# linnanwang/FastGen

Measured on AMD Instinct MI355X. Metric: images/sec at 4-step distilled (DMD2) sampling, higher is better.
Workload: dtype fp32 (tensors, accumulate) with split-bf16 x3 MFMA conv products; 1 GPU; EDM CIFAR-10 32x32 SongUNet (55.7M params) DMD2 4-step 'sde' sampling, batch=512 per GPU; global_batch=512, sample_steps=4, parallelism=replicas x1 (no data-path collective), graph=True

## Files before the change

### fastgen_amd/_lib.py

```python
import ctypes
import os
from ctypes import POINTER, c_char_p, c_double, c_float, c_int, c_int64, c_size_t, c_uint64, c_void_p

_HERE = os.path.dirname(os.path.abspath(__file__))
LIB_PATH = os.path.join(_HERE, "libfastgen_amd.so")

FG_MAX_LEVELS = 8
FG_DTYPE_F32, FG_DTYPE_BF16, FG_DTYPE_BF16X3 = 0, 1, 2
DTYPE_NAMES = {"fp32": FG_DTYPE_F32, "bf16": FG_DTYPE_BF16, "bf16x3": FG_DTYPE_BF16X3}
FG_SAMPLE_SDE, FG_SAMPLE_ODE = 0, 1
SAMPLE_TYPES = {"sde": FG_SAMPLE_SDE, "ode": FG_SAMPLE_ODE}
FG_LOOP_X0, FG_LOOP_MEANFLOW, FG_LOOP_EULER = 0, 1, 2
LOOP_KINDS = {"x0": FG_LOOP_X0, "meanflow": FG_LOOP_MEANFLOW, "euler": FG_LOOP_EULER}
FG_SCHEDULE_EDM, FG_SCHEDULE_RF = 0, 1
FG_DROP_PRECOND_INPUT, FG_DROP_PRECOND_OUTPUT = 1, 2
FG_BWD_DECODER, FG_BWD_ENCODER, FG_BWD_EMBED = 1, 2, 4
FG_MODEL_SONGUNET, FG_MODEL_DHARIWAL = 0, 1


class fg_edm_config(ctypes.Structure):
    _fields_ = [
        ("img_resolution", c_int), ("img_channels", c_int), ("label_dim", c_int), ("augment_dim", c_int),
        ("model_channels", c_int), ("num_levels", c_int), ("channel_mult", c_int * FG_MAX_LEVELS),
        ("channel_mult_emb", c_int), ("num_blocks", c_int), ("num_attn_resolutions", c_int),
        ("attn_resolutions", c_int * FG_MAX_LEVELS), ("channel_mult_noise", c_int), ("sigma_data", c_double),
        ("sigma_shift", c_double), ("compute_dtype", c_int), ("r_timestep", c_int), ("drop_precond", c_int),
        ("schedule", c_int), ("model_type", c_int),
    ]


class fg_edm2_config(ctypes.Structure):
    _fields_ = [
        ("img_resolution", c_int), ("img_channels", c_int), ("label_dim", c_int), ("model_channels", c_int), ("num_levels", c_int),
        ("channel_mult", c_int * FG_MAX_LEVELS), ("channel_mult_noise", c_int), ("channel_mult_emb", c_int), ("num_blocks", c_int),
        ("num_attn_resolutions", c_int), ("attn_resolutions", c_int * FG_MAX_LEVELS), ("label_balance", c_double),
        ("concat_balance", c_double), ("res_balance", c_double), ("attn_balance", c_double), ("clip_act", c_double),
        ("sigma_data", c_double), ("sigma_shift", c_double), ("compute_dtype", c_int), ("drop_precond", c_int),
    ]


class fg_dit_config(ctypes.Structure):
    _fields_ = [("input_size", c_int), ("patch_size", c_int), ("in_channels", c_int), ("hidden_size", c_int), ("depth", c_int),
                ("num_heads", c_int), ("mlp_hidden", c_int), ("embedding_rows", c_int), ("r_timestep", c_int), ("compute_dtype", c_int)]


class fg_wan_config(ctypes.Structure):
    _fields_ = [("num_heads", c_int), ("head_dim", c_int), ("in_channels", c_int), ("out_channels", c_int), ("text_dim", c_int),
                ("freq_dim", c_int), ("ffn_dim", c_int), ("num_layers", c_int), ("rope_max_seq_len", c_int), ("chunk_size", c_int),
                ("total_num_frames", c_int), ("eps", c_float)]


class fg_wan_block_taps(ctypes.Structure):
    _fields_ = [("attn1", c_void_p), ("x_attn1", c_void_p), ("attn2", c_void_p), ("x_attn2", c_void_p), ("x_ffn", c_void_p)]


class fg_dit_sampler_config(ctypes.Structure):
    _fields_ = [("t_scale", c_double), ("guidance_scale", c_double), ("use_sit_convention", c_int), ("time_cond_diff", c_int),
                ("net_pred_flow", c_int), ("schedule", c_int)]


class fg_wan_sampler_config(ctypes.Structure):
    _fields_ = [("t_scale", c_double), ("context_noise", c_double), ("net_pred_flow", c_int), ("schedule", c_int), ("prefill_frames", c_int)]


class fg_wan_guided_sampler_config(ctypes.Structure):
    _fields_ = [("t_scale", c_double), ("context_noise", c_double), ("guidance", c_int)]


SIGNATURES = {
    "fg_last_error": (c_char_p, []),
    "fg_version": (c_char_p, []),
    "fg_edm_create": (c_int, [POINTER(fg_edm_config), POINTER(c_void_p)]),
    "fg_edm_destroy": (None, [c_void_p]),
    "fg_edm_num_params": (c_int, [c_void_p]),
    "fg_edm_param_info": (c_int, [c_void_p, c_int, POINTER(c_char_p), POINTER(c_int), POINTER(c_int64)]),
    "fg_edm_bind_param": (c_int, [c_void_p, c_char_p, c_void_p, c_int64]),
    "fg_edm_pack_weights": (c_int, [c_void_p, c_void_p]),
    "fg_edm_workspace_bytes": (c_size_t, [c_void_p, c_int]),
    "fg_edm_forward": (c_int, [c_void_p, c_void_p, c_void_p, c_void_p, c_void_p, c_void_p, c_void_p, c_int, c_void_p,
                               c_size_t, c_void_p]),
    "fg_edm_num_feature_taps": (c_int, [c_void_p]),
    "fg_edm_feature_info": (c_int, [c_void_p, c_int, POINTER(c_char_p), POINTER(c_int), POINTER(c_int)]),
    "fg_edm_forward_features": (c_int, [c_void_p, c_void_p, c_void_p, c_void_p, c_void_p, c_void_p, POINTER(c_void_p), c_int,
                                        c_void_p, c_size_t, c_void_p]),
    "fg_sampler_run": (c_int, [c_void_p, c_void_p, c_void_p, POINTER(c_double), c_int, c_int, c_int, c_void_p, c_uint64,
                               c_void_p, c_int, c_void_p, c_size_t, c_int, c_void_p]),
    "fg_edm_t_list": (c_int, [c_int, POINTER(c_double)]),
    "fg_rf_t_list": (c_int, [c_int, POINTER(c_double)]),
    "fg_edm_profile_begin": (c_int, [c_void_p]),
    "fg_edm_profile_end": (c_int, [c_void_p, POINTER(c_int64), POINTER(c_double), POINTER(c_double)]),
    "fg_edm_num_blocks": (c_int, [c_void_p]),
    "fg_edm_block_info": (c_int, [c_void_p, c_int, POINTER(c_char_p), POINTER(c_int), POINTER(c_int), POINTER(c_int),
                                  POINTER(c_int), POINTER(c_int)]),
    "fg_edm_run_block": (c_int, [c_void_p, c_int, c_void_p, c_int, c_void_p, c_int, c_void_p, c_void_p, c_int, c_void_p,
                                 c_size_t, c_void_p]),
    "fg_op_gn_coeffs": (c_int, [c_void_p, c_int, c_void_p, c_int, c_void_p, c_void_p, c_float, c_void_p, c_int, c_int, c_void_p]),
    "fg_op_adm_conv_pack_bytes": (c_size_t, [c_int, c_int, c_int, c_int]),
    "fg_op_adm_conv_pack": (c_int, [c_int, c_void_p, c_void_p, c_int, c_int, c_int, c_void_p]),
    "fg_op_adm_conv": (c_int, [c_int, c_int, c_void_p, c_int, c_void_p, c_int, c_int, c_int, c_int, c_int, c_void_p, c_int, c_void_p,
                               c_void_p, c_void_p, c_int, c_void_p, c_int, c_void_p]),
    "fg_op_adm_gn_workspace_bytes": (c_size_t, [c_int, c_int, c_int]),
    "fg_op_adm_gn_coeffs": (c_int, [c_void_p, c_int, c_void_p, c_int, c_void_p, c_void_p, c_float, c_void_p, c_int, c_void_p, c_int,
                                    c_int, c_void_p, c_size_t, c_void_p]),
    "fg_op_adm_attention": (c_int, [c_void_p, c_void_p, c_int, c_int, c_int, c_void_p]),
    "fg_op_adm_map_in": (c_int, [c_void_p, c_void_p, c_void_p, c_void_p, c_int, c_void_p, c_int, c_int, c_void_p]),
    "fg_op_latents": (c_int, [c_void_p, c_double, c_void_p, c_int64, c_void_p]),
    "fg_op_forward_process": (c_int, [c_void_p, c_void_p, c_double, c_int, c_void_p, c_int64, c_void_p]),
    "fg_op_x0_to_eps": (c_int, [c_void_p, c_void_p, c_double, c_int, c_void_p, c_int64, c_void_p]),
    "fg_op_conv_wgrad_workspace_bytes": (ctypes.c_size_t, [c_int, c_int, c_int, c_int, c_int]),
    "fg_op_conv_wgrad": (c_int, [c_void_p, c_void_p, c_void_p, c_int, c_int, c_int, c_int, c_int, c_int, c_void_p, ctypes.c_size_t, c_void_p]),
    "fg_op_conv_wgrad_f32": (c_int, [c_void_p, c_void_p, c_void_p, c_int, c_int, c_int, c_int, c_int, c_int, c_void_p, ctypes.c_size_t, c_void_p]),
    "fg_edm_bind_grad": (c_int, [c_void_p, c_char_p, c_void_p, c_int64]),
    "fg_edm_block_backward_workspace_bytes": (c_size_t, [c_void_p, c_int, c_int]),
    "fg_edm_run_block_backward": (c_int, [c_void_p, c_int, c_void_p, c_int, c_void_p, c_int, c_void_p, c_void_p, c_void_p,
                                          c_void_p, c_void_p, c_int, c_void_p, c_size_t, c_void_p]),
    "fg_edm_backward_workspace_bytes": (c_size_t, [c_void_p, c_int]),
    "fg_edm_backward": (c_int, [c_void_p, c_void_p, c_void_p, c_void_p, c_void_p, c_void_p, c_void_p, c_int, c_int, c_void_p,
                                c_size_t, c_void_p]),
    "fg_edm_forward_train": (c_int, [c_void_p, c_void_p, c_void_p, c_void_p, c_void_p, c_void_p, c_void_p, c_int, c_void_p,
                                     c_size_t, c_void_p]),
    "fg_edm_backward_ex": (c_int, [c_void_p, c_void_p, c_void_p, c_void_p, c_void_p, c_void_p, c_void_p, c_void_p, c_void_p, c_int,
                                   c_int, c_void_p, c_size_t, c_void_p]),
    "fg_edm_backward_part": (c_int, [c_void_p, c_void_p, c_void_p, c_void_p, c_void_p, c_void_p, c_void_p, c_void_p, c_void_p, c_int,
                                     c_int, c_int, c_void_p, c_size_t, c_void_p]),
    "fg_edm2_create": (c_int, [POINTER(fg_edm2_config), POINTER(c_void_p)]),
    "fg_edm2_destroy": (None, [c_void_p]),
    "fg_edm2_num_params": (c_int, [c_void_p]),
    "fg_edm2_param_info": (c_int, [c_void_p, c_int, POINTER(c_char_p), POINTER(c_int), POINTER(c_int64)]),
    "fg_edm2_bind_param": (c_int, [c_void_p, c_char_p, c_void_p, c_int64]),
    "fg_edm2_pack_weights": (c_int, [c_void_p, c_void_p]),
    "fg_edm2_workspace_bytes": (c_size_t, [c_void_p, c_int]),
    "fg_edm2_forward": (c_int, [c_void_p, c_void_p, c_void_p, c_void_p, c_void_p, c_void_p, c_int, c_void_p, c_size_t, c_void_p]),
    "fg_edm2_set_training": (c_int, [c_void_p, c_int]),
    "fg_edm2_sampler_run": (c_int, [c_void_p, c_void_p, c_void_p, POINTER(c_double), c_int, c_int, c_int, c_void_p, c_uint64,
                                    c_void_p, c_int, c_void_p, c_size_t, c_int, c_void_p]),
    "fg_edm2_num_blocks": (c_int, [c_void_p]),
    "fg_edm2_block_info": (c_int, [c_void_p, c_int, POINTER(c_char_p), POINTER(c_int), POINTER(c_int), POINTER(c_int),
                                   POINTER(c_int), POINTER(c_int)]),
    "fg_edm2_run_block": (c_int, [c_void_p, c_int, c_void_p, c_int, c_void_p, c_int, c_void_p, c_void_p, c_int, c_void_p,
                                  c_size_t, c_void_p]),
    "fg_dit_create": (c_int, [POINTER(fg_dit_config), POINTER(c_void_p)]),
    "fg_dit_destroy": (None, [c_void_p]),
    "fg_dit_num_params": (c_int, [c_void_p]),
    "fg_dit_param_info": (c_int, [c_void_p, c_int, POINTER(c_char_p), POINTER(c_int), POINTER(c_int64)]),
    "fg_dit_bind_param": (c_int, [c_void_p, c_char_p, c_void_p, c_int64]),
    "fg_dit_pack_weights": (c_int, [c_void_p, c_void_p]),
    "fg_dit_pack_group": (c_int, [c_void_p, c_char_p, c_char_p, c_void_p]),
    "fg_dit_workspace_bytes": (c_size_t, [c_void_p, c_int]),
    "fg_dit_forward": (c_int, [c_void_p, c_void_p, c_void_p, c_void_p, c_void_p, c_void_p, c_void_p, c_int, c_void_p, c_size_t, c_void_p]),
    "fg_dit_forward_features": (c_int, [c_void_p, c_void_p, c_void_p, c_void_p, c_void_p, c_void_p, c_void_p, POINTER(c_int), POINTER(c_void_p),
                                        c_int, c_int, c_void_p, c_size_t, c_void_p]),
    "fg_dit_sampler_workspace_bytes": (c_size_t, [c_void_p, c_int, c_int]),
    "fg_dit_sampler_run": (c_int, [c_void_p, POINTER(fg_dit_sampler_config), c_void_p, c_void_p, c_void_p, POINTER(c_double), c_int, c_int, c_int,
                                   c_void_p, c_uint64, c_void_p, c_int, c_void_p, c_size_t, c_int, c_void_p]),
    "fg_wan_sampler_workspace_bytes": (c_size_t, [c_void_p, c_int, c_int, c_int, c_int]),
    "fg_wan_sampler_run": (c_int, [c_void_p, POINTER(fg_wan_sampler_config), c_void_p, POINTER(c_double), c_int, c_int, POINTER(c_int), c_void_p,
                                   c_uint64, c_int, c_int, c_int, c_int, c_void_p, c_size_t, c_int, c_void_p]),
    "fg_wan_guided_sampler_workspace_bytes": (c_size_t, [c_void_p, c_int, c_int, c_int, c_int, c_int, c_int]),
    "fg_wan_guided_sampler_run": (c_int, [c_void_p, POINTER(fg_wan_guided_sampler_config), c_void_p, POINTER(c_double), POINTER(c_double), c_int,
                                          c_void_p, c_uint64, c_int, c_int, c_int, c_int, c_void_p, c_size_t, c_int, c_void_p]),
    "fg_op_guided_multistep": (c_int, [c_void_p, c_void_p, c_void_p, c_void_p, c_void_p, c_void_p, c_int, c_int, c_int64, c_void_p]),
    "fg_wan_select_cache_tag": (c_int, [c_void_p, c_int]),
    "fg_wan_create": (c_int, [POINTER(fg_wan_config), POINTER(c_void_p)]),
    "fg_wan_destroy": (None, [c_void_p]),
    "fg_wan_num_params": (c_int, [c_void_p]),
    "fg_wan_param_info": (c_int, [c_void_p, c_int, POINTER(c_char_p), POINTER(c_int), POINTER(c_int64)]),
    "fg_wan_bind_param": (c_int, [c_void_p, c_char_p, c_void_p, c_int64]),
    "fg_wan_pack_weights": (c_int, [c_void_p, c_void_p]),
    "fg_wan_pack_group": (c_int, [c_void_p, c_char_p, c_char_p, c_void_p]),
    "fg_wan_workspace_bytes": (c_size_t, [c_void_p, c_int, c_int, c_int, c_int]),
    "fg_wan_clear_caches": (c_int, [c_void_p, c_void_p]),
    "fg_wan_set_text": (c_int, [c_void_p, c_void_p, c_int, c_int, c_void_p, c_size_t, c_void_p]),
    "fg_wan_forward": (c_int, [c_void_p, c_void_p, c_void_p, c_void_p, c_int, c_int, c_int, c_int, c_int, c_int, c_void_p, c_size_t,
                               c_void_p]),
    "fg_wan_forward_block_causal": (c_int, [c_void_p, c_void_p, c_void_p, c_void_p, c_int, c_int, c_int, c_int, c_void_p, c_size_t, c_void_p]),
    "fg_wan_forward_features": (c_int, [c_void_p, c_void_p, c_void_p, c_void_p, c_int, c_int, c_int, c_int, c_int, c_int, c_int, POINTER(c_int),
                                        POINTER(fg_wan_block_taps), c_int, c_void_p, c_void_p, c_void_p, c_size_t, c_void_p]),
    "fg_disc_edm_num_params": (c_int, [c_int]),
    "fg_disc_edm_workspace_bytes": (c_size_t, [c_int, c_int]),
    "fg_disc_edm_run": (c_int, [c_void_p, c_int, c_void_p, c_void_p, c_void_p, c_void_p, c_void_p, c_int, c_void_p, c_size_t, c_void_p]),
    "fg_edm_jvp": (c_int, [c_void_p, c_void_p, c_void_p, c_void_p, c_void_p, c_void_p, c_void_p, c_void_p, c_void_p, c_void_p, c_int,
                           c_void_p, c_size_t, c_void_p]),
    "fg_edm_set_dropout": (c_int, [c_void_p, c_float, c_uint64]),
    "fg_op_dropout_mask": (c_int, [c_void_p, c_int64, c_float, ctypes.c_uint32, c_uint64, c_void_p]),
    "fg_edm_set_augment": (c_int, [c_void_p, c_void_p]),
    "fg_edm_set_training": (c_int, [c_void_p, c_int]),
    "fg_op_images_to_u8": (c_int, [c_void_p, c_void_p, c_int64, c_int, c_int, c_int, c_void_p]),
    "fg_op_randn": (c_int, [c_void_p, c_int64, c_uint64, c_uint64, c_void_p]),
    "fg_op_attention": (c_int, [c_void_p, c_void_p, c_void_p, c_void_p, c_int, c_int, c_int, c_int, c_int, c_void_p]),
    "fg_op_attention_split": (c_int, [c_void_p, c_void_p, c_void_p, c_void_p, c_int, c_int, c_int, c_int, c_int, c_int, c_void_p]),
    "fg_op_gemm_bf16": (c_int, [c_void_p, c_void_p, c_void_p, c_void_p, c_int, c_int, c_int, c_int, c_void_p, c_int, c_int, c_void_p,
                                c_int, c_void_p]),
    "fg_op_gemm_x3": (c_int, [c_void_p, c_void_p, c_void_p, c_void_p, c_int, c_int, c_int, c_int, c_void_p, c_int, c_int, c_void_p,
                              c_int, c_void_p]),
}

_lib = None


def lib():
    global _lib
    if _lib is None:
        if not os.path.exists(LIB_PATH):
            raise RuntimeError(
                f"{LIB_PATH} not found: build it with `python -c 'import __graft_entry__ as g; g.build()'` "
                "(or `make -C fastgen_amd/csrc`).  fastgen_amd has no non-HIP fallback.")
        L = ctypes.CDLL(LIB_PATH)
        for name, (res, args) in SIGNATURES.items():
            fn = getattr(L, name)
            fn.restype = res
            fn.argtypes = args
        _lib = L
    return _lib


class FastGenAMDError(RuntimeError):
    pass


def check(rc: int):
    if rc != 0:
        msg = lib().fg_last_error().decode("utf-8", "replace")
        raise FastGenAMDError(f"fastgen_amd error {rc}: {msg}")
```

### fastgen_amd/csrc/aux.hip

```cpp
#include "common.h"
#include "misc.h"

namespace {

constexpr int APITCH = 144;
constexpr int HWID = 34, HROWS = 6;

template <typename T>
__global__ __launch_bounds__(256) void aux_head_kernel(const typename DT<T>::ST* __restrict__ x, const float2* __restrict__ ab,
                                                       const typename DT<T>::WT* __restrict__ wpack, const float* __restrict__ bias,
                                                       const float* __restrict__ x_t, const float* __restrict__ coef,
                                                       float* __restrict__ out, float* __restrict__ raw, int B, int C, int cout) {
    typedef typename DT<T>::ST ST;
    typedef typename DT<T>::WT WT;
    constexpr int KC = DT<T>::KC, KK = KC / 16, OPP = KC / 8;
    constexpr int FB = DT<T>::FRAG_BYTES, WP = DT<T>::WPARTS;
    constexpr bool FAST = DT<T>::FAST;
    constexpr int LOG_OPP = (OPP == 8) ? 3 : 2;
    constexpr int PSTRIDE = 256 / OPP;
    constexpr int HALO_PIX = HROWS * HWID;
    constexpr int NITEMS = (HALO_PIX * OPP + 255) / 256;
    __shared__ __attribute__((aligned(16))) char smem[HALO_PIX * APITCH];

    const int tid = threadIdx.x, lane = tid & 63, wave = tid >> 6;
    const int r = lane & 31, h = lane >> 5;
    const int n = blockIdx.x >> 3, row0 = (blockIdx.x & 7) * 4;
    const int oct = tid & (OPP - 1), hq0 = tid >> LOG_OPP;
    const int nchunk = C / KC;

    f32x16 acc;
#pragma unroll
    for (int i = 0; i < 16; ++i) acc[i] = 0.f;

    for (int chunk = 0; chunk < nchunk; ++chunk) {
        float2 abr[8];
        {
            const float2* p = ab + (size_t)n * C + chunk * KC + oct * 8;
#pragma unroll
            for (int j = 0; j < 8; j += 2) {
                const f32x4 q = *reinterpret_cast<const f32x4*>(p + j);
                abr[j] = make_float2(q[0], q[1]);
                abr[j + 1] = make_float2(q[2], q[3]);
            }
        }
#pragma unroll
        for (int i = 0; i < NITEMS; ++i) {
            const int hq = hq0 + i * PSTRIDE;
            if (hq < HALO_PIX) {
                const int hx = hq % HWID, hy = hq / HWID;
                const int y = row0 + hy - 1, xx = hx - 1;
                float o[8];
#pragma unroll
                for (int j = 0; j < 8; ++j) o[j] = 0.f;
                if (y >= 0 && y < 32 && xx >= 0 && xx < 32) {
                    const ST* p = x + (((size_t)n * 32 + y) * 32 + xx) * C + chunk * KC + oct * 8;
                    const f32x4 lo = load4(p), hi = load4(p + 4);
#pragma unroll
                    for (int j = 0; j < 4; ++j) {
                        o[j] = silu_f<FAST>(fmaf(lo[j], abr[j].x, abr[j].y));
                        o[j + 4] = silu_f<FAST>(fmaf(hi[j], abr[j + 4].x, abr[j + 4].y));
                    }
                }
                lds_store_a<T>(smem + hq * APITCH + oct * FB, o);
            }
        }
        __syncthreads();
        const WT* wp = wpack + (size_t)chunk * 9 * KK * 512 * WP + lane * 8;
#pragma unroll
        for (int tap = 0; tap < 9; ++tap) {
            const char* abase = smem + ((wave + tap / 3) * HWID + r + tap % 3) * APITCH + h * FB;
#pragma unroll
            for (int kk = 0; kk < KK; ++kk) {
                const Frag8<T> af = lds_read_a<T>(abase, kk);
                const Frag8<T> bf = load_wfrag<T>(wp + (tap * KK + kk) * 512 * WP);
                mma16(acc, af, bf);
            }
        }
        __syncthreads();
    }
    if (r < cout) {
        const float c_skip = coef[2 * B + n], c_out = coef[3 * B + n];
        const float bv = bias[r];
        const int y = row0 + wave;
#pragma unroll
        for (int i = 0; i < 16; ++i) {
            const size_t o = (((size_t)n * cout + r) * 32 + y) * 32 + acc_row(i, h);
            out[o] = c_skip * x_t[o] + c_out * (acc[i] + bv);
            if (raw) raw[o] = acc[i] + bv;
        }
    }
}

template <typename T>
__global__ void pack_aux_weights_kernel(const float* __restrict__ w, typename DT<T>::WT* __restrict__ out, int C, int cout) {
    constexpr int KC = DT<T>::KC, KK = KC / 16;
    const int total = C * 9 * 32;
    for (int idx = blockIdx.x * blockDim.x + threadIdx.x; idx < total; idx += gridDim.x * blockDim.x) {
        int t = idx;
        const int j = t % 8; t /= 8;
        const int lane = t % 64; t /= 64;
        const int kk = t % KK; t /= KK;
        const int tap = t % 9; t /= 9;
        const int chunk = t;
        const int co = lane & 31;
        const int ci = chunk * KC + kk * 16 + 8 * (lane >> 5) + j;
        const float v = (co < cout) ? w[((size_t)co * C + ci) * 9 + tap] : 0.f;
        if constexpr (DT<T>::WPARTS == 1) {
            out[idx] = (typename DT<T>::WT)v;
        } else {
            const size_t o = ((size_t)idx / 512) * 1024 + (idx % 512);
            const __bf16 hi = (__bf16)v;
            out[o] = hi;
            out[o + 512] = (__bf16)(v - (float)hi);
        }
    }
}

template <typename T>
__global__ __launch_bounds__(256) void stem_kernel(const float* __restrict__ x, const float* __restrict__ c_in,
                                                   const T* __restrict__ wpack, const float* __restrict__ bias,
                                                   T* __restrict__ out, float2* __restrict__ stats, int B, int res, int cin) {
    const int lane = threadIdx.x & 63, wave = threadIdx.x >> 6;
    const int r = lane & 31, h = lane >> 5;
    const int hw = res * res;
    const long long p0 = ((long long)blockIdx.x * 4 + wave) * 32;
    const int n = (int)(p0 / hw);
    if (n >= B) return;
    const int pix = (int)(p0 % hw) + r;
    const int y = pix / res, xx = pix % res;
    const float ci_scale = c_in[n];
    f32x16 acc[4];
#pragma unroll
    for (int nt = 0; nt < 4; ++nt)
#pragma unroll
        for (int i = 0; i < 16; ++i) acc[nt][i] = 0.f;
#pragma unroll
    for (int s = 0; s < 2; ++s) {
        float v[8];
#pragma unroll
        for (int j = 0; j < 8; ++j) {
            const int k = s * 16 + 8 * h + j;
            const int ci = k / 9, kh = (k % 9) / 3, kw = k % 3;
            const int yy = y + kh - 1, xs = xx + kw - 1;
            v[j] = 0.f;
            if (k < cin * 9 && yy >= 0 && yy < res && xs >= 0 && xs < res)
                v[j] = ci_scale * x[(((size_t)n * cin + ci) * res + yy) * res + xs];
        }
        Frag8<T> af;
        store_frag(reinterpret_cast<T*>(&af), v);
#pragma unroll
        for (int nt = 0; nt < 4; ++nt) {
            const Frag8<T> bf = load_frag(wpack + ((s * 4 + nt) * 64 + lane) * 8);
            mma16(acc[nt], af, bf);
        }
    }
    T* obase = out + ((size_t)n * hw + (p0 % hw)) * 128;
#pragma unroll
    for (int nt = 0; nt < 4; ++nt) {
        const float bv = bias[nt * 32 + r];
        float sv = 0.f, qv = 0.f;
#pragma unroll
        for (int i = 0; i < 16; ++i) {
            const float v = acc[nt][i] + bv;
            obase[(size_t)acc_row(i, h) * 128 + nt * 32 + r] = (T)v;
            sv += v;
            qv = fmaf(v, v, qv);
        }
        if (stats) {
            sv += __shfl_xor(sv, 32), qv += __shfl_xor(qv, 32);
            sv += __shfl_xor(sv, 1), qv += __shfl_xor(qv, 1);
            sv += __shfl_xor(sv, 2), qv += __shfl_xor(qv, 2);
            if (h == 0 && (r & 3) == 0)
                stats[((size_t)n * (hw / 32) + (int)(p0 % hw) / 32) * 32 + nt * 8 + (r >> 2)] = make_float2(sv, qv);
        }
    }
}

template <typename T>
__global__ void pack_stem_weights_kernel(const float* __restrict__ w, T* __restrict__ out, int cin) {
    const int idx = blockIdx.x * blockDim.x + threadIdx.x;
    if (idx >= 2 * 4 * 64 * 8) return;
    const int j = idx & 7, lane = (idx >> 3) & 63, nt = (idx >> 9) & 3, s = idx >> 11;
    const int co = nt * 32 + (lane & 31), k = s * 16 + 8 * (lane >> 5) + j;
    out[idx] = (k < cin * 9) ? (T)w[(size_t)co * cin * 9 + k] : (T)0.f;
}

}

size_t aux_pack_elems(int C) { return (size_t)C * 9 * 32; }

int launch_pack_aux_weights(int dtype, const float* w, void* out, int C, int cout, hipStream_t s) {
    const int grid = (int)((aux_pack_elems(C) + 255) / 256);
    if (dtype == 2)
        hipLaunchKernelGGL(pack_aux_weights_kernel<bf16x3>, dim3(grid), dim3(256), 0, s, w, (__bf16*)out, C, cout);
    else if (dtype)
        hipLaunchKernelGGL(pack_aux_weights_kernel<__bf16>, dim3(grid), dim3(256), 0, s, w, (__bf16*)out, C, cout);
    else
        hipLaunchKernelGGL(pack_aux_weights_kernel<float>, dim3(grid), dim3(256), 0, s, w, (float*)out, C, cout);
    return (int)hipGetLastError();
}

int aux_head_supported(int dtype, int res, int C, int cout) { return res == 32 && C % (dtype == 1 ? 64 : 32) == 0 && cout <= 32; }

int launch_aux_head(int dtype, const void* x, const float2* ab, const void* wpack, const float* bias, const float* x_t,
                    const float* coef, float* out, int B, int C, int cout, hipStream_t s, float* raw) {
    if (dtype == 2)
        hipLaunchKernelGGL(aux_head_kernel<bf16x3>, dim3(B * 8), dim3(256), 0, s, (const float*)x, ab, (const __bf16*)wpack, bias, x_t, coef, out, raw, B, C, cout);
    else if (dtype)
        hipLaunchKernelGGL(aux_head_kernel<__bf16>, dim3(B * 8), dim3(256), 0, s, (const __bf16*)x, ab, (const __bf16*)wpack, bias, x_t, coef, out, raw, B, C, cout);
    else
        hipLaunchKernelGGL(aux_head_kernel<float>, dim3(B * 8), dim3(256), 0, s, (const float*)x, ab, (const float*)wpack, bias, x_t, coef, out, raw, B, C, cout);
    return (int)hipGetLastError();
}

int stem_supported(int res, int cin, int cout) { return cout == 128 && cin * 9 <= 32 && (res * res) % 32 == 0; }
size_t stem_pack_elems() { return 2 * 4 * 64 * 8; }
int launch_pack_stem_weights(int dtype, const float* w, void* out, int cin, hipStream_t s) {
    if (dtype)
        hipLaunchKernelGGL(pack_stem_weights_kernel<__bf16>, dim3(16), dim3(256), 0, s, w, (__bf16*)out, cin);
    else
        hipLaunchKernelGGL(pack_stem_weights_kernel<float>, dim3(16), dim3(256), 0, s, w, (float*)out, cin);
    return (int)hipGetLastError();
}
int launch_stem(int dtype, const float* x, const float* c_in, const void* wpack, const float* bias, void* out, float2* stats,
                int B, int res, int cin, hipStream_t s) {
    const long long waves = (long long)B * res * res / 32;
    dim3 grid((unsigned)((waves + 3) / 4));
    if (dtype)
        hipLaunchKernelGGL(stem_kernel<__bf16>, grid, dim3(256), 0, s, x, c_in, (const __bf16*)wpack, bias, (__bf16*)out, stats, B, res, cin);
    else
        hipLaunchKernelGGL(stem_kernel<float>, grid, dim3(256), 0, s, x, c_in, (const float*)wpack, bias, (float*)out, stats, B, res, cin);
    return (int)hipGetLastError();
}
```

### fastgen_amd/csrc/engine.hip

```cpp
#include <hip/hip_runtime.h>

#include <cmath>
#include <cstdarg>
#include <cstdio>
#include <cstdlib>
#include <cstring>
#include <string>
#include <map>
#include <vector>

#include "../../include/fastgen_amd.h"
#include "common.h"
#include "adm.h"
#include "edm2.h"
#include "conv.h"
#include "misc.h"

namespace {

thread_local std::string g_err;

int fail(int code, const char* fmt, ...) {
    char buf[512];
    va_list ap;
    va_start(ap, fmt);
    vsnprintf(buf, sizeof buf, fmt, ap);
    va_end(ap);
    g_err = buf;
    return code;
}

#define HIP_TRY(expr)                                                                                          \
    do {                                                                                                       \
        hipError_t e_ = (hipError_t)(expr);                                                                    \
        if (e_ != hipSuccess) return fail(FG_EHIP, "%s failed: %s (%s:%d)", #expr, hipGetErrorString(e_), __FILE__, __LINE__); \
    } while (0)

struct Param {
    std::string name;
    int ndim = 0;
    int64_t shape[4] = {1, 1, 1, 1};
    int64_t numel = 0;
    const float* ptr = nullptr;
    float* grad = nullptr;
};

enum Kind { K_STEM, K_BLOCK, K_AUX_NORM, K_AUX_CONV };

struct Block {
    std::string key;
    Kind kind = K_BLOCK;
    int cin = 0, cout = 0, res_in = 0, res_out = 0;
    bool up = false, down = false, attn = false, has_skip = false, is_dec = false;
    int skip_c = 0;
    int temb_off = 0;
    int norm0_w = -1, norm0_b = -1, conv0_w = -1, conv0_b = -1, aff_w = -1, aff_b = -1, norm1_w = -1, norm1_b = -1,
        conv1_w = -1, conv1_b = -1, skip_w = -1, skip_b = -1, norm2_w = -1, norm2_b = -1, qkv_w = -1, qkv_b = -1,
        proj_w = -1, proj_b = -1, w = -1, b = -1;
    void *p_conv0 = nullptr, *p_conv1 = nullptr, *p_skip = nullptr, *p_qkv = nullptr, *p_proj = nullptr;
    void *p_conv0_ws = nullptr, *p_conv1_ws = nullptr;
    void* p_conv0_sub = nullptr;
    int tap = -1;
    float* qkv_bias = nullptr;
    void* p_qv = nullptr;
    float* qv_bias = nullptr;
    void* p_aux = nullptr;
    void* p_stem = nullptr;
};

struct Arena {
    char* base = nullptr;
    size_t off = 0, cap = 0;
    bool dry = false;
    void* take(size_t bytes) {
        off = (off + 255) & ~(size_t)255;
        void* p = dry ? nullptr : base + off;
        off += bytes;
        return p;
    }
    template <typename T>
    T* get(size_t n) {
        return reinterpret_cast<T*>(take(n * sizeof(T)));
    }
};

struct Act {
    void* p = nullptr;
    float2* st = nullptr;
    int slots = 0;
};

struct AdmWs {
    float *e2 = nullptr, *lab = nullptr;
    float2* part = nullptr;
    std::vector<float*> skip;
    float *xa = nullptr, *xb = nullptr, *h = nullptr, *s = nullptr, *t1 = nullptr, *qkv = nullptr, *a = nullptr;
};
struct AdmNet;

struct Workspace {
    AdmWs adm;
    float *coef, *emb0, *emb1, *emb, *temb;
    float2 *ab0, *ab1, *ab2;
    float2 *mr0 = nullptr, *mr1 = nullptr, *mr2 = nullptr;
    void* a1d = nullptr;
    bool infer = false;
    DropArgs drop;
    std::vector<Act> skip;
    Act xa, xb, h, xattn;
    void *sbuf, *aout, *pool;
    void *cvt1, *cvt2;
    void *q, *k, *vt;
    float *x, *x_pred, *eps;
    double* tl;
    uint64_t* seed;
};

struct BlockStash {
    void* h = nullptr;
    float2 *ab0 = nullptr, *ab1 = nullptr, *ab2 = nullptr, *mr0 = nullptr, *mr1 = nullptr, *mr2 = nullptr;
    void *xattn = nullptr, *q = nullptr, *k = nullptr, *vt = nullptr, *aout = nullptr;
    void* a1d = nullptr;
    uint32_t index = 0;
};
struct TrainStash {
    std::vector<Act> dec_store;
    std::vector<BlockStash> blocks;
    float2* aux_ab = nullptr;
    float2* aux_mr = nullptr;
    float* raw_out = nullptr;
};

struct HandleBase {
    std::vector<Param> params;
    std::string name_prefix;
    std::vector<void*> owned;
    bool packed = false, device_ready = false;

    HandleBase() = default;
    HandleBase(const HandleBase&) = delete;
    HandleBase& operator=(const HandleBase&) = delete;
    ~HandleBase() {
        for (void* p : owned) (void)hipFree(p);
    }
    int find(const std::string& n) const {
        for (size_t i = 0; i < params.size(); ++i)
            if (params[i].name == n) return (int)i;
        return -1;
    }
    int add(const std::string& n, std::initializer_list<int64_t> shp) {
        Param p;
        p.name = name_prefix + n;
        p.ndim = (int)shp.size();
        p.numel = 1;
        int i = 0;
        for (int64_t s : shp) {
            p.shape[i++] = s;
            p.numel *= s;
        }
        params.push_back(p);
        return (int)params.size() - 1;
    }
    template <typename F>
    int check_bound(F&& optional) const {
        for (size_t i = 0; i < params.size(); ++i)
            if (!params[i].ptr && !optional((int)i)) return fail(FG_ENOTREADY, "parameter '%s' is not bound", params[i].name.c_str());
        return FG_OK;
    }
    int alloc(void** p, size_t bytes) {
        HIP_TRY(hipMalloc(p, bytes));
        owned.push_back(*p);
        return FG_OK;
    }
    void free(void* p) {
        if (!p) return;
        for (size_t i = 0; i < owned.size(); ++i)
            if (owned[i] == p) {
                owned.erase(owned.begin() + i);
                break;
            }
        (void)hipFree(p);
    }
};

int param_info(const HandleBase* h, int index, const char** name, int* ndim, int64_t shape[4]) {
    if (!h || index < 0 || index >= (int)h->params.size()) return fail(FG_EINVAL, "param index out of range");
    const Param& p = h->params[index];
    if (name) *name = p.name.c_str();
    if (ndim) *ndim = p.ndim;
    if (shape)
        for (int i = 0; i < 4; ++i) shape[i] = p.shape[i];
    return FG_OK;
}
int bind_param(HandleBase* h, const char* name, const float* device_ptr, int64_t numel, int* index = nullptr) {
    if (!h || !name || !device_ptr) return fail(FG_EINVAL, "null argument");
    const int i = h->find(name);
    if (i < 0) return fail(FG_EINVAL, "unknown parameter '%s'", name);
    if (h->params[i].numel != numel)
        return fail(FG_EINVAL, "parameter '%s': expected %lld elements, got %lld", name, (long long)h->params[i].numel, (long long)numel);
    h->params[i].ptr = device_ptr;
    h->packed = false;
    if (index) *index = i;
    return FG_OK;
}

struct ScalarRing {
    static constexpr int kSlots = 8, kDoubles = 72;
    struct Slot {
        double tl[kDoubles];
        uint64_t seed[8];
    };
    Slot* slots = nullptr;
    hipEvent_t ev[kSlots] = {};
    bool used[kSlots] = {};
    int next = 0;
    int ensure() {
        if (slots) return FG_OK;
        HIP_TRY(hipHostMalloc((void**)&slots, sizeof(Slot) * kSlots));
        for (int i = 0; i < kSlots; ++i) HIP_TRY(hipEventCreateWithFlags(&ev[i], hipEventDisableTiming));
        return FG_OK;
    }
    int upload(const double* tl, int n, uint64_t seed, double* tl_dev, uint64_t* seed_dev, hipStream_t s) {
        int rc = ensure();
        if (rc) return rc;
        const int si = next;
        next = (si + 1) % kSlots;
        if (used[si]) HIP_TRY(hipEventSynchronize(ev[si]));
        Slot& sl = slots[si];
        for (int i = 0; i < n; ++i) sl.tl[i] = tl[i];
        sl.seed[0] = seed;
        sl.seed[1] = 0;
        HIP_TRY(hipMemcpyAsync(tl_dev, sl.tl, sizeof(double) * n, hipMemcpyHostToDevice, s));
        HIP_TRY(hipMemcpyAsync(seed_dev, sl.seed, sizeof(uint64_t) * 2, hipMemcpyHostToDevice, s));
        HIP_TRY(hipEventRecord(ev[si], s));
        used[si] = true;
        return FG_OK;
    }
    void destroy() {
        if (slots) (void)hipHostFree(slots);
        for (int i = 0; i < kSlots; ++i)
            if (ev[i]) (void)hipEventDestroy(ev[i]);
        slots = nullptr;
    }
};

struct GraphEntry {
    std::vector<int64_t> key;
    hipGraph_t graph = nullptr;
    hipGraphExec_t exec = nullptr;
    void drop() {
        if (exec) (void)hipGraphExecDestroy(exec);
        if (graph) (void)hipGraphDestroy(graph);
        exec = nullptr, graph = nullptr;
        key.clear();
    }
};

template <typename F>
int graph_run(GraphEntry& e, const std::vector<int64_t>& key, hipStream_t& cap, hipStream_t s, F&& enqueue) {
    if (!e.exec || e.key != key) {
        e.drop();
        if (!cap) HIP_TRY(hipStreamCreateWithFlags(&cap, hipStreamNonBlocking));
        HIP_TRY(hipStreamBeginCapture(cap, hipStreamCaptureModeThreadLocal));
// ... 253 lines not shown
            b.skip_w = h->add(key + ".skip.weight", {cout, cin, 1, 1});
            b.skip_b = h->add(key + ".skip.bias", {cout});
        }
        if (attn) {
            b.norm2_w = h->add(key + ".norm2.weight", {cout});
            b.norm2_b = h->add(key + ".norm2.bias", {cout});
            b.qkv_w = h->add(key + ".qkv.weight", {3 * cout, cout, 1, 1});
            b.qkv_b = h->add(key + ".qkv.bias", {3 * cout});
            b.proj_w = h->add(key + ".proj.weight", {cout, cout, 1, 1});
            b.proj_b = h->add(key + ".proj.bias", {cout});
        }
        b.temb_off = h->temb_total;
        h->temb_total += cout;
        return b;
    };
    auto res_name = [](int r) { return std::to_string(r) + "x" + std::to_string(r); };

    std::vector<int> skips;
    int cout = c.img_channels;
    for (int level = 0; level < c.num_levels; ++level) {
        const int res = c.img_resolution >> level;
        if (level == 0) {
            Block b;
            b.key = "model.enc." + res_name(res) + "_conv";
            b.kind = K_STEM;
            b.cin = cout;
            b.cout = cout = c.model_channels;
            b.res_in = b.res_out = res;
            b.w = h->add(b.key + ".weight", {b.cout, b.cin, 3, 3});
            b.b = h->add(b.key + ".bias", {b.cout});
            h->enc.push_back(b);
        } else {
            h->enc.push_back(make_block("model.enc." + res_name(res) + "_down", cout, cout, res, false, true, false, 0, false));
        }
        skips.push_back(cout);
        for (int idx = 0; idx < c.num_blocks; ++idx) {
            const int cin = cout;
            cout = c.model_channels * c.channel_mult[level];
            h->enc.push_back(make_block("model.enc." + res_name(res) + "_block" + std::to_string(idx), cin, cout, res,
                                        false, false, is_attn_res(res), 0, false));
            if (std::to_string(idx).rfind("3", 0) == 0) h->enc.back().tap = h->num_taps++;
            skips.push_back(cout);
        }
    }
    for (int level = c.num_levels - 1; level >= 0; --level) {
        const int res = c.img_resolution >> level;
        if (level == c.num_levels - 1) {
            h->dec.push_back(make_block("model.dec." + res_name(res) + "_in0", cout, cout, res, false, false, true, 0, true));
            h->dec.push_back(make_block("model.dec." + res_name(res) + "_in1", cout, cout, res, false, false, false, 0, true));
        } else {
            h->dec.push_back(make_block("model.dec." + res_name(res) + "_up", cout, cout, res, true, false, false, 0, true));
        }
        for (int idx = 0; idx <= c.num_blocks; ++idx) {
            const int sk = skips.back();
            skips.pop_back();
            const int cin = cout + sk;
            cout = c.model_channels * c.channel_mult[level];
            const bool attn = (idx == c.num_blocks) && is_attn_res(res);
            h->dec.push_back(make_block("model.dec." + res_name(res) + "_block" + std::to_string(idx), cin, cout, res,
                                        false, false, attn, sk, true));
        }
        if (level == 0) {
            Block n;
            n.key = "model.dec." + res_name(res) + "_aux_norm";
            n.kind = K_AUX_NORM;
            n.cin = n.cout = cout;
            n.res_in = n.res_out = res;
            n.w = h->add(n.key + ".weight", {cout});
            n.b = h->add(n.key + ".bias", {cout});
            h->dec.push_back(n);
            Block a;
            a.key = "model.dec." + res_name(res) + "_aux_conv";
            a.kind = K_AUX_CONV;
            a.cin = cout;
            a.cout = c.img_channels;
            a.res_in = a.res_out = res;
            a.w = h->add(a.key + ".weight", {a.cout, a.cin, 3, 3});
            a.b = h->add(a.key + ".bias", {a.cout});
            h->dec.push_back(a);
        }
    }
    h->add("model.logvar_linear.weight", {1, h->noise_ch});
    h->add("model.logvar_linear.bias", {1});
    for (auto& b : h->enc)
        if (b.kind == K_BLOCK) h->blocks.push_back(&b);
    for (auto& b : h->dec)
        if (b.kind == K_BLOCK) h->blocks.push_back(&b);
}

int check_supported(const fg_edm* h) {
    const fg_edm_config& c = h->cfg;
    const int kc = h->dtype ? 64 : 32;
    if (c.img_resolution != 32 && c.img_resolution != 16 && c.img_resolution != 8)
        return fail(FG_EINVAL, "img_resolution %d unsupported (8, 16, 32)", c.img_resolution);
    if ((c.img_resolution >> (c.num_levels - 1)) < 8)
        return fail(FG_EINVAL, "lowest resolution %d < 8 unsupported", c.img_resolution >> (c.num_levels - 1));
    if (c.img_channels > 4) return fail(FG_EINVAL, "img_channels %d > 4 unsupported", c.img_channels);
    for (const Block* b : h->blocks) {
        if (b->cout != 256) return fail(FG_EINVAL, "%s: out_channels %d unsupported (kernels are tiled for 256)", b->key.c_str(), b->cout);
        if (b->cin % kc || (b->cin - b->skip_c) % kc)
            return fail(FG_EINVAL, "%s: in_channels %d not a multiple of %d", b->key.c_str(), b->cin, kc);
        if (b->attn && b->res_out > 16) return fail(FG_EINVAL, "%s: attention at %dx%d unsupported", b->key.c_str(), b->res_out, b->res_out);
    }
    return FG_OK;
}

void adm_build_layout(fg_edm* h);
int adm_check_supported(const fg_edm* h);
size_t adm_plan_workspace(const fg_edm* h, int B, Arena& A, Workspace& w);
int adm_pack_weights(fg_edm* h, hipStream_t s);
int adm_forward(fg_edm* h, const float* x_t, const double* t, int t_stride, const float* labels, float* out, int B, Workspace& w,
                hipStream_t s);
int adm_refuse(const fg_edm* h, const char* what) {
    return fail(FG_EINVAL, "%s is not implemented for DhariwalUNet (forward and sampling only)", what);
}

size_t plan_workspace(const fg_edm* h, int B, Arena& A, Workspace& w) {
    if (h->adm) return adm_plan_workspace(h, B, A, w);
    const fg_edm_config& c = h->cfg;
    const size_t tsz = h->dtype ? 2 : 4;
    const int R = c.img_resolution;
    size_t max_act = 0;
    int max_c = 0, max_attn_hw = 0;
    for (const Block& b : h->enc) max_act = std::max(max_act, (size_t)b.res_out * b.res_out * b.cout);
    for (const Block* b : h->blocks) {
        max_act = std::max(max_act, (size_t)b->res_out * b->res_out * b->cout);
        max_c = std::max(max_c, std::max(b->cin, b->cout));
        if (b->attn) max_attn_hw = std::max(max_attn_hw, b->res_out * b->res_out);
    }
    w.coef = A.get<float>(5 * (size_t)B);
    w.emb0 = A.get<float>((size_t)B * h->cond_ch);
    w.emb1 = A.get<float>((size_t)B * h->emb_ch);
    w.emb = A.get<float>((size_t)B * h->emb_ch);
    w.temb = A.get<float>((size_t)B * h->temb_total);
    w.ab0 = A.get<float2>((size_t)B * max_c);
    w.ab1 = A.get<float2>((size_t)B * max_c);
    w.ab2 = A.get<float2>((size_t)B * max_c);
    const size_t st_elems = (size_t)B * 32 * 64;
    auto act = [&](size_t elems, size_t st_n) {
        Act a;
        a.p = A.take(elems * tsz);
        a.st = A.get<float2>(st_n);
        return a;
    };
    w.skip.clear();
    for (const Block& b : h->enc)
        w.skip.push_back(act((size_t)B * b.res_out * b.res_out * b.cout,
                             (b.kind == K_STEM && b.p_stem) ? (size_t)B * b.res_out * b.res_out : st_elems));
    w.xa = act((size_t)B * max_act, st_elems);
    w.xb = act((size_t)B * max_act, st_elems);
    w.h = act((size_t)B * max_act, st_elems);
    w.sbuf = A.take((size_t)B * max_act * tsz);
    w.pool = A.take((size_t)B * max_act * tsz);
    w.cvt1 = A.take((size_t)B * max_act * 4 * tsz);
    w.cvt2 = A.take((size_t)B * max_act * 4 * tsz);
    w.xattn = act((size_t)B * max_attn_hw * 256, st_elems);
    w.aout = A.take((size_t)B * max_attn_hw * 256 * tsz);
    w.q = A.take((size_t)B * max_attn_hw * 256 * tsz);
    w.k = A.take((size_t)B * max_attn_hw * 256 * tsz);
    w.vt = A.take((size_t)B * max_attn_hw * 256 * tsz);
    const size_t img = (size_t)B * c.img_channels * R * R;
    w.x = A.get<float>(img);
    w.x_pred = A.get<float>(img);
    w.eps = A.get<float>(img);
    w.tl = A.get<double>(ScalarRing::kDoubles);
    w.seed = A.get<uint64_t>(8);
    return (A.off + 255) & ~(size_t)255;
}

int conv_launch(fg_edm* h, int ks, int pro, int res, int outmode, const ConvArgs& a, hipStream_t s) {
    const bool timed = h->prof_on && ks == 3 && res == RES_NONE && a.W == 32 && outmode == OUT_NHWC;
    hipEvent_t e0 = nullptr, e1 = nullptr;
    if (timed) {
        if (hipEventCreate(&e0) != hipSuccess || hipEventCreate(&e1) != hipSuccess) return (int)hipErrorUnknown;
        (void)hipEventRecord(e0, s);
    }
    const int rc = launch_conv_fused(h->cmode, ks, pro, res, outmode, a, s);
    if (timed) {
        (void)hipEventRecord(e1, s);
        h->prof_ev.push_back(e0);
        h->prof_ev.push_back(e1);
        h->prof_flops += 2.0 * a.B * a.H * a.W * (double)a.Cout * 9.0 * (a.C1 + a.C2);
    }
    return rc;
}

const float kSkipScale = (float)std::sqrt(0.5);
const float kBlockEps = 1e-6f;

int norm_coeffs(int dtype, const Act& x1, int c1, const Act& x2, int c2, const float* gamma, const float* beta, float2* ab,
                int B, int hw, hipStream_t s, float2* mr = nullptr) {
    if (x1.st && (!c2 || x2.st))
        HIP_TRY(launch_gn_finalize(x1.st, c1, x1.slots, c2 ? x2.st : nullptr, c2, c2 ? x2.slots : 0, gamma, beta, kBlockEps, ab, B, hw, s, mr));
    else
        HIP_TRY(launch_gn_coeffs(dtype, x1.p, c1, c2 ? x2.p : nullptr, c2, gamma, beta, kBlockEps, ab, B, hw, s, mr));
    return FG_OK;
}

void use_stash(Workspace& w, const BlockStash& st) {
    w.h.p = st.h;
    w.ab0 = st.ab0, w.ab1 = st.ab1, w.mr0 = st.mr0, w.mr1 = st.mr1;
    w.a1d = st.a1d;
    w.drop.block = st.index;
    if (st.xattn) {
        w.xattn.p = st.xattn;
        w.ab2 = st.ab2, w.mr2 = st.mr2;
        w.q = st.q, w.k = st.k, w.vt = st.vt, w.aout = st.aout;
    }
}
int block_index(const fg_edm* h, const Block* b) {
    for (size_t i = 0; i < h->blocks.size(); ++i)
        if (h->blocks[i] == b) return (int)i;
    return -1;
}

bool attn_merge_enabled() {
    static const bool on = [] {
        const char* e = getenv("FASTGEN_AMD_ATTN_MERGE");
        return !(e && e[0] == '0');
    }();
    return on;
}

int run_block(fg_edm* h, const Block& b, const Act& x1, int c1, const Act& x2, int c2, const float* temb, Act& out, int B,
              Workspace& w, hipStream_t s) {
    if (c1 + c2 != b.cin) return fail(FG_EINVAL, "%s: got %d+%d input channels, expected %d", b.key.c_str(), c1, c2, b.cin);
    const int hw_in = b.res_in * b.res_in, hw = b.res_out * b.res_out;
    const int res_mode = b.down ? RES_DOWN : (b.up ? RES_UP : RES_NONE);
    const int slots = conv_stat_slots(b.res_out);
    int rc;
    if ((rc = norm_coeffs(h->dtype, x1, c1, x2, c2, h->P(b.norm0_w), h->P(b.norm0_b), w.ab0, B, hw_in, s, w.mr0))) return rc;
    ConvArgs a{};
    a.src1 = x1.p; a.src2 = c2 ? x2.p : nullptr; a.C1 = c1; a.C2 = c2;
    a.Hs = a.Ws = b.res_in; a.H = a.W = b.res_out; a.B = B;
    a.ab = w.ab0; a.wpack = b.p_conv0; a.wpack_ws = b.p_conv0_ws; a.bias = h->P(b.conv0_b);
    a.temb = temb + b.temb_off; a.temb_stride = h->temb_total;
    a.resid = nullptr; a.scale = 1.0f; a.out = w.h.p; a.Cout = b.cout; a.stats = w.h.st;
    const bool x3_up = b.up && w.infer && !w.a1d && h->cmode == FG_DTYPE_BF16X3 && conv_ws_enabled();
    bool sub0 = false;
    if (x3_up && conv_subpix_mode() == 2 && b.p_conv0_sub) {
        ConvArgs p = a;
        p.wpack_ws = b.p_conv0_sub;
        sub0 = conv_x3ws_supported(3, PRO_GN_SILU, RES_SUBPIX, OUT_NHWC, p);
    }
    if (sub0) {
        a.wpack_ws = b.p_conv0_sub;
        w.h.slots = conv_launch_stat_slots(h->cmode, 3, PRO_GN_SILU, RES_SUBPIX, OUT_NHWC, a);
        HIP_TRY(conv_launch(h, 3, PRO_GN_SILU, RES_SUBPIX, OUT_NHWC, a, s));
    } else if (b.down && !c2) {
        HIP_TRY(launch_gn_silu_pool(h->dtype, x1.p, w.ab0, w.pool, B, b.res_out, b.res_out, c1, s));
        a.src1 = w.pool; a.Hs = a.Ws = b.res_out; a.ab = nullptr;
        w.h.slots = conv_launch_stat_slots(h->cmode, 3, PRO_NONE, RES_NONE, OUT_NHWC, a);
        HIP_TRY(conv_launch(h, 3, PRO_NONE, RES_NONE, OUT_NHWC, a, s));
    } else {
        w.h.slots = conv_launch_stat_slots(h->cmode, 3, PRO_GN_SILU, res_mode, OUT_NHWC, a);
        HIP_TRY(conv_launch(h, 3, PRO_GN_SILU, res_mode, OUT_NHWC, a, s));
    }
    ConvArgs d{};
    d.src1 = w.h.p; d.C1 = b.cout; d.Hs = d.Ws = d.H = d.W = b.res_out; d.B = B;
    d.ab = w.ab1; d.wpack = b.p_conv1; d.wpack_ws = b.p_conv1_ws; d.bias = h->P(b.conv1_b);
    d.scale = kSkipScale; d.Cout = b.cout;
    const void* resid = x1.p;
    if (b.has_skip) {
        bool low = false;
        if (x3_up && conv_subpix_mode() >= 1) {
            ConvArgs p = d;
            p.resid = w.sbuf; p.rshift = 1;
            low = conv_x3ws_supported(3, PRO_GN_SILU, RES_NONE, OUT_NHWC, p);
        }
        ConvArgs k{};
        k.src1 = x1.p; k.src2 = c2 ? x2.p : nullptr; k.C1 = c1; k.C2 = c2;
        k.Hs = k.Ws = b.res_in; k.H = k.W = low ? b.res_in : b.res_out; k.B = B;
        k.wpack = b.p_skip; k.bias = h->P(b.skip_b); k.scale = 1.0f; k.out = w.sbuf; k.Cout = b.cout;
        HIP_TRY(conv_launch(h, 1, PRO_NONE, low ? RES_NONE : res_mode, OUT_NHWC, k, s));
        resid = w.sbuf;
        d.rshift = low ? 1 : 0;
    }
    HIP_TRY(launch_gn_finalize(w.h.st, b.cout, w.h.slots, nullptr, 0, 0, h->P(b.norm1_w), h->P(b.norm1_b), kBlockEps, w.ab1, B, hw, s, w.mr1));
    Act& x_mid = b.attn ? w.xattn : out;
    d.resid = resid; d.out = x_mid.p; d.stats = x_mid.st;
    if (w.a1d) {
        HIP_TRY(launch_gn_act(h->dtype, 0, w.h.p, b.cout, nullptr, 0, w.ab1, w.a1d, B, b.res_out, 0, s, w.drop));
        d.src1 = w.a1d; d.ab = nullptr;
        x_mid.slots = conv_launch_stat_slots(h->cmode, 3, PRO_NONE, RES_NONE, OUT_NHWC, d);
        HIP_TRY(conv_launch(h, 3, PRO_NONE, RES_NONE, OUT_NHWC, d, s));
    } else {
        x_mid.slots = conv_launch_stat_slots(h->cmode, 3, PRO_GN_SILU, RES_NONE, OUT_NHWC, d);
        HIP_TRY(conv_launch(h, 3, PRO_GN_SILU, RES_NONE, OUT_NHWC, d, s));
    }
    if (b.attn) {
        HIP_TRY(launch_gn_finalize(x_mid.st, b.cout, x_mid.slots, nullptr, 0, 0, h->P(b.norm2_w), h->P(b.norm2_b), kBlockEps, w.ab2, B, hw, s, w.mr2));
        ConvArgs q{};
        q.src1 = x_mid.p; q.C1 = b.cout; q.Hs = q.Ws = q.H = q.W = b.res_out; q.B = B;
        if (w.infer && !w.a1d && h->cmode == FG_DTYPE_BF16X3 && hw == 256 && b.cout == 256 && b.p_qv && attn_merge_enabled()) {
            q.ab = w.ab2; q.wpack = b.p_qv; q.bias = b.qv_bias; q.scale = 1.0f; q.Cout = 2 * b.cout;
            q.q_out = w.q; q.vt_out = w.vt;
            HIP_TRY(conv_launch(h, 1, PRO_GN, RES_NONE, OUT_QV, q, s));
            HIP_TRY(launch_attention_merged((const float*)w.q, (const float*)x_mid.p, w.ab2, (const float*)w.vt, h->P(b.proj_b), kSkipScale,
                                            (float*)out.p, out.st, B, s));
            out.slots = 8;
            return FG_OK;
        }
        q.ab = w.ab2; q.wpack = b.p_qkv; q.bias = b.qkv_bias; q.scale = 1.0f; q.Cout = 3 * b.cout;
        q.q_out = w.q; q.k_out = w.k; q.vt_out = w.vt;
        HIP_TRY(conv_launch(h, 1, PRO_GN, RES_NONE, OUT_QKV, q, s));
        HIP_TRY(launch_attention(h->cmode, w.q, w.k, w.vt, w.aout, B, hw, s));
        ConvArgs p{};
        p.src1 = w.aout; p.C1 = b.cout; p.Hs = p.Ws = p.H = p.W = b.res_out; p.B = B;
        p.wpack = b.p_proj; p.bias = h->P(b.proj_b); p.resid = x_mid.p; p.scale = kSkipScale; p.out = out.p; p.Cout = b.cout;
        p.stats = out.st;
        HIP_TRY(conv_launch(h, 1, PRO_NONE, RES_NONE, OUT_NHWC, p, s));
        out.slots = slots;
    }
    return FG_OK;
}

int run_mapping(fg_edm* h, const float* labels, int B, Workspace& w, hipStream_t s) {
    const fg_edm_config& c = h->cfg;
    HIP_TRY(launch_mapping_in(w.coef + B, w.coef + 4 * (size_t)B, h->freqs, labels, c.label_dim,
                              h->P(h->find("model.map_label.weight")), h->P(h->find("model.map_label.bias")), w.emb0, B,
                              h->cond_ch, h->noise_ch, s, h->augment, h->augment ? h->P(h->find("model.map_augment.weight")) : nullptr, c.augment_dim));
    HIP_TRY(launch_linear(w.emb0, h->P(h->find("model.map_layer0.weight")), h->P(h->find("model.map_layer0.bias")), w.emb1,
                          B, h->cond_ch, h->emb_ch, 1, s));
    HIP_TRY(launch_linear(w.emb1, h->P(h->find("model.map_layer1.weight")), h->P(h->find("model.map_layer1.bias")), w.emb, B,
                          h->emb_ch, h->emb_ch, 1, s));
    HIP_TRY(launch_linear(w.emb, h->aff_w, h->aff_b, w.temb, B, h->emb_ch, h->temb_total, 0, s));
    return FG_OK;
}

int run_forward(fg_edm* h, const float* x_t, const double* t, int t_stride, const double* r, int r_stride,
                const float* labels, float* out, int B, Workspace& w, hipStream_t s, float* const* feats = nullptr,
                bool early = false, TrainStash* ts = nullptr) {
    if (h->adm) return adm_forward(h, x_t, t, t_stride, labels, out, B, w, s);
    const fg_edm_config& c = h->cfg;
    HIP_TRY(launch_precond_coef(t, t_stride, c.r_timestep ? r : nullptr, r_stride, c.sigma_data, h->shift(), 1e-6,
                                c.drop_precond, w.coef, B, s));
    int rc = run_mapping(h, labels, B, w, s);
    if (rc) return rc;
    w.drop = DropArgs{};
    w.infer = ts == nullptr;
    if (ts && h->dropout_p > 0.f) w.drop.p = h->dropout_p, w.drop.seed = h->dropout_seed;
    const Act none;
    const Act* x = nullptr;
    for (size_t i = 0; i < h->enc.size(); ++i) {
        const Block& b = h->enc[i];
        if (b.kind == K_STEM) {
            if (b.p_stem) {
                HIP_TRY(launch_stem(h->dtype, x_t, w.coef, b.p_stem, h->P(b.b), w.skip[i].p, w.skip[i].st, B, b.res_out, b.cin, s));
                w.skip[i].slots = b.res_out * b.res_out / 32;
            } else {
                HIP_TRY(launch_conv_in(h->dtype, x_t, w.coef, h->P(b.w), h->P(b.b), w.skip[i].p, B, b.res_out, b.cin, b.cout, s));
                w.skip[i].st = nullptr;
            }
        } else {
            if (ts) use_stash(w, ts->blocks[block_index(h, &b)]);
            rc = run_block(h, b, *x, b.cin, none, 0, w.temb, w.skip[i], B, w, s);
            if (rc) return rc;
            if (feats && b.tap >= 0 && feats[b.tap])
                HIP_TRY(launch_act_to_nchw(h->dtype, w.skip[i].p, feats[b.tap], B, b.cout, b.res_out * b.res_out, s));
        }
        x = &w.skip[i];
    }
    if (early) return FG_OK;
    int sp = (int)h->enc.size();
    Act* pong[2] = {&w.xa, &w.xb};
    int cur = 0;
    size_t di = 0;
    const float2* aux_ab = nullptr;
    for (const Block& b : h->dec) {
        if (b.kind == K_BLOCK) {
            const Act& x2 = b.skip_c ? w.skip[--sp] : none;
            Act& dst = ts ? ts->dec_store[di++] : *pong[cur];
            if (ts) use_stash(w, ts->blocks[block_index(h, &b)]);
            rc = run_block(h, b, *x, b.cin - b.skip_c, x2, b.skip_c, w.temb, dst, B, w, s);
            if (rc) return rc;
            x = &dst;
            cur ^= 1;
        } else if (b.kind == K_AUX_NORM) {
            if (ts) w.ab0 = ts->aux_ab, w.mr0 = ts->aux_mr;
            if ((rc = norm_coeffs(h->dtype, *x, b.cin, none, 0, h->P(b.w), h->P(b.b), w.ab0, B, b.res_in * b.res_in, s, ts ? w.mr0 : nullptr))) return rc;
            aux_ab = w.ab0;
        } else if (b.kind == K_AUX_CONV) {
            if (b.p_aux)
                HIP_TRY(launch_aux_head(h->cmode, x->p, aux_ab, b.p_aux, h->P(b.b), x_t, w.coef, out, B, b.cin, b.cout, s, ts ? ts->raw_out : nullptr));
            else
                HIP_TRY(launch_aux_out(h->dtype, x->p, aux_ab, h->P(b.w), h->P(b.b), x_t, w.coef, out, B, b.res_out, b.cin, b.cout, s, ts ? ts->raw_out : nullptr));
        }
    }
    return FG_OK;
}

int enqueue_sampler(fg_edm* h, const float* noise, const float* labels, const double* t_list, int steps, int type,
                    int loop, const float* eps, float* out, int B, Workspace& w, hipStream_t s) {
    const fg_edm_config& c = h->cfg;
    const int64_t total = (int64_t)B * c.img_channels * c.img_resolution * c.img_resolution;
    const StudentLoop L{noise, t_list, steps, type, c.schedule, total, w.x, w.eps, eps, w.tl, w.seed, out, s};
    if (loop == FG_LOOP_MEANFLOW)
        return meanflow_loop(L, w.x_pred, [&](int i, float* u) {
            return run_forward(h, w.x, w.tl + i, 0, w.tl + (type == FG_SAMPLE_SDE ? steps : i + 1), 0, labels, u, B, w, s);
        });
    return x0_loop(L, w.x_pred, [&](int i, float* pred) { return run_forward(h, w.x, w.tl + i, 0, w.tl + steps, 0, labels, pred, B, w, s); });
}

int ensure_device_state(fg_edm* h) {
    if (h->device_ready) return FG_OK;
    int rc;
    const size_t tsz = h->dtype ? 2 : 4;
    for (Block* b : h->blocks) {
        if ((rc = h->alloc(&b->p_conv0, conv_pack_elems(b->cout, b->cin, 3) * tsz))) return rc;
        if ((rc = h->alloc(&b->p_conv1, conv_pack_elems(b->cout, b->cout, 3) * tsz))) return rc;
        const bool x3 = h->cmode == FG_DTYPE_BF16X3;
        if ((x3 ? conv_x3ws_shape_ok(b->cout, b->cin, b->res_out) : conv_ws_shape_ok(h->cmode, b->cout, b->cin, b->res_out)) && !b->down &&
            (rc = h->alloc(&b->p_conv0_ws, conv_pack_elems(b->cout, b->cin, 3) * tsz)))
            return rc;
        if ((x3 ? conv_x3ws_shape_ok(b->cout, b->cout, b->res_out) : conv_ws_shape_ok(h->cmode, b->cout, b->cout, b->res_out)) &&
            (rc = h->alloc(&b->p_conv1_ws, conv_pack_elems(b->cout, b->cout, 3) * tsz)))
            return rc;
        if (x3 && b->up && conv_x3ws_shape_ok(b->cout, b->cin, b->res_in) && (rc = h->alloc(&b->p_conv0_sub, conv_pack_elems(b->cout, b->cin, 4) * 4)))
            return rc;
        if (b->has_skip && (rc = h->alloc(&b->p_skip, conv_pack_elems(b->cout, b->cin, 1) * tsz))) return rc;
        if (b->attn) {
            if ((rc = h->alloc(&b->p_qkv, conv_pack_elems(3 * b->cout, b->cout, 1) * tsz))) return rc;
            if ((rc = h->alloc(&b->p_proj, conv_pack_elems(b->cout, b->cout, 1) * tsz))) return rc;
            if ((rc = h->alloc((void**)&b->qkv_bias, sizeof(float) * 3 * b->cout))) return rc;
            if (x3 && b->cout == 256 && b->res_out == 16) {
                if ((rc = h->alloc(&b->p_qv, conv_pack_elems(2 * b->cout, b->cout, 1) * tsz))) return rc;
                if ((rc = h->alloc((void**)&b->qv_bias, sizeof(float) * 2 * b->cout))) return rc;
                if (!h->qv_w && (rc = h->alloc((void**)&h->qv_w, sizeof(float) * 2 * b->cout * b->cout))) return rc;
            }
        }
    }
    for (Block& b : h->enc)
        if (b.kind == K_STEM && stem_supported(b.res_out, b.cin, b.cout))
            if ((rc = h->alloc(&b.p_stem, stem_pack_elems() * tsz))) return rc;
    for (Block& b : h->dec)
        if (b.kind == K_AUX_CONV && aux_head_supported(h->cmode, b.res_out, b.cin, b.cout))
            if ((rc = h->alloc(&b.p_aux, aux_pack_elems(b.cin) * tsz))) return rc;
    if ((rc = h->alloc((void**)&h->aff_w, sizeof(float) * (size_t)h->temb_total * h->emb_ch))) return rc;
    if ((rc = h->alloc((void**)&h->aff_b, sizeof(float) * (size_t)h->temb_total))) return rc;
    const int half = h->noise_ch / 2;
    std::vector<float> fr(half);
    for (int j = 0; j < half; ++j) fr[j] = powf(1.0f / 10000.0f, (float)j / (float)(half - 1));
    if ((rc = h->alloc((void**)&h->freqs, sizeof(float) * half))) return rc;
    HIP_TRY(hipMemcpy(h->freqs, fr.data(), sizeof(float) * half, hipMemcpyHostToDevice));
    if (conv_prepare_all(h->cmode) != 0) return fail(FG_EHIP, "hipFuncSetAttribute(dynamic LDS) failed");
    if (launch_attention(h->cmode, nullptr, nullptr, nullptr, nullptr, 1, 256, nullptr) != 0) return fail(FG_EHIP, "attention prepare failed");
    if (h->cmode == FG_DTYPE_BF16X3 && launch_attention_merged(nullptr, nullptr, nullptr, nullptr, nullptr, 0.f, nullptr, nullptr, 1, nullptr) != 0)
        return fail(FG_EHIP, "attention prepare failed");
    h->device_ready = true;
    return FG_OK;
}

#include "engine_adm.inc"

}

extern "C" {

const char* fg_last_error(void) { return g_err.c_str(); }
const char* fg_version(void) { return "fastgen_amd 0.1 gfx950"; }

int fg_edm_create(const fg_edm_config* cfg, fg_edm** out) {
    if (!cfg || !out) return fail(FG_EINVAL, "null argument");
    if (cfg->num_levels < 1 || cfg->num_levels > FG_MAX_LEVELS || cfg->num_attn_resolutions < 0 ||
        cfg->num_attn_resolutions > FG_MAX_LEVELS)
        return fail(FG_EINVAL, "bad num_levels / num_attn_resolutions");
    if (cfg->compute_dtype != FG_DTYPE_F32 && cfg->compute_dtype != FG_DTYPE_BF16 && cfg->compute_dtype != FG_DTYPE_BF16X3)
        return fail(FG_EINVAL, "bad compute_dtype");
    if ((cfg->drop_precond & ~3) || (cfg->schedule != FG_SCHEDULE_EDM && cfg->schedule != FG_SCHEDULE_RF) ||
        (cfg->r_timestep & ~1))
        return fail(FG_EINVAL, "bad r_timestep / drop_precond / schedule");
    if (cfg->model_channels <= 0 || cfg->model_channels % 16 || cfg->channel_mult_noise < 1 || cfg->channel_mult_emb < 1)
        return fail(FG_EINVAL, "bad channel configuration");
    if (cfg->model_type != FG_MODEL_SONGUNET && cfg->model_type != FG_MODEL_DHARIWAL) return fail(FG_EINVAL, "bad model_type");
    fg_edm* h = new fg_edm();
    h->cfg = *cfg;
    h->cmode = cfg->compute_dtype;
    h->dtype = cfg->compute_dtype == FG_DTYPE_BF16 ? 1 : 0;
    h->emb_ch = cfg->model_channels * cfg->channel_mult_emb;
    int rc;
    if (cfg->model_type == FG_MODEL_DHARIWAL) {
        h->adm = new AdmNet();
        h->dtype = 0;
        h->noise_ch = h->cond_ch = cfg->model_channels;
        adm_build_layout(h);
        rc = adm_check_supported(h);
        if (rc) {
            delete h->adm;
            delete h;
            return rc;
        }
        *out = h;
        return FG_OK;
    }
    h->noise_ch = cfg->model_channels * cfg->channel_mult_noise;
    h->cond_ch = h->noise_ch * (cfg->r_timestep ? 2 : 1);
    build_layout(h);
    rc = check_supported(h);
    if (rc) {
        delete h;
        return rc;
    }
    *out = h;
    return FG_OK;
}

void fg_edm_destroy(fg_edm* h) {
    if (!h) return;
    h->sampler.release();
    for (hipEvent_t e : h->prof_ev) (void)hipEventDestroy(e);
    delete h->adm;
    delete h;
}

int fg_edm_num_params(const fg_edm* h) { return h ? (int)h->params.size() : 0; }

int fg_edm_param_info(const fg_edm* h, int index, const char** name, int* ndim, int64_t shape[4]) {
    return param_info(h, index, name, ndim, shape);
}

int fg_edm_bind_param(fg_edm* h, const char* name, const float* device_ptr, int64_t numel) {
    return bind_param(h, name, device_ptr, numel);
}

int fg_edm_pack_weights(fg_edm* h, void* stream) {
    if (!h) return fail(FG_EINVAL, "null handle");
    hipStream_t s = (hipStream_t)stream;
    auto unused = [&](int i) {
        const std::string& n = h->params[i].name;
        return (n == "model.map_augment.weight" && (h->adm || !h->augment)) || n.rfind("model.logvar_linear", 0) == 0;
    };
    int rc;
    if (h->adm) {
        if ((rc = h->check_bound(unused))) return rc;
        ++h->pack_epoch;
        if ((rc = adm_pack_weights(h, s))) return rc;
        h->sampler.graph.drop();
        h->packed = true;
        return FG_OK;
    }
    if ((rc = ensure_device_state(h)) || (rc = h->check_bound(unused))) return rc;
    ++h->pack_epoch;
    for (Block* b : h->blocks) {
        HIP_TRY(launch_pack_conv_weights(h->cmode, h->P(b->conv0_w), b->p_conv0, b->cout, b->cin, 3, 0, s));
        HIP_TRY(launch_pack_conv_weights(h->cmode, h->P(b->conv1_w), b->p_conv1, b->cout, b->cout, 3, 0, s));
        if (h->cmode == FG_DTYPE_BF16X3) {
            if (b->p_conv0_ws) HIP_TRY(launch_pack_conv_weights_x3ws(h->P(b->conv0_w), b->p_conv0_ws, b->cout, b->cin, s));
            if (b->p_conv0_sub) HIP_TRY(launch_pack_conv_weights_x3sub(h->P(b->conv0_w), b->p_conv0_sub, b->cout, b->cin, s));
            if (b->p_conv1_ws) HIP_TRY(launch_pack_conv_weights_x3ws(h->P(b->conv1_w), b->p_conv1_ws, b->cout, b->cout, s));
        } else {
            if (b->p_conv0_ws) HIP_TRY(launch_pack_conv_weights_ws(h->P(b->conv0_w), b->p_conv0_ws, b->cout, b->cin, s));
            if (b->p_conv1_ws) HIP_TRY(launch_pack_conv_weights_ws(h->P(b->conv1_w), b->p_conv1_ws, b->cout, b->cout, s));
        }
        if (b->has_skip) HIP_TRY(launch_pack_conv_weights(h->cmode, h->P(b->skip_w), b->p_skip, b->cout, b->cin, 1, 0, s));
        if (b->attn) {
            HIP_TRY(launch_pack_conv_weights(h->cmode, h->P(b->qkv_w), b->p_qkv, 3 * b->cout, b->cout, 1, 1, s));
            HIP_TRY(launch_pack_conv_weights(h->cmode, h->P(b->proj_w), b->p_proj, b->cout, b->cout, 1, 0, s));
            for (int plane = 0; plane < 3; ++plane)
                HIP_TRY(hipMemcpy2DAsync(b->qkv_bias + plane * b->cout, sizeof(float), h->P(b->qkv_b) + plane,
                                         3 * sizeof(float), sizeof(float), b->cout, hipMemcpyDeviceToDevice, s));
            if (b->p_qv) {
                HIP_TRY(launch_attn_merge_weights(h->P(b->qkv_w), h->P(b->qkv_b), h->P(b->proj_w), h->qv_w, b->qv_bias, b->cout, s));
                HIP_TRY(launch_pack_conv_weights(h->cmode, h->qv_w, b->p_qv, 2 * b->cout, b->cout, 1, 0, s));
            }
        }
// ... 71 lines not shown
    if (sample_steps < 1 || sample_steps > 64 || !out_host) return fail(FG_EINVAL, "bad sample_steps");
    const int num_steps = 1000;
    const double min_t = 0.002, max_t = 80.0, rho = 7.0;
    const double a = std::pow(min_t, 1.0 / rho), b = std::pow(max_t, 1.0 / rho);
    const int lo = (int)(0.002 * num_steps), hi = (int)(0.998 * num_steps);
    for (int i = 0; i <= sample_steps; ++i) {
        const int n = sample_steps + 1;
        const float step = ((float)lo - (float)hi) / (float)(n - 1);
        const float v = (i < n / 2) ? (float)hi + step * (float)i : (float)lo - step * (float)(n - 1 - i);
        const int idx = (int)v;
        const int j = num_steps - 1 - idx;
        const double dstep = 1.0 / (double)(num_steps - 1);
        const double ramp = (j < num_steps / 2) ? dstep * j : 1.0 - dstep * (double)(num_steps - 1 - j);
        double sig = std::pow(b + ramp * (a - b), rho);
        if (i == sample_steps) sig = 0.0;
        out_host[i] = sig > max_t ? max_t : sig;
    }
    return FG_OK;
}

int fg_rf_t_list(int sample_steps, double* out_host) {
    if (sample_steps < 1 || sample_steps > 64 || !out_host) return fail(FG_EINVAL, "bad sample_steps");
    const double max_t = 0.999;
    const int n = sample_steps + 1;
    const double step = (0.0 - max_t) / (double)(n - 1);
    for (int i = 0; i < n; ++i) {
        const double v = (i < n / 2) ? max_t + step * (double)i : 0.0 - step * (double)(n - 1 - i);
        out_host[i] = v > max_t ? max_t : v;
    }
    return FG_OK;
}

int fg_sampler_run(fg_edm* h, const float* noise, const float* class_labels, const double* t_list, int steps,
                   int sample_type, int loop_kind, const float* eps, uint64_t seed, float* out, int batch, void* workspace,
                   size_t workspace_bytes, int use_graph, void* stream) {
    if (!h || !noise || !t_list || !out) return fail(FG_EINVAL, "null argument");
    int rc = check_sampler_args(t_list, steps, sample_type, loop_kind, h->cfg.schedule);
    if (rc) return rc;
    if (loop_kind != FG_LOOP_X0 && loop_kind != FG_LOOP_MEANFLOW) return fail(FG_EINVAL, "bad loop_kind");
    if ((loop_kind == FG_LOOP_MEANFLOW) != (h->cfg.r_timestep != 0))
        return fail(FG_EINVAL, "FG_LOOP_MEANFLOW needs an r_timestep network and FG_LOOP_X0 a network without one");
    Workspace w;
    if ((rc = setup_ws(plan_workspace, h, batch, workspace, workspace_bytes, w))) return rc;
    if (!h->packed) return fail(FG_ENOTREADY, "weights are not packed (call fg_edm_pack_weights)");
    return sampler_launch(h->sampler, batch, t_list, steps, sample_type, loop_kind, seed, w.tl, w.seed, use_graph && !h->prof_on,
                          {(int64_t)(uintptr_t)noise, (int64_t)(uintptr_t)class_labels, (int64_t)(uintptr_t)eps, (int64_t)(uintptr_t)out,
                           (int64_t)(uintptr_t)workspace, sample_type == FG_SAMPLE_SDE && !eps},
                          (hipStream_t)stream, [&](hipStream_t q) {
                              return enqueue_sampler(h, noise, class_labels, t_list, steps, sample_type, loop_kind, eps, out, batch, w, q);
                          });
}

int fg_edm_profile_begin(fg_edm* h) {
    if (!h) return fail(FG_EINVAL, "null handle");
    for (hipEvent_t e : h->prof_ev) (void)hipEventDestroy(e);
    h->prof_ev.clear();
    h->prof_flops = 0.0;
    h->prof_on = true;
    return FG_OK;
}

int fg_edm_profile_end(fg_edm* h, int64_t* launches, double* total_ms, double* total_flops) {
    if (!h) return fail(FG_EINVAL, "null handle");
    h->prof_on = false;
    double ms = 0.0;
    for (size_t i = 0; i + 1 < h->prof_ev.size(); i += 2) {
        HIP_TRY(hipEventSynchronize(h->prof_ev[i + 1]));
        float t = 0.f;
        HIP_TRY(hipEventElapsedTime(&t, h->prof_ev[i], h->prof_ev[i + 1]));
        ms += t;
    }
    if (launches) *launches = (int64_t)h->prof_ev.size() / 2;
    if (total_ms) *total_ms = ms;
    if (total_flops) *total_flops = h->prof_flops;
    for (hipEvent_t e : h->prof_ev) (void)hipEventDestroy(e);
    h->prof_ev.clear();
    return FG_OK;
}

FG_API int fg_debug_conv_bench(int dtype, int batch, int cin, int res, int ks, int with_resid, int dbg, int iters, float* ms_out) {
    const size_t npix = (size_t)batch * res * res;
    float *x = nullptr, *out = nullptr, *resid = nullptr, *bias = nullptr;
    float2* ab = nullptr;
    void* wp = nullptr;
    if (dtype < 0 || dtype > 2) return fail(FG_EINVAL, "bad dtype");
    HIP_TRY(hipMalloc((void**)&x, npix * cin * 4));
    HIP_TRY(hipMalloc((void**)&out, npix * 256 * 4));
    HIP_TRY(hipMalloc((void**)&resid, npix * 256 * 4));
    HIP_TRY(hipMalloc((void**)&bias, 256 * 4));
    HIP_TRY(hipMalloc((void**)&ab, (size_t)batch * cin * 8));
    HIP_TRY(hipMalloc(&wp, (size_t)256 * cin * ks * ks * 4));
    {
        const size_t blk = 4u << 20;
        std::vector<uint16_t> hb(blk / 2);
        uint32_t st = 0x12345u;
        for (auto& v : hb) {
            st = st * 1664525u + 1013904223u;
            v = (uint16_t)(((st >> 16) & 0x8000u) | ((0x78u + ((st >> 12) & 7u)) << 7) | ((st >> 20) & 0x7fu));
        }
        auto fill = [&](void* dst, size_t bytes) -> int {
            for (size_t o = 0; o < bytes; o += blk)
                HIP_TRY(hipMemcpy((char*)dst + o, hb.data(), std::min(blk, bytes - o), hipMemcpyHostToDevice));
            return FG_OK;
        };
        int rc;
        if ((rc = fill(x, npix * cin * 4)) || (rc = fill(resid, npix * 256 * 4)) || (rc = fill(ab, (size_t)batch * cin * 8)) ||
            (rc = fill(wp, (size_t)256 * cin * ks * ks * (dtype == 1 ? 2 : 4))))
            return rc;
    }
    HIP_TRY(hipMemset(bias, 0, 256 * 4));
    if (conv_prepare_all(dtype) != 0) return fail(FG_EHIP, "prepare failed");
    ConvArgs a{};
    a.src1 = x; a.C1 = cin; a.Hs = a.Ws = a.H = a.W = res; a.B = batch;
    a.ab = ab; a.wpack = wp; a.wpack_ws = wp; a.bias = bias; a.resid = with_resid ? resid : nullptr; a.scale = 1.f; a.out = out; a.Cout = 256;
    a.dbg = dbg;
    hipEvent_t e0, e1;
    HIP_TRY(hipEventCreate(&e0));
    HIP_TRY(hipEventCreate(&e1));
    auto run = [&]() { return dbg >= 64 ? launch_conv_ws_debug(a, dbg - 64, nullptr) : dbg < 0 ? launch_conv_fused(dtype, ks, ks == 3 ? PRO_GN_SILU : PRO_NONE, RES_NONE, OUT_NHWC, a, nullptr) : launch_conv_debug(dtype, a, nullptr); };
    for (int i = 0; i < 3; ++i) HIP_TRY(run());
    HIP_TRY(hipEventRecord(e0, nullptr));
    for (int i = 0; i < iters; ++i) HIP_TRY(run());
    HIP_TRY(hipEventRecord(e1, nullptr));
    HIP_TRY(hipEventSynchronize(e1));
    float ms = 0.f;
    HIP_TRY(hipEventElapsedTime(&ms, e0, e1));
    if (ms_out) *ms_out = ms / iters;
    (void)hipEventDestroy(e0); (void)hipEventDestroy(e1);
    (void)hipFree(x); (void)hipFree(out); (void)hipFree(resid); (void)hipFree(bias); (void)hipFree(ab); (void)hipFree(wp);
    return FG_OK;
}

int fg_edm_num_blocks(const fg_edm* h) {
    if (h && h->adm) return adm_num_blocks(h);
    return h ? (int)h->blocks.size() : 0;
}

int fg_edm_block_info(const fg_edm* h, int index, const char** key, int* cin, int* cout, int* res_in, int* res_out,
                      int* has_attention) {
    if (h && h->adm) return adm_block_info(h, index, key, cin, cout, res_in, res_out, has_attention);
    if (!h || index < 0 || index >= (int)h->blocks.size()) return fail(FG_EINVAL, "block index out of range");
    const Block* b = h->blocks[index];
    if (key) *key = b->key.c_str();
    if (cin) *cin = b->cin;
    if (cout) *cout = b->cout;
    if (res_in) *res_in = b->res_in;
    if (res_out) *res_out = b->res_out;
    if (has_attention) *has_attention = b->attn ? 1 : 0;
    return FG_OK;
}

int fg_edm_run_block(fg_edm* h, int index, const float* x1, int c1, const float* x2, int c2, const float* emb, float* out,
                     int batch, void* workspace, size_t workspace_bytes, void* stream) {
    if (!h || !x1 || !emb || !out) return fail(FG_EINVAL, "null argument");
    if (h->adm) return adm_run_block(h, index, x1, c1, x2, c2, emb, out, batch, workspace, workspace_bytes, (hipStream_t)stream);
    if (!h->packed) return fail(FG_ENOTREADY, "weights are not packed (call fg_edm_pack_weights)");
    if (index < 0 || index >= (int)h->blocks.size()) return fail(FG_EINVAL, "block index out of range");
    Workspace w;
    int rc0 = setup_ws(plan_workspace, h, batch, workspace, workspace_bytes, w);
    if (rc0) return rc0;
    hipStream_t s = (hipStream_t)stream;
    HIP_TRY(launch_linear(emb, h->aff_w, h->aff_b, w.temb, batch, h->emb_ch, h->temb_total, 0, s));
    const Block& b = *h->blocks[index];
    const size_t npix_in = (size_t)batch * b.res_in * b.res_in, npix_out = (size_t)batch * b.res_out * b.res_out;
    Act a1, a2;
    HIP_TRY(launch_to_act(h->dtype, x1, w.cvt1, (int64_t)npix_in * c1, s));
    a1.p = w.cvt1;
    if (c2) {
        HIP_TRY(launch_to_act(h->dtype, x2, w.cvt2, (int64_t)npix_in * c2, s));
        a2.p = w.cvt2;
    }
    w.infer = true;
    int rc = run_block(h, b, a1, c1, a2, c2, w.temb, w.xa, batch, w, s);
    if (rc) return rc;
    HIP_TRY(launch_from_act(h->dtype, w.xa.p, out, (int64_t)npix_out * b.cout, s));
    return FG_OK;
}

#include "engine_train.inc"
#include "engine_dit.inc"
#include "engine_wan.inc"
#include "engine_sampler.inc"
#include "engine_edm2.inc"

int fg_op_gn_coeffs(const float* x1, int c1, const float* x2, int c2, const float* gamma, const float* beta, float eps,
                    float* ab_out, int batch, int hw, void* stream) {
    if (!x1 || !gamma || !beta || !ab_out) return fail(FG_EINVAL, "null argument");
    HIP_TRY(launch_gn_coeffs(0, x1, c1, c2 ? x2 : nullptr, c2, gamma, beta, eps, (float2*)ab_out, batch, hw, (hipStream_t)stream));
    return FG_OK;
}

size_t fg_op_adm_conv_pack_bytes(int mode, int cout, int cin, int ks) {
    if ((mode != FG_DTYPE_BF16 && mode != FG_DTYPE_BF16X3) || (ks != 1 && ks != 3) || cout <= 0 || cin <= 0 || cin % 32) return 0;
    return adm_conv_pack_elems(mode, cout, cin, ks) * sizeof(__bf16);
}
int fg_op_adm_conv_pack(int mode, const float* w_oihw, void* packed, int cout, int cin, int ks, void* stream) {
    if (!fg_op_adm_conv_pack_bytes(mode, cout, cin, ks))
        return fail(FG_EINVAL, "fg_op_adm_conv_pack: mode %d (1 bf16, 2 bf16x3), ks %d (1, 3), cout %d > 0, cin %d (multiple of 32)", mode,
                    ks, cout, cin);
    if (!w_oihw || !packed) return fail(FG_EINVAL, "fg_op_adm_conv_pack: null pointer");
    HIP_TRY(adm_pack_conv_weights(mode, w_oihw, packed, cout, cin, ks, (hipStream_t)stream));
    return FG_OK;
}
int fg_op_adm_conv(int mode, int ks, const float* src1, int c1, const float* src2, int c2, int batch, int hs, int h, int res_mode,
                   const float* ab, int silu, const void* packed, const float* bias, const float* resid, int resid_mode, float* out,
                   int cout, void* stream) {
    if ((mode != FG_DTYPE_BF16 && mode != FG_DTYPE_BF16X3) || (ks != 1 && ks != 3))
        return fail(FG_EINVAL, "fg_op_adm_conv: mode %d (1 bf16, 2 bf16x3), ks %d (1, 3)", mode, ks);
    if (c1 <= 0 || c1 % 32 || c2 < 0 || c2 % 32 || cout <= 0 || batch <= 0 || batch > 65535)
        return fail(FG_EINVAL, "fg_op_adm_conv: c1 %d > 0 and c2 %d >= 0 multiples of 32, cout %d > 0, batch %d in 1 .. 65535", c1, c2,
                    cout, batch);
    const bool res_ok = (res_mode == 0 && hs == h) || (res_mode == 1 && hs == 2 * h) || (res_mode == 2 && h == 2 * hs);
    if (h <= 0 || h > 4096 || !res_ok) return fail(FG_EINVAL, "fg_op_adm_conv: res_mode %d with hs %d, h %d", res_mode, hs, h);
    if (resid && (resid_mode < 0 || resid_mode > 2 || (resid_mode == 2 && h % 2)))
        return fail(FG_EINVAL, "fg_op_adm_conv: resid_mode %d (0, 1, 2 with h even) at h %d", resid_mode, h);
    if (!src1 || (c2 && !src2) || !packed || !out) return fail(FG_EINVAL, "fg_op_adm_conv: null pointer");
    if (((uintptr_t)src1 | (uintptr_t)(c2 ? src2 : nullptr) | (uintptr_t)packed) & 15 || (uintptr_t)ab & 7)
        return fail(FG_EINVAL, "fg_op_adm_conv: src1 / src2 / packed must be 16-byte aligned, ab 8-byte aligned");
    AdmConvArgs a;
    a.src1 = src1, a.src2 = c2 ? src2 : nullptr, a.C1 = c1, a.C2 = c2, a.Hs = hs, a.H = h, a.B = batch, a.res_mode = res_mode;
    a.ab = (const float2*)ab, a.silu = silu ? 1 : 0, a.w = packed, a.bias = bias, a.resid = resid, a.resid_mode = resid ? resid_mode : 0;
    a.out = out, a.Cout = cout;
    HIP_TRY(adm_launch_conv(mode, ks, a, (hipStream_t)stream));
    return FG_OK;
}
size_t fg_op_adm_gn_workspace_bytes(int batch, int hw, int c) {
    if (batch <= 0 || hw <= 0 || c <= 0) return 0;
    return adm_gn_part_elems(batch, hw, c) * sizeof(float2);
}
int fg_op_adm_gn_coeffs(const float* x1, int c1, const float* x2, int c2, const float* gamma, const float* beta, float eps,
                        const float* temb, int temb_stride, float* ab_out, int batch, int hw, void* workspace, size_t workspace_bytes,
                        void* stream) {
    const int C = c1 + c2;
    if (c1 <= 0 || c1 % 2 || c2 < 0 || c2 % 2 || C < 8)
        return fail(FG_EINVAL, "fg_op_adm_gn_coeffs: c1 %d > 0 and c2 %d >= 0 must be even, c1 + c2 >= 8", c1, c2);
    const int G = std::min(32, C / 4);
    if (C % G || (C / G) % 2)
        return fail(FG_EINVAL, "fg_op_adm_gn_coeffs: %d channels in %d groups: the group size must be a whole, even number", C, G);
    if (batch <= 0 || batch > 65535 || hw <= 0 || hw > (1 << 22))
        return fail(FG_EINVAL, "fg_op_adm_gn_coeffs: batch %d (1 .. 65535), hw %d (1 .. 2^22)", batch, hw);
    if (temb && temb_stride < 2 * C) return fail(FG_EINVAL, "fg_op_adm_gn_coeffs: temb_stride %d < 2 C = %d", temb_stride, 2 * C);
    if (!x1 || (c2 && !x2) || !gamma || !beta || !ab_out || !workspace) return fail(FG_EINVAL, "fg_op_adm_gn_coeffs: null pointer");
    if (((uintptr_t)x1 | (uintptr_t)(c2 ? x2 : nullptr) | (uintptr_t)ab_out | (uintptr_t)workspace) & 7)
        return fail(FG_EINVAL, "fg_op_adm_gn_coeffs: x1 / x2 / ab_out / workspace must be 8-byte aligned");
    const size_t need = fg_op_adm_gn_workspace_bytes(batch, hw, C);
    if (workspace_bytes < need)
        return fail(FG_EINVAL, "fg_op_adm_gn_coeffs: workspace too small (%zu < %zu bytes)", workspace_bytes, need);
    HIP_TRY(adm_launch_gn(x1, c1, c2 ? x2 : nullptr, c2, gamma, beta, eps, temb, temb_stride, (float2*)workspace, (float2*)ab_out, batch,
                          hw, (hipStream_t)stream));
    return FG_OK;
}
int fg_op_adm_attention(const float* qkv, float* out, int batch, int t, int heads, void* stream) {
    if (t <= 0 || t % 64 || heads <= 0 || heads > 65535 || batch <= 0 || batch > 65535)
        return fail(FG_EINVAL, "fg_op_adm_attention: t %d (a positive multiple of 64), heads %d, batch %d (1 .. 65535)", t, heads, batch);
    if (!qkv || !out) return fail(FG_EINVAL, "fg_op_adm_attention: null pointer");
    HIP_TRY(adm_launch_attention(qkv, out, batch, t, heads, (hipStream_t)stream));
    return FG_OK;
}
int fg_op_adm_map_in(const float* c_noise, const float* freqs, const float* aug, const float* wa, int aug_dim, float* out, int batch,
                     int n, void* stream) {
    if (batch <= 0 || n <= 0 || n % 2 || (int64_t)batch * n > (1 << 30) || (aug && aug_dim <= 0))
        return fail(FG_EINVAL, "fg_op_adm_map_in: batch %d > 0, n %d > 0 even, aug_dim %d > 0 with aug", batch, n, aug_dim);
    if (!c_noise || !freqs || !out || (aug && !wa)) return fail(FG_EINVAL, "fg_op_adm_map_in: null pointer");
    HIP_TRY(adm_launch_map_in(c_noise, freqs, aug, aug ? wa : nullptr, aug ? aug_dim : 0, out, batch, n, (hipStream_t)stream));
    return FG_OK;
}
int fg_op_latents(const float* noise, double t_init, float* out, int64_t total, void* stream) {
    HIP_TRY(launch_latents(noise, t_init, nullptr, 0, out, total, (hipStream_t)stream));
    return FG_OK;
}
int fg_op_forward_process(const float* x0, const float* eps, double t, int schedule, float* out, int64_t total,
                          void* stream) {
    HIP_TRY(launch_forward_process(x0, eps, t, nullptr, 0, schedule, out, total, (hipStream_t)stream));
    return FG_OK;
}
int fg_op_x0_to_eps(const float* xt, const float* x0, double t, int schedule, float* out, int64_t total, void* stream) {
    HIP_TRY(launch_x0_to_eps(xt, x0, t, nullptr, 0, schedule, 1e-6, out, total, (hipStream_t)stream));
    return FG_OK;
}
int fg_edm_set_dropout(fg_edm* h, float p, uint64_t seed) {
    if (!h) return fail(FG_EINVAL, "null handle");
    if (!(p >= 0.f && p < 1.f)) return fail(FG_EINVAL, "dropout probability must be in [0, 1), got %g", (double)p);
    h->dropout_p = p;
    h->dropout_seed = seed;
    return FG_OK;
}
int fg_op_guided_multistep(const float* v, float* x, float* x2, float* x_last, float* m_prev, const double* tab, int guided, int first,
                           int64_t total, void* stream) {
    if (!v || !x || !x_last || !m_prev || !tab || total <= 0) return fail(FG_EINVAL, "fg_op_guided_multistep: bad argument");
    HIP_TRY(launch_guided_multistep(v, x, x2, x_last, m_prev, tab, guided != 0, first != 0, total, (hipStream_t)stream));
    return FG_OK;
}

int fg_op_dropout_mask(float* out, int64_t total, float p, uint32_t block_index, uint64_t seed, void* stream) {
    if (!out || total <= 0 || (total % 8)) return fail(FG_EINVAL, "fg_op_dropout_mask: bad argument");
    DropArgs d;
    d.p = p, d.block = block_index, d.seed = seed;
    HIP_TRY(launch_dropout_mask(out, total, d, (hipStream_t)stream));
    return FG_OK;
}
int fg_edm_set_training(fg_edm* h, int training) {
    if (!h) return fail(FG_EINVAL, "null handle");
    if ((training != 0) != h->training && h->cfg.sigma_shift != 0.0) h->sampler.graph.drop();
    h->training = training != 0;
    return FG_OK;
}
int fg_edm_set_augment(fg_edm* h, const float* augment_labels) {
    if (!h) return fail(FG_EINVAL, "null handle");
    if (augment_labels && h->cfg.augment_dim <= 0) return fail(FG_EINVAL, "this network was built without augment_dim");
    h->augment = augment_labels;
    return FG_OK;
}
int fg_disc_edm_num_params(int res) { return disc_num_params(res); }
size_t fg_disc_edm_workspace_bytes(int res, int batch) { return disc_workspace_bytes(res, batch); }
int fg_disc_edm_run(const float* feat, int res, const float* const* params, float* logits, const float* dlogits, float* dfeat,
                    float* const* grads, int batch, void* workspace, size_t workspace_bytes, void* stream) {
    const int np = disc_num_params(res);
    if (!np) return fail(FG_EINVAL, "fg_disc_edm_run: resolution %d unsupported (8, 16, 32)", res);
    if (!feat || !params || !logits || batch <= 0 || !workspace || (((uintptr_t)workspace) & 255))
        return fail(FG_EINVAL, "fg_disc_edm_run: bad argument");
    for (int i = 0; i < np; ++i)
        if (!params[i]) return fail(FG_EINVAL, "fg_disc_edm_run: parameter %d is null", i);
    if (workspace_bytes < disc_workspace_bytes(res, batch))
        return fail(FG_ENOMEM, "fg_disc_edm_run: workspace too small (%zu < %zu bytes)", workspace_bytes, disc_workspace_bytes(res, batch));
    HIP_TRY(disc_run(feat, res, params, logits, dlogits, dfeat, grads, batch, workspace, (hipStream_t)stream));
    return FG_OK;
}
size_t fg_op_conv_wgrad_workspace_bytes(int batch, int res, int cin, int cout, int ks) {
    return conv_wgrad_supported(res, cin, cout, ks) && batch > 0 ? conv_wgrad_workspace_bytes(batch, res, cin, cout, ks) : 0;
}
int fg_op_conv_wgrad(const void* act, const void* dy, float* dw, int batch, int res, int cin, int cout, int ks,
                     int accumulate, void* workspace, size_t workspace_bytes, void* stream) {
    if (!conv_wgrad_supported(res, cin, cout, ks))
        return fail(FG_EINVAL, "fg_op_conv_wgrad: unsupported shape res=%d cin=%d cout=%d ks=%d (res 8/16/32, cin %% 32 [k3] / 128 [k1], cout %% 128, ks 1/3)",
                    res, cin, cout, ks);
    if (batch <= 0 || !act || !dy || !dw || !workspace) return fail(FG_EINVAL, "fg_op_conv_wgrad: bad argument");
    if (workspace_bytes < conv_wgrad_workspace_bytes(batch, res, cin, cout, ks))
        return fail(FG_EINVAL, "fg_op_conv_wgrad: workspace too small (%zu < %zu bytes)", workspace_bytes,
                    conv_wgrad_workspace_bytes(batch, res, cin, cout, ks));
    HIP_TRY(launch_conv_wgrad(FG_DTYPE_BF16, act, dy, dw, batch, res, cin, cout, ks, accumulate, workspace, (hipStream_t)stream));
    return FG_OK;
// ... 134 lines not shown
```

### fastgen_amd/csrc/engine_train.inc

```

namespace {
struct BwdScratch {
    void *g1, *aop, *da, *dh0, *dskip, *dxin, *wpk, *wg;
    void *gmid = nullptr, *dq = nullptr, *dk = nullptr, *dvt = nullptr, *dqkv = nullptr, *att = nullptr;
    float2 *P, *S, *mr0, *mr1, *mr2;
    float *dtemb, *wt;
    size_t wg_bytes;
};
int pad256(int c) { return (c + 255) / 256 * 256; }
size_t block_wgrad_bytes(int B, int res, int cin, int cout, bool attn) {
    size_t m = 0;
    const int shapes[5][3] = {{cout, cout, 3}, {cin, cout, 3}, {cin, cout, 1}, {cout, 3 * cout, 1}, {cout, cout, 1}};
    for (int i = 0; i < (attn ? 5 : 3); ++i)
        if (conv_wgrad_supported(res, shapes[i][0], shapes[i][1], shapes[i][2]))
            m = std::max(m, conv_wgrad_workspace_bytes(B, res, shapes[i][0], shapes[i][1], shapes[i][2]));
    return m;
}
size_t plan_block_bwd(const fg_edm* h, int B, int res_in, int res, int cin, int cout, Arena& A, BwdScratch& q, int attn_hw = 0, size_t wg_bytes = 0) {
    const size_t tsz = h->dtype ? 2 : 4, wsz = h->cmode == FG_DTYPE_BF16 ? 2 : 4;
    const size_t npix = (size_t)B * res * res, npix_in = (size_t)B * res_in * res_in;
    const int cp = pad256(cin), cm = cin > cout ? cin : cout;
    q.g1 = A.take(npix * cout * tsz);
    q.aop = A.take(npix * cm * tsz);
    q.da = A.take(npix * (cp > cout ? cp : cout) * tsz);
// ... 293 lines not shown
        HIP_TRY(hipMemsetAsync(nb.vec, 0, sizeof(float) * 8, s));
        HIP_TRY(launch_batchsum_add(q.dtemb, nb.vec, B, 8, s));
        HIP_TRY(launch_add_sub_tensor(nb.vec, 8, h->G(aux_conv->b), 1, aux_conv->cout, 1, s));
    }
    if (h->G(aux_conv->w)) {
        HIP_TRY(launch_gn_act(h->dtype, 0, y.p, 256, nullptr, 0, w.ab0, q.aop, B, res, 0, s));
        if ((rc = wgrad_checked(h, q.aop, nb.dfp, nb.wtmp, B, res, 256, 128, 3, 0, nb.wgx, nb.wgx_bytes, s))) return rc;
        HIP_TRY(launch_add_sub_tensor(nb.wtmp, 256, h->G(aux_conv->w), aux_conv->cout, 256, 9, s));
    }
    HIP_TRY(launch_pad_rows(h->P(aux_conv->w), nb.wpad, aux_conv->cout, 128, 256 * 9, s));
    if ((rc = conv_dgrad(h, nb.wpad, 128, 256, 3, nb.dfp, q.da, B, res, q, s, false))) return rc;
    void* g_cur = nb.ga;
    void* g_alt = nb.gb;
    HIP_TRY(launch_gn_bwd(h->dtype, 0, y.p, 256, nullptr, 0, q.da, 256, w.ab0, q.mr0, h->P(aux_norm->w), q.P, q.S, h->G(aux_norm->w),
                          h->G(aux_norm->b), nullptr, 0, 0.f, g_cur, B, res, 0, s));
    struct Rec {
        const Block* b;
        const Act* x;
        const Act* x2;
        int sk;
    };
    std::vector<Rec> recs;
    {
        int sp = (int)h->enc.size();
        const Act* x = &w.skip.back();
        size_t di = 0;
        for (const Block& b : h->dec) {
            if (b.kind != K_BLOCK) continue;
            Rec rcd{&b, x, nullptr, -1};
            if (b.skip_c) {
                rcd.sk = --sp;
                rcd.x2 = &w.skip[rcd.sk];
            }
            recs.push_back(rcd);
            x = &nb.ts.dec_store[di++];
        }
    }
    for (int i = (int)recs.size() - 1; i >= 0; --i) {
        const Block& b = *recs[i].b;
        const int c2 = b.skip_c, c1 = b.cin - c2;
        const size_t npin = (size_t)B * b.res_in * b.res_in;
        if ((rc = block_backward(h, b, *recs[i].x, c1, c2 ? *recs[i].x2 : none, c2, w.emb, w.temb, g_cur, g_alt, nb.demb, B, w, q, s, nb.dtemb_all,
                                 &nb.ts.blocks[block_index(h, &b)], c2 ? nb.genc[recs[i].sk] : nullptr, 0)))
            return rc;
        if ((rc = block_affine_grads(h, b, nb, w, B, s))) return rc;
        (void)npin;
        std::swap(g_cur, g_alt);
    }
    {
        const Block& last = h->enc.back();
        HIP_TRY(launch_add_act(h->dtype, nb.genc.back(), g_cur, (int64_t)B * last.res_out * last.res_out * last.cout, s));
    }
    }
    if (parts & FG_BWD_ENCODER) {
    if (dfeats)
        for (size_t i = 0; i < h->enc.size(); ++i) {
            const Block& b = h->enc[i];
            if (b.tap >= 0 && dfeats[b.tap]) HIP_TRY(launch_add_nchw_to_nhwc(h->dtype, dfeats[b.tap], nb.genc[i], B, b.cout, b.res_out * b.res_out, s));
        }
    for (int i = (int)h->enc.size() - 1; i >= 1; --i) {
        const Block& b = h->enc[i];
        if ((rc = block_backward(h, b, w.skip[i - 1], b.cin, none, 0, w.emb, w.temb, nb.genc[i], nb.genc[i - 1], nb.demb, B, w, q, s, nb.dtemb_all,
                                 &nb.ts.blocks[block_index(h, &b)], nullptr, 1)))
            return rc;
        if ((rc = block_affine_grads(h, b, nb, w, B, s))) return rc;
    }
    {
        const Block& b = h->enc[0];
        if (h->G(b.b)) {
            HIP_TRY(launch_colsum(h->dtype, nb.genc[0], b.cout, b.cout, q.dtemb, B, hw, 1.0f, s));
            HIP_TRY(launch_batchsum_add(q.dtemb, h->G(b.b), B, b.cout, s));
        }
        if (h->G(b.w)) {
            HIP_TRY(launch_stem_operand(h->dtype, x_t, w.coef, nb.op32, B, b.cin, 32, hw, s));
            if ((rc = wgrad_checked(h, nb.op32, nb.genc[0], nb.wtmp, B, res, 32, b.cout, 3, 0, nb.wgx, nb.wgx_bytes, s))) return rc;
            HIP_TRY(launch_add_sub_tensor(nb.wtmp, 32, h->G(b.w), b.cout, b.cin, 9, s));
        }
        if (dx_t) {
            if ((rc = conv_dgrad(h, h->P(b.w), b.cout, b.cin, 3, nb.genc[0], q.da, B, res, q, s))) return rc;
            HIP_TRY(launch_input_grad(h->dtype, q.da, 256, w.coef, w.coef + 2 * (size_t)B, dout, dx_t, B, b.cin, hw, s));
        }
    }
    }
    if (!(parts & FG_BWD_EMBED)) return FG_OK;
    {
        const int E = h->emb_ch, TT = h->temb_total;
        if (!h->aff_wT) {
            int rc2 = h->alloc((void**)&h->aff_wT, sizeof(float) * (size_t)E * TT);
            if (rc2) return rc2;
        }
        if (h->aff_wT_epoch != h->pack_epoch) {
            HIP_TRY(launch_transpose_f32(h->aff_w, h->aff_wT, TT, E, s));
            h->aff_wT_epoch = h->pack_epoch;
        }
        HIP_TRY(launch_linear(nb.dtemb_all, h->aff_wT, nullptr, nb.demb, B, TT, E, 0, s));
    }
    {
        const int E = h->emb_ch, N = h->cond_ch;
        const int w1 = h->find("model.map_layer1.weight"), b1 = h->find("model.map_layer1.bias");
        const int w0 = h->find("model.map_layer0.weight"), b0 = h->find("model.map_layer0.bias");
        HIP_TRY(launch_linear(w.emb1, h->P(w1), h->P(b1), nb.pre, B, E, E, 0, s));
        HIP_TRY(launch_silu_bwd(nb.demb, nb.pre, nb.d1, B * E, s));
        HIP_TRY(hipMemsetAsync(nb.d0, 0, sizeof(float) * (size_t)B * E, s));
        HIP_TRY(launch_linear_bwd(nb.d1, w.emb1, h->P(w1), h->G(w1), h->G(b1), nb.d0, B, E, E, 1.0f, s));
        HIP_TRY(launch_linear(w.emb0, h->P(w0), h->P(b0), nb.pre, B, N, E, 0, s));
        HIP_TRY(launch_silu_bwd(nb.d0, nb.pre, nb.d1, B * E, s));
        HIP_TRY(hipMemsetAsync(nb.d0, 0, sizeof(float) * (size_t)B * N, s));
        HIP_TRY(launch_linear_bwd(nb.d1, w.emb0, h->P(w0), h->G(w0), h->G(b0), nb.d0, B, E, N, 1.0f, s));
        if (h->augment && c.augment_dim > 0) {
            const int wa = h->find("model.map_augment.weight");
            if (h->G(wa)) HIP_TRY(launch_linear_bwd(nb.d0, h->augment, nullptr, h->G(wa), nullptr, nullptr, B, N, c.augment_dim, 1.0f, s));
        }
        if (c.label_dim > 0) {
            const int wl = h->find("model.map_label.weight"), bl = h->find("model.map_label.bias");
            HIP_TRY(launch_linear_bwd(nb.d0, labels, nullptr, labels ? h->G(wl) : nullptr, h->G(bl), nullptr, B, N, c.label_dim,
                                      std::sqrt((float)c.label_dim), s));
        }
    }
    return FG_OK;
}

int tangent_conv(fg_edm* h, int ks, int res_mode, const void* src, int cin, int res_in, int res_out, const void* wpack, int cout,
                 const float* temb, const void* resid, float scale, void* out, int B, hipStream_t s, const void* wpack_ws = nullptr) {
    ConvArgs a{};
    a.src1 = src; a.C1 = cin; a.C2 = 0;
    a.Hs = a.Ws = res_in; a.H = a.W = res_out; a.B = B;
    a.wpack = wpack; a.wpack_ws = wpack_ws; a.bias = nullptr;
    a.temb = temb; a.temb_stride = h->temb_total;
    a.resid = resid; a.scale = scale; a.out = out; a.Cout = cout;
    HIP_TRY(launch_conv_fused(h->cmode, ks, PRO_NONE, res_mode, OUT_NHWC, a, s));
    return FG_OK;
}

int block_jvp(fg_edm* h, const Block& b, const Act& a1, int c1, const void* xd1, const Act& a2, int c2, const void* xd2,
              const float* dtemb, void* yd, int B, Workspace& w, BwdScratch& q, const BlockStash& st, const float2* ident_ab,
              hipStream_t s) {
    const int res = b.res_out, res_in = b.res_in, hw = res * res, cin = b.cin, cout = b.cout;
    const int rm = b.down ? 1 : (b.up ? 2 : 0);
    const int res_mode = b.down ? RES_DOWN : (b.up ? RES_UP : RES_NONE);
    int rc;
    use_stash(w, st);
    const void* xd = xd1;
    if (c2) {
        HIP_TRY(launch_gn_act(h->dtype, 2, xd1, c1, xd2, c2, nullptr, q.aop, B, res_in, 0, s));
        xd = q.aop;
    }
    HIP_TRY(launch_gn_jvp(h->dtype, 0, a1.p, c1, c2 ? a2.p : nullptr, c2, xd, st.ab0, st.mr0, q.P, q.S, q.da, B, res_in, s));
    const void* ad0 = q.da;
    if (rm) {
        HIP_TRY(launch_gn_act(h->dtype, 2, q.da, cin, nullptr, 0, nullptr, q.dskip, B, res, rm, s));
        ad0 = q.dskip;
    }
    if ((rc = tangent_conv(h, 3, RES_NONE, ad0, cin, res, res, b.p_conv0, cout, dtemb + b.temb_off, nullptr, 1.0f, q.dh0, B, s,
                           b.p_conv0_ws))) return rc;
    DropArgs drop;
    if (st.a1d && h->dropout_p > 0.f) drop.p = h->dropout_p, drop.seed = h->dropout_seed, drop.block = st.index;
    HIP_TRY(launch_gn_jvp(h->dtype, 0, st.h, cout, nullptr, 0, q.dh0, st.ab1, st.mr1, q.P, q.S, q.g1, B, res, s, drop));
    const void* sd = xd;
    if (b.has_skip) {
        if ((rc = tangent_conv(h, 1, res_mode, xd, cin, res_in, res, b.p_skip, cout, nullptr, nullptr, 1.0f, q.dxin, B, s))) return rc;
        sd = q.dxin;
    }
    void* mid = b.attn ? q.gmid : yd;
    if ((rc = tangent_conv(h, 3, RES_NONE, q.g1, cout, res, res, b.p_conv1, cout, nullptr, sd, kSkipScale, mid, B, s, b.p_conv1_ws))) return rc;
    if (b.attn) {
        HIP_TRY(launch_gn_jvp(h->dtype, 1, st.xattn, cout, nullptr, 0, q.gmid, st.ab2, st.mr2, q.P, q.S, q.da, B, res, s));
        ConvArgs qa{};
        qa.src1 = q.da; qa.C1 = cout; qa.Hs = qa.Ws = qa.H = qa.W = res; qa.B = B;
        qa.ab = ident_ab; qa.wpack = b.p_qkv; qa.bias = nullptr; qa.scale = 1.0f; qa.Cout = 3 * cout;
        qa.q_out = q.dq; qa.k_out = q.dk; qa.vt_out = q.dvt;
        HIP_TRY(launch_conv_fused(h->cmode, 1, PRO_GN, RES_NONE, OUT_QKV, qa, s));
        HIP_TRY(launch_attention_jvp(h->dtype, st.q, st.k, st.vt, q.dq, q.dk, q.dvt, q.da, q.att, B, hw, cout, s));
        if ((rc = tangent_conv(h, 1, RES_NONE, q.da, cout, res, res, b.p_proj, cout, nullptr, q.gmid, kSkipScale, yd, B, s))) return rc;
    }
    return FG_OK;
}

int run_jvp(fg_edm* h, const float* x_t, const double* t, const double* r, const float* labels, const float* vx, const float* vt,
            const float* vr, float* out, float* jvp, int B, Workspace& w, NetBwd& nb, hipStream_t s) {
    const fg_edm_config& c = h->cfg;
    const int res = c.img_resolution, hw = res * res, C = c.img_channels;
    BwdScratch& q = nb.q;
    if (h->dropout_p <= 0.f)
        for (BlockStash& st : nb.ts.blocks) st.a1d = nullptr;
    int rc = run_forward(h, x_t, t, 1, r, 1, labels, out, B, w, s, nullptr, false, &nb.ts);
    if (rc) return rc;
    const Block *aux_norm = nullptr, *aux_conv = nullptr;
    for (const Block& b : h->dec) {
        if (b.kind == K_AUX_NORM) aux_norm = &b;
        if (b.kind == K_AUX_CONV) aux_conv = &b;
    }
    if (!aux_norm || !aux_conv || aux_conv->cin != 256 || !h->enc[0].p_stem || !q.att)
        return fail(FG_EINVAL, "jvp: head / stem shape not covered");
    const int E = h->emb_ch, N = h->cond_ch, TT = h->temb_total;
    float* ct = nb.vec_all;
    if (8 * B > TT) return fail(FG_EINVAL, "jvp: batch too large for the coefficient scratch");
    float* e0 = nb.d0;
    float* dtemb = nb.dtemb_all;
    float2* ident = (float2*)nb.pre;
    float* ones = nb.vec;
    float* zeros = nb.vec + 512;
    if (B > 512) return fail(FG_EINVAL, "jvp: batch too large for the constant scratch");
    HIP_TRY(launch_fill_f32(ones, 1.0f, 512, s));
    HIP_TRY(launch_fill_f32(zeros, 0.0f, 512, s));
    HIP_TRY(launch_jvp_coef(t, c.r_timestep ? r : nullptr, vt, vr, c.sigma_data, h->shift(), c.drop_precond, ct, B, s));
    {
        const int w1 = h->find("model.map_layer1.weight"), b1 = h->find("model.map_layer1.bias");
        const int w0 = h->find("model.map_layer0.weight"), b0 = h->find("model.map_layer0.bias");
        HIP_TRY(launch_jvp_embed(w.coef + B, w.coef + 4 * (size_t)B, ct + 2 * (size_t)B, ct + 3 * (size_t)B, h->freqs, e0, B, N, h->noise_ch, s));
        HIP_TRY(launch_linear(w.emb0, h->P(w0), h->P(b0), nb.d1, B, N, E, 0, s));
        HIP_TRY(launch_linear(e0, h->P(w0), nullptr, nb.demb, B, N, E, 0, s));
        HIP_TRY(launch_silu_bwd(nb.demb, nb.d1, e0, B * E, s));
        HIP_TRY(launch_linear(w.emb1, h->P(w1), h->P(b1), nb.d1, B, E, E, 0, s));
        HIP_TRY(launch_linear(e0, h->P(w1), nullptr, nb.demb, B, E, E, 0, s));
        HIP_TRY(launch_silu_bwd(nb.demb, nb.d1, e0, B * E, s));
        HIP_TRY(launch_linear(e0, h->aff_w, nullptr, dtemb, B, E, TT, 0, s));
    }
    HIP_TRY(launch_fill_f2(ident, 1.0f, 0.0f, B * 256, s));
    float* xin = (float*)q.wg;
    HIP_TRY(launch_jvp_input(vx, x_t, ct, ct + B, xin, B, C * hw, s));
    HIP_TRY(launch_stem(h->dtype, xin, ones, h->enc[0].p_stem, zeros, nb.genc[0], nullptr, B, res, h->enc[0].cin, s));
    const Act none;
    for (size_t i = 1; i < h->enc.size(); ++i) {
        const Block& b = h->enc[i];
        if ((rc = block_jvp(h, b, w.skip[i - 1], b.cin, nb.genc[i - 1], none, 0, nullptr, dtemb, nb.genc[i], B, w, q,
                            nb.ts.blocks[block_index(h, &b)], ident, s)))
            return rc;
    }
    const Act* x = &w.skip.back();
    const void* xd = nb.genc.back();
    void* pong[2] = {nb.ga, nb.gb};
    int cur = 0, sp = (int)h->enc.size();
    size_t di = 0;
    for (const Block& b : h->dec) {
        if (b.kind != K_BLOCK) continue;
        const int c2 = b.skip_c, c1 = b.cin - c2;
        const Act* x2 = &none;
        const void* xd2 = nullptr;
        if (c2) {
            --sp;
            x2 = &w.skip[sp];
            xd2 = nb.genc[sp];
        }
        if ((rc = block_jvp(h, b, *x, c1, xd, *x2, c2, xd2, dtemb, pong[cur], B, w, q, nb.ts.blocks[block_index(h, &b)], ident, s)))
            return rc;
        x = &nb.ts.dec_store[di++];
        xd = pong[cur];
        cur ^= 1;
    }
    HIP_TRY(launch_gn_jvp(h->dtype, 0, x->p, 256, nullptr, 0, xd, nb.ts.aux_ab, nb.ts.aux_mr, q.P, q.S, q.da, B, res, s));
    HIP_TRY(launch_pad_rows(h->P(aux_conv->w), nb.wpad, aux_conv->cout, 256, 256 * 9, s));
    HIP_TRY(launch_pack_conv_weights(h->cmode, nb.wpad, q.wpk, 256, 256, 3, 0, s));
    if ((rc = tangent_conv(h, 3, RES_NONE, q.da, 256, res, res, q.wpk, 256, nullptr, nullptr, 1.0f, q.dh0, B, s))) return rc;
    HIP_TRY(launch_jvp_output(h->dtype, q.dh0, 256, nb.ts.raw_out, x_t, vx, ct, jvp, B, C, hw, s));
    return FG_OK;
}
}

int fg_edm_jvp(fg_edm* h, const float* x_t, const double* t, const double* r, const float* labels, const float* vx, const float* vt,
               const float* vr, float* out, float* jvp, int batch, void* workspace, size_t workspace_bytes, void* stream) {
    if (!h || !x_t || !t || !vx || !out || !jvp) return fail(FG_EINVAL, "null argument");
    if (h->adm) return adm_refuse(h, "fg_edm_jvp");
    if (!h->packed) return fail(FG_ENOTREADY, "weights are not packed (call fg_edm_pack_weights)");
    if (h->cmode == FG_DTYPE_F32) return fail(FG_EINVAL, "the forward-mode pass runs in the bf16 and bf16x3 compute modes (not in exact fp32)");
    if (h->cfg.r_timestep && !r) return fail(FG_EINVAL, "r is required by an r_timestep network");
    if (batch <= 0 || !workspace || (((uintptr_t)workspace) & 255)) return fail(FG_EINVAL, "bad batch / workspace");
    Arena A;
    A.base = (char*)workspace;
    Workspace w;
    plan_workspace(h, batch, A, w);
    NetBwd nb;
    const size_t need = plan_net_bwd(h, batch, A, nb);
    if (need > workspace_bytes) return fail(FG_ENOMEM, "workspace too small: need %zu bytes for batch %d, got %zu", need, batch, workspace_bytes);
    return run_jvp(h, x_t, t, r, labels, vx, vt, vr, out, jvp, batch, w, nb, (hipStream_t)stream);
}

size_t fg_edm_backward_workspace_bytes(const fg_edm* h, int batch) {
    if (!h || batch <= 0 || h->adm) return 0;
    Arena A;
    A.dry = true;
    Workspace w;
    plan_workspace(h, batch, A, w);
    NetBwd nb;
    return plan_net_bwd(h, batch, A, nb);
}

int fg_edm_forward_train(fg_edm* h, const float* x_t, const double* t, const double* r, const float* labels, float* out,
                         float* const* features, int batch, void* workspace, size_t workspace_bytes, void* stream) {
    if (!h || !x_t || !t || (!out && !features)) return fail(FG_EINVAL, "null argument");
    if (h->adm) return adm_refuse(h, "fg_edm_forward_train");
    if (!h->packed) return fail(FG_ENOTREADY, "weights are not packed (call fg_edm_pack_weights)");
    if (h->cmode == FG_DTYPE_F32) return fail(FG_EINVAL, "the backward pass runs in the bf16 and bf16x3 compute modes (not in exact fp32)");
    if (features)
        for (const Block& b : h->enc)
            if (b.tap >= 0 && features[b.tap] && ((b.cout % 32) || ((b.res_out * b.res_out) % 32)))
                return fail(FG_EINVAL, "feature tap %d: channels and pixels must be multiples of 32", b.tap);
    if (h->cfg.r_timestep && !r) return fail(FG_EINVAL, "r is required by an r_timestep network");
    if (batch <= 0 || !workspace || (((uintptr_t)workspace) & 255)) return fail(FG_EINVAL, "bad batch / workspace");
    Arena A;
    A.base = (char*)workspace;
    Workspace w;
    plan_workspace(h, batch, A, w);
    NetBwd nb;
    const size_t need = plan_net_bwd(h, batch, A, nb);
    if (need > workspace_bytes) return fail(FG_ENOMEM, "workspace too small: need %zu bytes for batch %d, got %zu", need, batch, workspace_bytes);
    return run_forward(h, x_t, t, 1, r, 1, labels, out, batch, w, (hipStream_t)stream, features, out == nullptr, &nb.ts);
}
// ... 95 lines not shown
```

### fastgen_amd/csrc/misc.h

```cpp
#pragma once
#include <hip/hip_runtime.h>
#include <stdint.h>

int launch_gn_coeffs(int dtype, const void* x1, int c1, const void* x2, int c2, const float* gamma, const float* beta,
                     float eps, float2* ab, int batch, int hw, hipStream_t s, float2* mr = nullptr);
int launch_gn_finalize(const float2* st1, int c1, int s1, const float2* st2, int c2, int s2, const float* gamma,
                       const float* beta, float eps, float2* ab, int batch, int hw, hipStream_t s, float2* mr = nullptr);
int launch_precond_coef(const double* t, int t_stride, const double* r, int r_stride, double sigma_data,
                        double sigma_shift, double clamp_min, int drop, float* coef, int B, hipStream_t s);
int launch_mapping_in(const float* c_noise, const float* r_noise, const float* freqs, const float* labels, int label_dim,
                      const float* wl, const float* bl, float* out, int B, int N, int noise_ch, hipStream_t s, const float* aug = nullptr, const float* wa = nullptr, int aug_dim = 0);
int launch_linear(const float* x, const float* w, const float* bias, float* y, int B, int I, int O, int act_silu,
                  hipStream_t s);
int launch_conv_in(int dtype, const float* x, const float* c_in, const float* w, const float* bias, void* out, int B,
                   int res, int cin, int cout, hipStream_t s);
int launch_aux_out(int dtype, const void* x, const float2* ab, const float* w, const float* bias, const float* x_t,
                   const float* coef, float* out, int B, int res, int C, int cout, hipStream_t s, float* raw = nullptr);
int launch_latents(const float* noise, double tv, const double* tp, int ti, float* out, int64_t total, hipStream_t s);
int launch_forward_process(const float* x0, const float* eps, double tv, const double* tp, int ti, int sched, float* out,
                           int64_t total, hipStream_t s);
int launch_x0_to_eps(const float* xt, const float* x0, double tv, const double* tp, int ti, int sched, double clamp_min,
                     float* out, int64_t total, hipStream_t s);
int launch_meanflow_update(const float* x, const float* u, const double* tp, int ia, int ib, float* out, int64_t total,
                           hipStream_t s);
int launch_randn(float* out, int64_t total, uint64_t seed, uint64_t offset, const uint64_t* seed_dev, hipStream_t s);
int launch_embed_times(const double* tp, int ti, double tv, int ri, double rv, double scale, int sit, int diff, int f32in, float* te, float* re,
                       int n, hipStream_t s);
int launch_flow_to_x0(const float* xt, const float* v, const double* tp, int ti, float sign, float* out, int64_t total, hipStream_t s);
int launch_euler_step(const float* x, const float* v, const double* tp, int ti, float g, int cfg, float sign, float* out, float* out2,
                      int64_t total, hipStream_t s);
int launch_guided_multistep(const float* v, float* x, float* x2, float* x_last, float* m_prev, const double* tab, int guided, int first,
                            int64_t total, hipStream_t s);
int launch_copy_rows(const float* src, int64_t src_pitch, float* dst, int64_t dst_pitch, int64_t run, int64_t rows, hipStream_t s);
int launch_gn_silu_pool(int dtype, const void* x, const float2* ab, void* out, int B, int H, int W, int C, hipStream_t s);
int launch_to_act(int dtype, const float* in, void* out, int64_t total, hipStream_t s);
int launch_from_act(int dtype, const void* in, float* out, int64_t total, hipStream_t s);
struct DropArgs {
    float p = 0.f;
    uint32_t block = 0;
    uint64_t seed = 0;
};
int launch_dropout_mask(float* out, int64_t total, DropArgs drop, hipStream_t s);
int launch_gn_act(int dtype, int mode, const void* x1, int c1, const void* x2, int c2, const float2* ab, void* out, int B, int res, int rm,
                  hipStream_t s, DropArgs drop = DropArgs{});
int launch_gn_bwd(int dtype, int mode, const void* x1, int c1, const void* x2, int c2, const void* dact, int cd, const float2* ab,
                  const float2* mr, const float* gamma, float2* P, float2* S, float* dgamma, float* dbeta, const void* add, int ca,
                  float add_scale, void* dx, int B, int res, int rm, hipStream_t s, void* dx2 = nullptr, int accumulate = 0,
                  DropArgs drop = DropArgs{});
int launch_colsum(int dtype, const void* t, int ct, int C, float* out, int B, int hw, float scale, hipStream_t s, int out_stride = 0);
int launch_transpose_f32(const float* in, float* out, int R, int Cc, hipStream_t s);
int launch_batchsum_add(const float* in, float* out, int B, int C, hipStream_t s, float* out2 = nullptr, int in_stride = 0);
int launch_scale_to_act(int dtype, const float* in, void* out, float scale, int64_t total, hipStream_t s);
int launch_slice_to_f32(int dtype, const void* in, int cs, int c_off, float* out, int C, int64_t npix, hipStream_t s);
int launch_affine_bwd(const float* dtemb, const float* emb, const float* w, float* dw, float* demb, int B, int C, int K, hipStream_t s);
int launch_dgrad_weights(const float* w, float* wt, int cout, int cin, int cin_pad, int taps, hipStream_t s);
int launch_head_grad(int dtype, const float* dout, const float* c_out, void* out, int B, int C, int Cp, int hw, hipStream_t s);
int launch_stem_operand(int dtype, const float* x, const float* c_in, void* out, int B, int C, int Cp, int hw, hipStream_t s);
int launch_add_sub_tensor(const float* src, int Is, float* dst, int O, int I, int T, hipStream_t s);
int launch_pad_rows(const float* src, float* dst, int O, int Op, int IT, hipStream_t s);
int launch_add_act(int dtype, void* dst, const void* src, int64_t total, hipStream_t s);
int launch_silu_bwd(const float* dy, const float* pre, float* dpre, int total, hipStream_t s);
int launch_linear_bwd(const float* dy, const float* x, const float* w, float* dw, float* db, float* dx, int B, int C, int K,
                      float scale, hipStream_t s, int dy_stride = 0);
int launch_add_nchw_to_nhwc(int dtype, const float* src, void* dst, int B, int C, int hw, hipStream_t s);
int launch_input_grad(int dtype, const void* da, int cd, const float* c_in, const float* c_skip, const float* dout, float* dx, int B, int C, int hw,
                      hipStream_t s);
int launch_gn_jvp(int dtype, int mode, const void* x1, int c1, const void* x2, int c2, const void* xd, const float2* ab, const float2* mr,
                  float2* P, float2* S, void* out, int B, int res, hipStream_t s, DropArgs drop = DropArgs{});
int launch_jvp_coef(const double* t, const double* r, const float* vt, const float* vr, double sigma_data, double sigma_shift, int drop,
                    float* ct, int B, hipStream_t s);
int launch_jvp_embed(const float* c_noise, const float* r_noise, const float* dc, const float* dr, const float* freqs, float* out, int B,
                     int N, int noise_ch, hipStream_t s);
int launch_jvp_input(const float* vx, const float* x, const float* c_in, const float* dc_in, float* out, int B, int chw, hipStream_t s);
int launch_jvp_output(int dtype, const void* fd, int cf, const float* out, const float* x, const float* vx, const float* ct, float* jvp, int B, int C,
                      int hw, hipStream_t s);
int launch_fill_f32(float* p, float v, int n, hipStream_t s);
int launch_fill_f2(float2* p, float a, float b, int n, hipStream_t s);
int launch_attention_jvp(int dtype, const void* q, const void* k, const void* vt, const void* qd, const void* kd, const void* vtd, void* od,
                         void* scratch, int B, int T, int C, hipStream_t s);
size_t attention_backward_scratch_bytes(int dtype, int B, int T, int C);
int launch_attention_backward(int dtype, const void* q, const void* k, const void* vt, const void* dO, void* dq, void* dk, void* dvt,
                              void* scratch, int B, int T, int C, hipStream_t s);
int launch_qkv_interleave(int dtype, const void* dq, const void* dk, const void* dvt, void* out, int B, int T, int C, hipStream_t s);
int launch_nt_gemm(const void* A, const void* Bm, void* C, int M, int N, int K, float scale, int out_bf16, hipStream_t s);
int launch_transpose_bf16(const void* in, void* out, int R, int Cc, hipStream_t s);
int disc_num_params(int res);
size_t disc_workspace_bytes(int res, int B);
int disc_run(const float* feat, int res, const float* const* params, float* logits, const float* dlogits, float* dfeat,
             float* const* grads, int B, void* ws, hipStream_t s);
int conv_wgrad_supported(int res, int cin, int cout, int ks);
size_t conv_wgrad_workspace_bytes(int B, int res, int cin, int cout, int ks);
int launch_conv_wgrad(int mode, const void* act, const void* dy, float* dw, int B, int res, int cin, int cout, int ks, int accumulate,
                      void* workspace, hipStream_t s, float scale = 1.0f);
int launch_images_to_u8(const float* x, uint8_t* out, int64_t B, int C, int HW, hipStream_t s);
int launch_act_to_nchw(int dtype, const void* in, float* out, int B, int C, int HW, hipStream_t s);
int launch_nchw_to_nhwc(const float* in, float* out, int B, int C, int HW, hipStream_t s);

int launch_attention(int dtype, const void* q, const void* k, const void* vt, void* out, int B, int T, hipStream_t s);
int launch_attn_merge_weights(const float* qkv_w, const float* qkv_b, const float* proj_w, float* w_out, float* b_out, int C, hipStream_t s);
int launch_attention_merged(const float* qm, const float* x_mid, const float2* ab, const float* vmt, const float* bp, float scale, float* out,
                            float2* stats, int B, hipStream_t s);

size_t aux_pack_elems(int C);
int launch_pack_aux_weights(int dtype, const float* w, void* out, int C, int cout, hipStream_t s);
int aux_head_supported(int dtype, int res, int C, int cout);
int launch_aux_head(int dtype, const void* x, const float2* ab, const void* wpack, const float* bias, const float* x_t,
                    const float* coef, float* out, int B, int C, int cout, hipStream_t s, float* raw = nullptr);

int stem_supported(int res, int cin, int cout);
size_t stem_pack_elems();
int launch_pack_stem_weights(int dtype, const float* w, void* out, int cin, hipStream_t s);
int launch_stem(int dtype, const float* x, const float* c_in, const void* wpack, const float* bias, void* out, float2* stats,
                int B, int res, int cin, hipStream_t s);

int launch_dit_ln_modulate(int dtype, int D, const void* x, const float* mod, int mod_stride, int shift_off, int scale_off, void* y,
                           int ntok, int tokens_per_image, hipStream_t s);
int launch_dit_ln_modulate_split(int D, const float* x, const float* mod, int mod_stride, int shift_off, int scale_off, void* y, int ntok,
                                 int tokens_per_image, hipStream_t s);
int launch_dit_final(int dtype, int D, const void* x, const float* mod, const float* w, const float* bias, float* out, int ntok, int grid,
                     int p, int C, hipStream_t s);
int launch_dit_patch_embed(int dtype, const float* x, const float* w, const float* bias, const float* pos, void* out, int B, int C, int grid,
                           int p, int D, hipStream_t s);
int launch_dit_fourier(const float* t, float* f, int B, int dim, hipStream_t s);
int launch_dit_cond(const float* t_emb, const float* r_emb, const float* table, const int64_t* cls, float* c, float* sc, int B, int D,
                    int rows, int* err, hipStream_t s);
int launch_dit_attention(int mode, const void* q, const void* k, const void* vt, void* out, int B, int heads, int head_dim, size_t lo_off,
                         hipStream_t s);

struct GemmArgs {
    const void* A = nullptr;
    const void* W = nullptr;
    const float* bias = nullptr;
    void* out = nullptr;
    int M = 0, N = 0, K = 0;
    int act = 0;
    const float* gate = nullptr;
    int gate_stride = 0, gate_rows = 1;
    const void* resid = nullptr;
    void *q = nullptr, *k = nullptr, *vt = nullptr;
    int heads = 0, head_dim = 0, T = 0;
    int row0 = 0;
    int lda = 0, ldw = 0;
    int a_wrap = 0;
    size_t lo_off = 0;
    float* scratch = nullptr;
    size_t scratch_bytes = 0;
    int ksplit = 1;
    int out_f32 = 0;
    int variant = -1;
    int xn = 1;
};
bool gemm_bf16_supported(const GemmArgs& a);
int launch_gemm_bf16(const GemmArgs& a, hipStream_t s, bool prepare_only = false);
int launch_cvt_bf16(const float* in, void* out, size_t n, hipStream_t s);
int launch_gemm_x3(const GemmArgs& a, int out_mode, hipStream_t s);
int launch_split3_weights(const float* w, void* out, int N, int K, hipStream_t s);
int launch_split_planes(const float* x, void* out, int64_t M, int K, hipStream_t s);

int launch_wan_patch_embed(const float* x, const float* w, const float* bias, void* out, int B, int C, int Fr, int H, int W, int D, hipStream_t s);
int launch_wan_mod(const float* table, const float* tproj, float* mod, int rows, int J, int D, hipStream_t s);
int launch_wan_outmod(const float* table, const float* temb, float* mod, int rows, int D, hipStream_t s);
int launch_silu(const float* x, float* y, int64_t n, hipStream_t s);
int launch_cvt_rows_bf16(const float* x, void* y, int64_t n, hipStream_t s);
int launch_wan_rope_table(const float2* tab_t, const float2* tab_h, const float2* tab_w, float2* cs, int L, int fs, int gw, int start, int S,
                          int nt, int nh, int nw, hipStream_t s);
int launch_rms_rope(int D, const void* src, int ld_src, const float* w, float eps, const float2* cs, void* dst, int64_t dst_bs, int dst_row0,
                    int ld_dst, int rows, int L, hipStream_t s);
size_t fa128_scratch_bytes(int B, int heads, int Lq);
int launch_fa(int hd, const void* q, int ldq, int64_t q_bs, const void* k, const void* v, int ldk, int64_t kv_bs, void* out, int ldo, int64_t o_bs,
              int B, int heads, int Lq, int Lkv, hipStream_t s, void* scratch = nullptr, int force_split = 0);
int launch_fa128(const void* q, int ldq, int64_t q_bs, const void* k, const void* v, int ldk, int64_t kv_bs, void* out, int ldo, int64_t o_bs,
                 int B, int heads, int Lq, int Lkv, hipStream_t s, void* scratch = nullptr);
int launch_wan_final(int D, const void* x, const float* mod, const float* w, const float* bias, float* out, int ntok, int Fr, int gh, int gw, int C,
                     float eps, hipStream_t s);
```

### fastgen_amd/csrc/misc.hip

```cpp
#include "common.h"
#include "misc.h"

namespace {

template <typename AT>
__global__ __launch_bounds__(512) void gn_coeffs_kernel(const AT* __restrict__ x1, int C1, const AT* __restrict__ x2,
                                                        int C2, const float* __restrict__ gamma,
                                                        const float* __restrict__ beta, float eps, float2* __restrict__ ab,
                                                        int hw, float2* __restrict__ mr) {
    const int C = C1 + C2;
    const int Q = C >> 2;
    const int lanes = blockDim.x / Q;
    const int groups = min(32, C / 4);
    const int cpg = C / groups;
    const int n = blockIdx.x;
    const int t = threadIdx.x;
    __shared__ double s_sum[512], s_sq[512];
    __shared__ float s_mean[32], s_rstd[32];
    float s = 0.f, ss = 0.f;
    if (t < Q * lanes) {
        const int q = t % Q, pl = t / Q;
        const int c = q * 4;
        const AT* base = (c < C1) ? x1 + (size_t)n * hw * C1 + c : x2 + (size_t)n * hw * C2 + (c - C1);
        const int stride = (c < C1) ? C1 : C2;
// ... 249 lines not shown
                    const float v = ci_scale * x[(((size_t)n * cin + ci) * res + yy) * res + xx];
                    const float* wr = sw + (size_t)(ci * 9 + kh * 3 + kw) * cout + cg * 16;
#pragma unroll
                    for (int j = 0; j < 16; ++j) acc[j] = fmaf(v, wr[j], acc[j]);
                }
            }
        AT* o = out + (((size_t)n * res + y) * res + px) * cout + cg * 16;
#pragma unroll
        for (int j = 0; j < 16; j += 4)
            store4(o + j, f32x4{acc[j] + bias[cg * 16 + j], acc[j + 1] + bias[cg * 16 + j + 1],
                                acc[j + 2] + bias[cg * 16 + j + 2], acc[j + 3] + bias[cg * 16 + j + 3]});
    }
}

template <bool FAST, typename AT>
__global__ __launch_bounds__(256) void aux_out_kernel(const AT* __restrict__ x, const float2* __restrict__ ab,
                                                      const float* __restrict__ w, const float* __restrict__ bias,
                                                      const float* __restrict__ x_t, const float* __restrict__ coef,
                                                      float* __restrict__ out, float* __restrict__ raw, int B, int res, int C, int cout) {
    extern __shared__ float smem_f[];
    float* sw = smem_f;
    float2* sab = reinterpret_cast<float2*>(smem_f + 9 * cout * C);
    const int n = blockIdx.x / res, y = blockIdx.x % res;
    for (int e = threadIdx.x; e < 9 * cout * C; e += blockDim.x) {
        const int c = e % C, co = (e / C) % cout, tap = e / (C * cout);
        sw[e] = w[((size_t)co * C + c) * 9 + tap];
    }
    for (int c = threadIdx.x; c < C; c += blockDim.x) sab[c] = ab[(size_t)n * C + c];
    __syncthreads();
    const int slice = C / 8;
    for (int px0 = 0; px0 < res; px0 += 32) {
        const int px = px0 + (threadIdx.x >> 3), cs = threadIdx.x & 7;
        float acc[4] = {0.f, 0.f, 0.f, 0.f};
        if (px < res) {
            for (int tap = 0; tap < 9; ++tap) {
                const int yy = y + tap / 3 - 1, xx = px + tap % 3 - 1;
                if (yy < 0 || yy >= res || xx < 0 || xx >= res) continue;
                const AT* xp = x + (((size_t)n * res + yy) * res + xx) * C + cs * slice;
                for (int c = 0; c < slice; c += 4) {
                    const f32x4 v = load4(xp + c);
#pragma unroll
                    for (int d = 0; d < 4; ++d) {
                        const float2 k = sab[cs * slice + c + d];
                        const float s = silu_f<FAST>(fmaf(v[d], k.x, k.y));
                        for (int co = 0; co < cout; ++co)
                            acc[co] = fmaf(s, sw[(tap * cout + co) * C + cs * slice + c + d], acc[co]);
                    }
                }
            }
        }
#pragma unroll
        for (int co = 0; co < 4; ++co) {
            acc[co] += __shfl_xor(acc[co], 1);
            acc[co] += __shfl_xor(acc[co], 2);
            acc[co] += __shfl_xor(acc[co], 4);
        }
        if (cs == 0 && px < res) {
            const float c_skip = coef[2 * B + n], c_out = coef[3 * B + n];
            for (int co = 0; co < cout; ++co) {
                const size_t o = (((size_t)n * cout + co) * res + y) * res + px;
                out[o] = c_skip * x_t[o] + c_out * (acc[co] + bias[co]);
                if (raw) raw[o] = acc[co] + bias[co];
            }
        }
    }
}

__device__ __forceinline__ double pick_t(double tv, const double* tp, int ti) { return tp ? tp[ti] : tv; }

__global__ void latents_kernel(const float* __restrict__ noise, double tv, const double* tp, int ti,
                               float* __restrict__ out, int64_t total) {
    const double t = pick_t(tv, tp, ti);
    for (int64_t i = (int64_t)blockIdx.x * blockDim.x + threadIdx.x; i < total; i += (int64_t)gridDim.x * blockDim.x)
        out[i] = (float)((double)noise[i] * t);
}
__device__ __forceinline__ double alpha_of(double t, int sched) { return sched ? 1.0 - t : 1.0; }

__global__ void forward_process_kernel(const float* x0, const float* __restrict__ eps, double tv, const double* tp,
                                       int ti, int sched, float* out, int64_t total) {
#pragma clang fp contract(off)
    const double t = pick_t(tv, tp, ti);
    const double al = alpha_of(t, sched);
    for (int64_t i = (int64_t)blockIdx.x * blockDim.x + threadIdx.x; i < total; i += (int64_t)gridDim.x * blockDim.x)
        out[i] = (float)((double)x0[i] * al + (double)eps[i] * t);
}
__global__ void x0_to_eps_kernel(const float* __restrict__ xt, const float* __restrict__ x0, double tv, const double* tp,
                                 int ti, int sched, double clamp_min, float* __restrict__ out, int64_t total) {
#pragma clang fp contract(off)
    const double t0 = pick_t(tv, tp, ti);
    const double al = alpha_of(t0, sched);
    const double t = (t0 >= 0.0) ? fmax(t0, clamp_min) : fmin(t0, -clamp_min);
    for (int64_t i = (int64_t)blockIdx.x * blockDim.x + threadIdx.x; i < total; i += (int64_t)gridDim.x * blockDim.x)
        out[i] = (float)(((double)xt[i] - (double)x0[i] * al) / t);
}
__global__ void meanflow_update_kernel(const float* x, const float* __restrict__ u, const double* tp, int ia, int ib,
                                       float* out, int64_t total) {
#pragma clang fp contract(off)
    const float dt = (float)(ib >= 0 ? tp[ia] - tp[ib] : tp[ia]);
    for (int64_t i = (int64_t)blockIdx.x * blockDim.x + threadIdx.x; i < total; i += (int64_t)gridDim.x * blockDim.x)
        out[i] = x[i] - dt * u[i];
}

__device__ __forceinline__ void philox_round(uint32_t (&c)[4], uint32_t k0, uint32_t k1) {
    const uint64_t p0 = (uint64_t)0xD2511F53u * c[0];
    const uint64_t p1 = (uint64_t)0xCD9E8D57u * c[2];
    const uint32_t n0 = (uint32_t)(p1 >> 32) ^ c[1] ^ k0;
    const uint32_t n2 = (uint32_t)(p0 >> 32) ^ c[3] ^ k1;
    c[1] = (uint32_t)p1;
    c[3] = (uint32_t)p0;
    c[0] = n0;
    c[2] = n2;
}
__global__ void randn_kernel(float* __restrict__ out, int64_t total, uint64_t seed_v, uint64_t offset_v,
                             const uint64_t* sp) {
    const uint64_t seed = sp ? sp[0] : seed_v;
    const uint64_t offset = sp ? sp[1] + offset_v : offset_v;
    const int64_t nquad = (total + 3) / 4;
    for (int64_t q = (int64_t)blockIdx.x * blockDim.x + threadIdx.x; q < nquad; q += (int64_t)gridDim.x * blockDim.x) {
        uint32_t c[4] = {(uint32_t)q, (uint32_t)((uint64_t)q >> 32), (uint32_t)offset, (uint32_t)(offset >> 32)};
        uint32_t k0 = (uint32_t)seed, k1 = (uint32_t)(seed >> 32);
#pragma unroll
        for (int rnd = 0; rnd < 10; ++rnd) {
            philox_round(c, k0, k1);
            k0 += 0x9E3779B9u;
            k1 += 0xBB67AE85u;
        }
        float z[4];
#pragma unroll
        for (int p = 0; p < 2; ++p) {
            const float u1 = ((float)c[2 * p] + 0.5f) * 2.3283064365386963e-10f;
            const float u2 = ((float)c[2 * p + 1] + 0.5f) * 2.3283064365386963e-10f;
            const float rad = sqrtf(-2.0f * logf(fmaxf(u1, 1e-37f)));
            float sn, cs;
            sincosf(6.283185307179586f * u2, &sn, &cs);
            z[2 * p] = rad * cs;
            z[2 * p + 1] = rad * sn;
        }
        for (int d = 0; d < 4; ++d)
            if (4 * q + d < total) out[4 * q + d] = z[d];
    }
}

__global__ void nchw_to_nhwc_kernel(const float* __restrict__ in, float* __restrict__ out, int B, int C, int HW) {
    const int64_t total = (int64_t)B * C * HW;
    for (int64_t i = (int64_t)blockIdx.x * blockDim.x + threadIdx.x; i < total; i += (int64_t)gridDim.x * blockDim.x) {
        const int c = i % C;
        const int64_t t = i / C;
        const int p = t % HW;
        const int n = t / HW;
        out[i] = in[((int64_t)n * C + c) * HW + p];
    }
}

template <typename AT, bool FAST>
__global__ void gn_silu_pool_kernel(const AT* __restrict__ x, const float2* __restrict__ ab, AT* __restrict__ out, int B,
                                    int H, int W, int C) {
    const int oc = C >> 3;
    const int64_t total = (int64_t)B * H * W * oc;
    for (int64_t i = (int64_t)blockIdx.x * blockDim.x + threadIdx.x; i < total; i += (int64_t)gridDim.x * blockDim.x) {
        const int o = (int)(i % oc);
        int64_t t = i / oc;
        const int xx = (int)(t % W); t /= W;
        const int y = (int)(t % H);
        const int n = (int)(t / H);
        float2 k[8];
        const float2* kp = ab + (size_t)n * C + o * 8;
#pragma unroll
        for (int j = 0; j < 8; ++j) k[j] = kp[j];
        float acc[8];
#pragma unroll
        for (int j = 0; j < 8; ++j) acc[j] = 0.f;
#pragma unroll
        for (int d = 0; d < 4; ++d) {
            const AT* p = x + ((((size_t)n * 2 * H + 2 * y + (d >> 1)) * 2 * W) + 2 * xx + (d & 1)) * C + o * 8;
            const f32x4 lo = load4(p), hi = load4(p + 4);
#pragma unroll
            for (int j = 0; j < 4; ++j) {
                acc[j] += silu_f<FAST>(fmaf(lo[j], k[j].x, k[j].y));
                acc[j + 4] += silu_f<FAST>(fmaf(hi[j], k[j + 4].x, k[j + 4].y));
            }
        }
        AT* q = out + (size_t)i * 8;
        store4(q, f32x4{0.25f * acc[0], 0.25f * acc[1], 0.25f * acc[2], 0.25f * acc[3]});
        store4(q + 4, f32x4{0.25f * acc[4], 0.25f * acc[5], 0.25f * acc[6], 0.25f * acc[7]});
    }
}

template <typename A, typename B>
__global__ void convert_kernel(const A* __restrict__ in, B* __restrict__ out, int64_t total) {
    for (int64_t i = (int64_t)blockIdx.x * blockDim.x + threadIdx.x; i < total; i += (int64_t)gridDim.x * blockDim.x)
        out[i] = (B)(float)in[i];
}

__global__ void embed_times_kernel(const double* __restrict__ tp, int ti, double tv, int ri, double rv, double scale, int sit, int diff,
                                   int f32in, float* __restrict__ te, float* __restrict__ re, int n) {
#pragma clang fp contract(off)
    const int i = blockIdx.x * blockDim.x + threadIdx.x;
    if (i >= n) return;
    const double t = ti >= 0 ? tp[ti] : tv;
    float t_e = f32in ? (float)scale * (float)t : (float)(scale * t);
    if (sit) t_e = 1.0f - t_e;
    te[i] = t_e;
    if (ri != -2 && re) {
        const double r = ri >= 0 ? tp[ri] : rv;
        float r_e = (float)(scale * r);
        if (diff) r_e = t_e - r_e;
        re[i] = r_e;
    }
}
__global__ void flow_to_x0_kernel(const float* __restrict__ xt, const float* __restrict__ v, const double* __restrict__ tp, int ti, float sign,
                                  float* __restrict__ out, int64_t total) {
#pragma clang fp contract(off)
    const double t = tp[ti];
    for (int64_t i = (int64_t)blockIdx.x * blockDim.x + threadIdx.x; i < total; i += (int64_t)gridDim.x * blockDim.x)
        out[i] = (float)((double)xt[i] - (double)(sign * v[i]) * t);
}
__global__ void euler_step_kernel(const float* x, const float* __restrict__ v, const double* __restrict__ tp, int ti, float g, int cfg, float sign,
                                  float* out, float* out2, int64_t total) {
#pragma clang fp contract(off)
    const float dt = (float)(tp[ti + 1] - tp[ti]);
    for (int64_t i = (int64_t)blockIdx.x * blockDim.x + threadIdx.x; i < total; i += (int64_t)gridDim.x * blockDim.x) {
        float vv;
        if (cfg) {
            const float vu = sign * v[i], vc = sign * v[total + i];
            const float d = vc - vu;
            const float gd = g * d;
            vv = vu + gd;
        } else {
            vv = sign * v[i];
        }
        const float dx = dt * vv;
        const float nx = x[i] + dx;
        out[i] = nx;
        if (out2) out2[i] = nx;
    }
}
struct MsCoef {
    float s, g, c0, c1, c2, p0, p1, p2;
};
__device__ __forceinline__ float multistep_elem(const MsCoef& k, int guided, int first, float vc, float vu, float x, float& xl, float& mp,
                                                float& m_out) {
#pragma clang fp contract(off)
    float v = vc;
    if (guided) {
        const float d = vc - vu;
        const float gd = k.g * d;
        v = vu + gd;
    }
    const float sv = k.s * v;
    const float m = x - sv;
    const float xlast = first ? x : xl, mprev = first ? m : mp;
    float xc = k.c0 * xlast;
    float t = k.c1 * mprev;
    xc = xc + t;
    t = k.c2 * m;
    xc = xc + t;
    float xn = k.p0 * xc;
    t = k.p1 * mprev;
    xn = xn + t;
    t = k.p2 * m;
    xn = xn + t;
    xl = xc;
    m_out = m;
    return xn;
}
template <int V>
__global__ void guided_multistep_kernel(const float* __restrict__ v, float* x, float* x2, float* __restrict__ x_last, float* __restrict__ m_prev,
                                        const double* __restrict__ tab, int guided, int first, int64_t total) {
    MsCoef k;
    k.s = (float)tab[0], k.g = (float)tab[1], k.c0 = (float)tab[2], k.c1 = (float)tab[3], k.c2 = (float)tab[4], k.p0 = (float)tab[5],
    k.p1 = (float)tab[6], k.p2 = (float)tab[7];
    const int64_t n = total / V;
    for (int64_t i = (int64_t)blockIdx.x * blockDim.x + threadIdx.x; i < n; i += (int64_t)gridDim.x * blockDim.x) {
        if constexpr (V == 4) {
            const float4 vc = ((const float4*)v)[i];
            const float4 vu = guided ? ((const float4*)(v + total))[i] : vc;
            const float4 xx = ((const float4*)x)[i];
            float4 xl = first ? xx : ((const float4*)x_last)[i], mp = first ? xx : ((const float4*)m_prev)[i], m, xn;
            xn.x = multistep_elem(k, guided, first, vc.x, vu.x, xx.x, xl.x, mp.x, m.x);
            xn.y = multistep_elem(k, guided, first, vc.y, vu.y, xx.y, xl.y, mp.y, m.y);
            xn.z = multistep_elem(k, guided, first, vc.z, vu.z, xx.z, xl.z, mp.z, m.z);
            xn.w = multistep_elem(k, guided, first, vc.w, vu.w, xx.w, xl.w, mp.w, m.w);
            ((float4*)x)[i] = xn;
            if (x2) ((float4*)x2)[i] = xn;
            ((float4*)x_last)[i] = xl;
            ((float4*)m_prev)[i] = m;
        } else {
            const float vc = v[i], vu = guided ? v[total + i] : vc, xx = x[i];
            float xl = first ? xx : x_last[i], mp = first ? xx : m_prev[i], m;
            const float xn = multistep_elem(k, guided, first, vc, vu, xx, xl, mp, m);
            x[i] = xn;
            if (x2) x2[i] = xn;
            x_last[i] = xl;
            m_prev[i] = m;
        }
    }
}
__global__ void copy_rows_kernel(const float* __restrict__ src, int64_t src_pitch, float* __restrict__ dst, int64_t dst_pitch, int64_t run,
                                 int64_t rows) {
    const int64_t total = rows * run;
    for (int64_t i = (int64_t)blockIdx.x * blockDim.x + threadIdx.x; i < total; i += (int64_t)gridDim.x * blockDim.x) {
        const int64_t r = i / run, c = i - r * run;
        dst[r * dst_pitch + c] = src[r * src_pitch + c];
    }
}

inline int ew_grid(int64_t total) {
    int64_t g = (total + 255) / 256;
    return (int)(g < 1 ? 1 : (g > 8192 ? 8192 : g));
}

}

#define RET_LAST() return (int)hipGetLastError()

int launch_gn_coeffs(int dtype, const void* x1, int c1, const void* x2, int c2, const float* gamma, const float* beta,
                     float eps, float2* ab, int batch, int hw, hipStream_t s, float2* mr) {
    const int C = c1 + c2;
    if (C % 4 || (c1 % 4) || C < 16 || C > 2048) return (int)hipErrorInvalidValue;
    const int groups = C / 4 < 32 ? C / 4 : 32;
    if (C % groups || (C / groups) % 4) return (int)hipErrorInvalidValue;
    const int Q = C / 4;
    if (Q > 512) return (int)hipErrorInvalidValue;
    const int threads = (512 / Q) * Q;
    if (dtype)
        hipLaunchKernelGGL(gn_coeffs_kernel<__bf16>, dim3(batch), dim3(threads), 0, s, (const __bf16*)x1, c1, (const __bf16*)x2, c2, gamma, beta, eps, ab, hw, mr);
    else
        hipLaunchKernelGGL(gn_coeffs_kernel<float>, dim3(batch), dim3(threads), 0, s, (const float*)x1, c1, (const float*)x2, c2, gamma, beta, eps, ab, hw, mr);
    RET_LAST();
}

int launch_gn_finalize(const float2* st1, int c1, int s1, const float2* st2, int c2, int s2, const float* gamma,
                       const float* beta, float eps, float2* ab, int batch, int hw, hipStream_t s, float2* mr) {
    const int C = c1 + c2;
    if (C % 4 || (c1 % 4) || C < 16) return (int)hipErrorInvalidValue;
    const int groups = C / 4 < 32 ? C / 4 : 32;
    if (C % groups || (C / groups) % 4) return (int)hipErrorInvalidValue;
    if (C > 512 || (C % 4) || (c1 % 4)) return (int)hipErrorInvalidValue;
    hipLaunchKernelGGL(gn_finalize_kernel, dim3(batch), dim3(512), 0, s, st1, c1, s1, st2, c2, s2, gamma, beta, eps, ab, hw, mr);
    RET_LAST();
}

int launch_precond_coef(const double* t, int t_stride, const double* r, int r_stride, double sigma_data,
                        double sigma_shift, double clamp_min, int drop, float* coef, int B, hipStream_t s) {
    hipLaunchKernelGGL(precond_coef_kernel, dim3((B + 127) / 128), dim3(128), 0, s, t, t_stride, r, r_stride, sigma_data,
                       sigma_shift, clamp_min, drop, coef, B);
    RET_LAST();
}

int launch_mapping_in(const float* c_noise, const float* r_noise, const float* freqs, const float* labels, int label_dim,
                      const float* wl, const float* bl, float* out, int B, int N, int noise_ch, hipStream_t s, const float* aug, const float* wa, int aug_dim) {
    hipLaunchKernelGGL(mapping_in_kernel, dim3((B * N + 255) / 256), dim3(256), 0, s, c_noise, r_noise, freqs, labels,
                       label_dim, wl, bl, out, B, N, noise_ch, aug, wa, aug_dim);
    RET_LAST();
}

int launch_linear(const float* x, const float* w, const float* bias, float* y, int B, int I, int O, int act_silu,
                  hipStream_t s) {
    if (I % 16 == 0 && O % 32 == 0) {
        const bool pair = I % 64 == 0 && B > 32 && O >= 2048;
        dim3 g(O / 32, pair ? (B + 63) / 64 : (B + 31) / 32);
        if (pair) {
            if (act_silu)
                hipLaunchKernelGGL((linear_mfma_kernel<1, 64, 2>), g, dim3(64), 0, s, x, w, bias, y, B, I, O);
            else
                hipLaunchKernelGGL((linear_mfma_kernel<0, 64, 2>), g, dim3(64), 0, s, x, w, bias, y, B, I, O);
        } else if (I % 64 == 0) {
            if (act_silu)
                hipLaunchKernelGGL((linear_mfma_kernel<1, 64, 1>), g, dim3(64), 0, s, x, w, bias, y, B, I, O);
            else
                hipLaunchKernelGGL((linear_mfma_kernel<0, 64, 1>), g, dim3(64), 0, s, x, w, bias, y, B, I, O);
        } else if (act_silu) {
            hipLaunchKernelGGL((linear_mfma_kernel<1, 16, 1>), g, dim3(64), 0, s, x, w, bias, y, B, I, O);
        } else {
            hipLaunchKernelGGL((linear_mfma_kernel<0, 16, 1>), g, dim3(64), 0, s, x, w, bias, y, B, I, O);
        }
        RET_LAST();
    }
    dim3 grid((O + 63) / 64, (B + 63) / 64);
    if (act_silu)
        hipLaunchKernelGGL(linear_kernel<1>, grid, dim3(256), 0, s, x, w, bias, y, B, I, O);
    else
        hipLaunchKernelGGL(linear_kernel<0>, grid, dim3(256), 0, s, x, w, bias, y, B, I, O);
    RET_LAST();
}

int launch_conv_in(int dtype, const float* x, const float* c_in, const float* w, const float* bias, void* out, int B,
                   int res, int cin, int cout, hipStream_t s) {
    if (cout % 16) return (int)hipErrorInvalidValue;
    const size_t lds = (size_t)cin * 9 * cout * sizeof(float);
    if (lds > 64 * 1024) return (int)hipErrorInvalidValue;
    if (dtype)
        hipLaunchKernelGGL(conv_in_kernel<__bf16>, dim3(B * res), dim3(256), lds, s, x, c_in, w, bias, (__bf16*)out, res, cin, cout);
    else
        hipLaunchKernelGGL(conv_in_kernel<float>, dim3(B * res), dim3(256), lds, s, x, c_in, w, bias, (float*)out, res, cin, cout);
    RET_LAST();
}

int launch_aux_out(int dtype, const void* x, const float2* ab, const float* w, const float* bias, const float* x_t,
                   const float* coef, float* out, int B, int res, int C, int cout, hipStream_t s, float* raw) {
    if (cout > 4 || C % 32) return (int)hipErrorInvalidValue;
    const size_t lds = (size_t)9 * cout * C * sizeof(float) + (size_t)C * sizeof(float2);
    if (lds > 64 * 1024) return (int)hipErrorInvalidValue;
    if (dtype)
        hipLaunchKernelGGL((aux_out_kernel<true, __bf16>), dim3(B * res), dim3(256), lds, s, (const __bf16*)x, ab, w, bias, x_t, coef, out, raw, B, res, C, cout);
    else
        hipLaunchKernelGGL((aux_out_kernel<false, float>), dim3(B * res), dim3(256), lds, s, (const float*)x, ab, w, bias, x_t, coef, out, raw, B, res, C, cout);
    RET_LAST();
}

int launch_latents(const float* noise, double tv, const double* tp, int ti, float* out, int64_t total, hipStream_t s) {
    hipLaunchKernelGGL(latents_kernel, dim3(ew_grid(total)), dim3(256), 0, s, noise, tv, tp, ti, out, total);
    RET_LAST();
}
int launch_forward_process(const float* x0, const float* eps, double tv, const double* tp, int ti, int sched, float* out,
                           int64_t total, hipStream_t s) {
    hipLaunchKernelGGL(forward_process_kernel, dim3(ew_grid(total)), dim3(256), 0, s, x0, eps, tv, tp, ti, sched, out, total);
    RET_LAST();
}
int launch_x0_to_eps(const float* xt, const float* x0, double tv, const double* tp, int ti, int sched, double clamp_min,
                     float* out, int64_t total, hipStream_t s) {
    hipLaunchKernelGGL(x0_to_eps_kernel, dim3(ew_grid(total)), dim3(256), 0, s, xt, x0, tv, tp, ti, sched, clamp_min, out, total);
    RET_LAST();
}
int launch_meanflow_update(const float* x, const float* u, const double* tp, int ia, int ib, float* out, int64_t total,
                           hipStream_t s) {
    hipLaunchKernelGGL(meanflow_update_kernel, dim3(ew_grid(total)), dim3(256), 0, s, x, u, tp, ia, ib, out, total);
    RET_LAST();
}
int launch_embed_times(const double* tp, int ti, double tv, int ri, double rv, double scale, int sit, int diff, int f32in, float* te, float* re,
                       int n, hipStream_t s) {
    hipLaunchKernelGGL(embed_times_kernel, dim3((n + 255) / 256), dim3(256), 0, s, tp, ti, tv, ri, rv, scale, sit, diff, f32in, te, re, n);
    RET_LAST();
}
int launch_flow_to_x0(const float* xt, const float* v, const double* tp, int ti, float sign, float* out, int64_t total, hipStream_t s) {
    hipLaunchKernelGGL(flow_to_x0_kernel, dim3(ew_grid(total)), dim3(256), 0, s, xt, v, tp, ti, sign, out, total);
    RET_LAST();
}
int launch_euler_step(const float* x, const float* v, const double* tp, int ti, float g, int cfg, float sign, float* out, float* out2,
                      int64_t total, hipStream_t s) {
    hipLaunchKernelGGL(euler_step_kernel, dim3(ew_grid(total)), dim3(256), 0, s, x, v, tp, ti, g, cfg, sign, out, out2, total);
    RET_LAST();
}
int launch_guided_multistep(const float* v, float* x, float* x2, float* x_last, float* m_prev, const double* tab, int guided, int first,
                            int64_t total, hipStream_t s) {
    const uintptr_t al = (uintptr_t)v | (uintptr_t)x | (uintptr_t)x2 | (uintptr_t)x_last | (uintptr_t)m_prev;
    if (total % 4 == 0 && al % 16 == 0)
        hipLaunchKernelGGL(guided_multistep_kernel<4>, dim3(ew_grid(total / 4)), dim3(256), 0, s, v, x, x2, x_last, m_prev, tab, guided, first, total);
    else
        hipLaunchKernelGGL(guided_multistep_kernel<1>, dim3(ew_grid(total)), dim3(256), 0, s, v, x, x2, x_last, m_prev, tab, guided, first, total);
    RET_LAST();
}
int launch_copy_rows(const float* src, int64_t src_pitch, float* dst, int64_t dst_pitch, int64_t run, int64_t rows, hipStream_t s) {
    hipLaunchKernelGGL(copy_rows_kernel, dim3(ew_grid(rows * run)), dim3(256), 0, s, src, src_pitch, dst, dst_pitch, run, rows);
    RET_LAST();
}
int launch_randn(float* out, int64_t total, uint64_t seed, uint64_t offset, const uint64_t* seed_dev, hipStream_t s) {
    hipLaunchKernelGGL(randn_kernel, dim3(ew_grid((total + 3) / 4)), dim3(256), 0, s, out, total, seed, offset, seed_dev);
    RET_LAST();
}
int launch_gn_silu_pool(int dtype, const void* x, const float2* ab, void* out, int B, int H, int W, int C, hipStream_t s) {
    if (C % 8) return (int)hipErrorInvalidValue;
    const int64_t total = (int64_t)B * H * W * (C / 8);
    if (dtype)
        hipLaunchKernelGGL((gn_silu_pool_kernel<__bf16, true>), dim3(ew_grid(total)), dim3(256), 0, s, (const __bf16*)x, ab, (__bf16*)out, B, H, W, C);
    else
        hipLaunchKernelGGL((gn_silu_pool_kernel<float, false>), dim3(ew_grid(total)), dim3(256), 0, s, (const float*)x, ab, (float*)out, B, H, W, C);
    RET_LAST();
}
int launch_to_act(int dtype, const float* in, void* out, int64_t total, hipStream_t s) {
    if (dtype)
        hipLaunchKernelGGL((convert_kernel<float, __bf16>), dim3(ew_grid(total)), dim3(256), 0, s, in, (__bf16*)out, total);
    else
        hipLaunchKernelGGL((convert_kernel<float, float>), dim3(ew_grid(total)), dim3(256), 0, s, in, (float*)out, total);
    RET_LAST();
}
int launch_from_act(int dtype, const void* in, float* out, int64_t total, hipStream_t s) {
    if (dtype)
        hipLaunchKernelGGL((convert_kernel<__bf16, float>), dim3(ew_grid(total)), dim3(256), 0, s, (const __bf16*)in, out, total);
    else
        hipLaunchKernelGGL((convert_kernel<float, float>), dim3(ew_grid(total)), dim3(256), 0, s, (const float*)in, out, total);
    RET_LAST();
}
template <typename AT>
__global__ __launch_bounds__(256) void nhwc_act_to_nchw_kernel(const AT* __restrict__ in, float* __restrict__ out, int C, int HW) {
    __shared__ float tile[32][33];
    const int b = blockIdx.z, p0 = blockIdx.x * 32, c0 = blockIdx.y * 32;
    const int tx = threadIdx.x & 31, ty = threadIdx.x >> 5;
    for (int i = ty; i < 32; i += 8) tile[i][tx] = (float)in[((size_t)b * HW + p0 + i) * C + c0 + tx];
    __syncthreads();
    for (int i = ty; i < 32; i += 8) out[((size_t)b * C + c0 + i) * HW + p0 + tx] = tile[tx][i];
}
int launch_act_to_nchw(int dtype, const void* in, float* out, int B, int C, int HW, hipStream_t s) {
    dim3 grid(HW / 32, C / 32, B);
    if (dtype)
        hipLaunchKernelGGL(nhwc_act_to_nchw_kernel<__bf16>, grid, dim3(256), 0, s, (const __bf16*)in, out, C, HW);
    else
        hipLaunchKernelGGL(nhwc_act_to_nchw_kernel<float>, grid, dim3(256), 0, s, (const float*)in, out, C, HW);
    RET_LAST();
}
__global__ __launch_bounds__(256) void images_to_u8_kernel(const float* __restrict__ x, uint8_t* __restrict__ out, int64_t npix,
                                                           int C, int HW) {
#pragma clang fp contract(off)
    const int64_t i = (int64_t)blockIdx.x * 256 + threadIdx.x;
    if (i >= npix) return;
    const int64_t n = i / HW;
    const int p = (int)(i - n * HW);
    const float* src = x + n * C * HW + p;
    uint8_t* dst = out + i * C;
    for (int c = 0; c < C; ++c) {
        float v = src[(int64_t)c * HW] * 127.5f;
        v = v + 128.0f;
        v = v < 0.f ? 0.f : (v > 255.f ? 255.f : v);
        dst[c] = v == v ? (uint8_t)(int)v : (uint8_t)0;
    }
}
int launch_images_to_u8(const float* x, uint8_t* out, int64_t B, int C, int HW, hipStream_t s) {
    const int64_t npix = B * HW;
    if (npix <= 0) return 0;
    hipLaunchKernelGGL(images_to_u8_kernel, dim3((unsigned)((npix + 255) / 256)), dim3(256), 0, s, x, out, npix, C, HW);
    RET_LAST();
}
int launch_nchw_to_nhwc(const float* in, float* out, int B, int C, int HW, hipStream_t s) {
    hipLaunchKernelGGL(nchw_to_nhwc_kernel, dim3(ew_grid((int64_t)B * C * HW)), dim3(256), 0, s, in, out, B, C, HW);
    RET_LAST();
}
```

### include/fastgen_amd.h

```cpp
#ifndef FASTGEN_AMD_H
#define FASTGEN_AMD_H

#include <stddef.h>
#include <stdint.h>

#ifdef __cplusplus
extern "C" {
#endif

#define FG_API __attribute__((visibility("default")))

#define FG_OK 0
#define FG_EINVAL 1
#define FG_ENOTREADY 2
#define FG_EHIP 3
#define FG_ENOMEM 4

#define FG_DTYPE_F32 0
#define FG_DTYPE_BF16 1
#define FG_DTYPE_BF16X3 2

#define FG_SAMPLE_SDE 0
#define FG_SAMPLE_ODE 1

#define FG_LOOP_X0 0
#define FG_LOOP_MEANFLOW 1
#define FG_LOOP_EULER 2

#define FG_SCHEDULE_EDM 0
#define FG_SCHEDULE_RF 1

#define FG_DROP_PRECOND_INPUT 1
#define FG_DROP_PRECOND_OUTPUT 2

#define FG_MAX_LEVELS 8

#define FG_MODEL_SONGUNET 0
#define FG_MODEL_DHARIWAL 1

typedef struct fg_edm_config {
    int img_resolution;
    int img_channels;
    int label_dim;
    int augment_dim;
    int model_channels;
    int num_levels;
    int channel_mult[FG_MAX_LEVELS];
    int channel_mult_emb;
    int num_blocks;
    int num_attn_resolutions;
    int attn_resolutions[FG_MAX_LEVELS];
    int channel_mult_noise;
    double sigma_data;
    double sigma_shift;
    int compute_dtype;
    int r_timestep;
    int drop_precond;
    int schedule;
    int model_type;
} fg_edm_config;

typedef struct fg_edm fg_edm;

FG_API const char* fg_last_error(void);
FG_API const char* fg_version(void);

FG_API int fg_edm_create(const fg_edm_config* cfg, fg_edm** out);
FG_API void fg_edm_destroy(fg_edm* h);

FG_API int fg_edm_num_params(const fg_edm* h);
FG_API int fg_edm_param_info(const fg_edm* h, int index, const char** name, int* ndim, int64_t shape[4]);

FG_API int fg_edm_bind_param(fg_edm* h, const char* name, const float* device_ptr, int64_t numel);
FG_API int fg_edm_pack_weights(fg_edm* h, void* stream);

FG_API size_t fg_edm_workspace_bytes(const fg_edm* h, int batch);

FG_API int fg_edm_forward(fg_edm* h, const float* x_t, const double* t, const double* r, const float* class_labels, float* out,
                   float* emb_out, int batch, void* workspace, size_t workspace_bytes, void* stream);

FG_API int fg_edm_num_feature_taps(const fg_edm* h);
FG_API int fg_edm_feature_info(const fg_edm* h, int index, const char** key, int* channels, int* resolution);
FG_API int fg_edm_forward_features(fg_edm* h, const float* x_t, const double* t, const double* r, const float* class_labels,
                            float* out, float* const* features, int batch, void* workspace, size_t workspace_bytes,
                            void* stream);

FG_API int fg_sampler_run(fg_edm* h, const float* noise, const float* class_labels, const double* t_list, int steps,
                   int sample_type, int loop_kind, const float* eps, uint64_t seed, float* out, int batch,
                   void* workspace, size_t workspace_bytes, int use_graph, void* stream);

FG_API int fg_edm_t_list(int sample_steps, double* out_host);
FG_API int fg_rf_t_list(int sample_steps, double* out_host);

FG_API int fg_edm_profile_begin(fg_edm* h);
FG_API int fg_edm_profile_end(fg_edm* h, int64_t* launches, double* total_ms, double* total_flops);


FG_API int fg_edm_num_blocks(const fg_edm* h);
FG_API int fg_edm_block_info(const fg_edm* h, int index, const char** key, int* cin, int* cout, int* res_in, int* res_out,
                      int* has_attention);
FG_API int fg_edm_run_block(fg_edm* h, int index, const float* x1, int c1, const float* x2, int c2, const float* emb,
                     float* out, int batch, void* workspace, size_t workspace_bytes, void* stream);

FG_API int fg_op_gn_coeffs(const float* x1, int c1, const float* x2, int c2, const float* gamma, const float* beta,
                    float eps, float* ab_out, int batch, int hw, void* stream);

FG_API size_t fg_op_adm_conv_pack_bytes(int mode, int cout, int cin, int ks);
FG_API int fg_op_adm_conv_pack(int mode, const float* w_oihw, void* packed, int cout, int cin, int ks, void* stream);
FG_API int fg_op_adm_conv(int mode, int ks, const float* src1, int c1, const float* src2, int c2, int batch, int hs, int h,
                          int res_mode, const float* ab, int silu, const void* packed, const float* bias, const float* resid,
                          int resid_mode, float* out, int cout, void* stream);
FG_API size_t fg_op_adm_gn_workspace_bytes(int batch, int hw, int c);
FG_API int fg_op_adm_gn_coeffs(const float* x1, int c1, const float* x2, int c2, const float* gamma, const float* beta, float eps,
                               const float* temb, int temb_stride, float* ab_out, int batch, int hw, void* workspace,
                               size_t workspace_bytes, void* stream);
FG_API int fg_op_adm_attention(const float* qkv, float* out, int batch, int t, int heads, void* stream);
FG_API int fg_op_adm_map_in(const float* c_noise, const float* freqs, const float* aug, const float* wa, int aug_dim, float* out,
                            int batch, int n, void* stream);

FG_API int fg_op_latents(const float* noise, double t_init, float* out, int64_t total, void* stream);
FG_API int fg_op_forward_process(const float* x0, const float* eps, double t, int schedule, float* out, int64_t total,
                          void* stream);
FG_API int fg_op_x0_to_eps(const float* xt, const float* x0, double t, int schedule, float* out, int64_t total, void* stream);
FG_API size_t fg_op_conv_wgrad_workspace_bytes(int batch, int res, int cin, int cout, int ks);
FG_API int fg_op_conv_wgrad(const void* act, const void* dy, float* dw, int batch, int res, int cin, int cout, int ks,
                     int accumulate, void* workspace, size_t workspace_bytes, void* stream);

FG_API int fg_op_conv_wgrad_f32(const float* act, const float* dy, float* dw, int batch, int res, int cin, int cout, int ks,
                                int accumulate, void* workspace, size_t workspace_bytes, void* stream);

FG_API int fg_edm_bind_grad(fg_edm* h, const char* name, float* grad, int64_t numel);
FG_API size_t fg_edm_block_backward_workspace_bytes(const fg_edm* h, int index, int batch);
FG_API int fg_edm_run_block_backward(fg_edm* h, int index, const float* x1, int c1, const float* x2, int c2, const float* emb,
                              const float* dout, float* dx1, float* dx2, float* demb, int batch, void* workspace,
                              size_t workspace_bytes, void* stream);

FG_API size_t fg_edm_backward_workspace_bytes(const fg_edm* h, int batch);
FG_API int fg_edm_backward(fg_edm* h, const float* x_t, const double* t, const double* r, const float* labels, const float* dout,
                    float* out, int have_forward, int batch, void* workspace, size_t workspace_bytes, void* stream);
FG_API int fg_edm_forward_train(fg_edm* h, const float* x_t, const double* t, const double* r, const float* labels, float* out,
                         float* const* features, int batch, void* workspace, size_t workspace_bytes, void* stream);
FG_API int fg_edm_backward_ex(fg_edm* h, const float* x_t, const double* t, const double* r, const float* labels, const float* dout,
                       const float* const* dfeatures, float* out, float* dx_t, int have_forward, int batch, void* workspace,
                       size_t workspace_bytes, void* stream);

#define FG_BWD_DECODER 1
#define FG_BWD_ENCODER 2
#define FG_BWD_EMBED 4
FG_API int fg_edm_backward_part(fg_edm* h, const float* x_t, const double* t, const double* r, const float* labels, const float* dout,
                                const float* const* dfeatures, float* out, float* dx_t, int have_forward, int parts, int batch,
                                void* workspace, size_t workspace_bytes, void* stream);

FG_API int fg_disc_edm_num_params(int res);
FG_API size_t fg_disc_edm_workspace_bytes(int res, int batch);
FG_API int fg_disc_edm_run(const float* feat, int res, const float* const* params, float* logits, const float* dlogits, float* dfeat,
                    float* const* grads, int batch, void* workspace, size_t workspace_bytes, void* stream);

FG_API int fg_edm_jvp(fg_edm* h, const float* x_t, const double* t, const double* r, const float* labels, const float* vx, const float* vt,
               const float* vr, float* out, float* jvp, int batch, void* workspace, size_t workspace_bytes, void* stream);

FG_API int fg_edm_set_training(fg_edm* h, int training);

FG_API int fg_edm_set_augment(fg_edm* h, const float* augment_labels);

FG_API int fg_edm_set_dropout(fg_edm* h, float p, uint64_t seed);
FG_API int fg_op_dropout_mask(float* out, int64_t total, float p, uint32_t block_index, uint64_t seed, void* stream);

typedef struct fg_dit_config {
    int input_size;
    int patch_size;
    int in_channels;
    int hidden_size;
    int depth;
    int num_heads;
    int mlp_hidden;
    int embedding_rows;
    int r_timestep;
    int compute_dtype;
} fg_dit_config;
typedef struct fg_dit fg_dit;

FG_API int fg_dit_create(const fg_dit_config* cfg, fg_dit** out);
FG_API void fg_dit_destroy(fg_dit* h);
FG_API int fg_dit_num_params(const fg_dit* h);
FG_API int fg_dit_param_info(const fg_dit* h, int index, const char** name, int* ndim, int64_t shape[4]);
FG_API int fg_dit_bind_param(fg_dit* h, const char* name, const float* device_ptr, int64_t numel);
FG_API int fg_dit_pack_weights(fg_dit* h, void* stream);
FG_API int fg_dit_pack_group(fg_dit* h, const char* prefix, const char* exclude, void* stream);
FG_API size_t fg_dit_workspace_bytes(const fg_dit* h, int batch);
FG_API int fg_dit_forward(fg_dit* h, const float* x_t, const float* t, const float* r, const int64_t* class_ids, float* out,
                          float* cond_out, int batch, void* workspace, size_t workspace_bytes, void* stream);

FG_API int fg_dit_forward_features(fg_dit* h, const float* x_t, const float* t, const float* r, const int64_t* class_ids, float* out,
                                   float* cond_out, const int* feature_blocks, float* const* features, int num_features, int batch,
                                   void* workspace, size_t workspace_bytes, void* stream);

typedef struct fg_dit_sampler_config {
    double t_scale;
    double guidance_scale;
    int use_sit_convention;
    int time_cond_diff;
    int net_pred_flow;
    int schedule;
} fg_dit_sampler_config;
FG_API size_t fg_dit_sampler_workspace_bytes(const fg_dit* h, int batch, int guided);
FG_API int fg_dit_sampler_run(fg_dit* h, const fg_dit_sampler_config* cfg, const float* noise, const int64_t* class_ids,
                              const int64_t* neg_class_ids, const double* t_list, int steps, int sample_type, int loop_kind, const float* eps,
                              uint64_t seed, float* out, int batch, void* workspace, size_t workspace_bytes, int use_graph, void* stream);

typedef struct fg_wan_config {
    int num_heads;
    int head_dim;
    int in_channels;
    int out_channels;
    int text_dim;
    int freq_dim;
    int ffn_dim;
    int num_layers;
    int rope_max_seq_len;
    int chunk_size;
    int total_num_frames;
    float eps;
} fg_wan_config;
typedef struct fg_wan fg_wan;

FG_API int fg_wan_create(const fg_wan_config* cfg, fg_wan** out);
FG_API void fg_wan_destroy(fg_wan* h);
FG_API int fg_wan_num_params(const fg_wan* h);
FG_API int fg_wan_param_info(const fg_wan* h, int index, const char** name, int* ndim, int64_t shape[5]);
FG_API int fg_wan_bind_param(fg_wan* h, const char* name, const float* device_ptr, int64_t numel);
FG_API int fg_wan_pack_weights(fg_wan* h, void* stream);
FG_API int fg_wan_pack_group(fg_wan* h, const char* prefix, const char* exclude, void* stream);
FG_API size_t fg_wan_workspace_bytes(const fg_wan* h, int batch, int frames, int height, int width);
FG_API int fg_wan_clear_caches(fg_wan* h, void* stream);
FG_API int fg_wan_select_cache_tag(fg_wan* h, int tag);
FG_API int fg_wan_set_text(fg_wan* h, const float* text, int batch, int text_len, void* workspace, size_t workspace_bytes, void* stream);
FG_API int fg_wan_forward(fg_wan* h, const float* x_t, const float* t_frames, float* out, int batch, int frames, int height, int width,
                          int cur_start_frame, int store_kv, void* workspace, size_t workspace_bytes, void* stream);
FG_API int fg_wan_forward_block_causal(fg_wan* h, const float* x_t, const float* t_frames, float* out, int batch, int frames, int height,
                                       int width, void* workspace, size_t workspace_bytes, void* stream);

typedef struct fg_wan_block_taps {
    float* attn1;
    float* x_attn1;
    float* attn2;
    float* x_attn2;
    float* x_ffn;
} fg_wan_block_taps;
FG_API int fg_wan_forward_features(fg_wan* h, const float* x_t, const float* t_frames, float* out, int batch, int frames, int height, int width,
                                   int cur_start_frame, int store_kv, int block_causal, const int* tap_blocks, const fg_wan_block_taps* taps,
                                   int num_taps, float* tokens_out, float* temb_out, void* workspace, size_t workspace_bytes, void* stream);

typedef struct fg_wan_sampler_config {
    double t_scale;
    double context_noise;
    int net_pred_flow;
    int schedule;
    int prefill_frames;
// ... 79 lines not shown
```

Before: 2895 img/s.

## Add 16-channel split-bf16 aux head and fuse pooled skip input into down blocks

Adds a specialized output-head kernel for cout<=16 that uses 16x16x32 MFMA tiles, double-buffered LDS staging and prefetched split-bf16 weights, replacing the generic 32-wide head that wasted half its tile. Down blocks in bf16x3 inference now have the GN-SiLU-pool kernel also emit the raw 2x2-pooled input, so the 1x1 skip conv reads the small pooled tensor instead of resampling the full-resolution input. Down blocks also become eligible for the ws-packed conv path. New exported APIs and env toggles are added alongside. This costs an extra workspace buffer and an extra write in the pool kernel.

Result: no change. 2908 img/s (median of 6 runs) (+0.4%).

```diff
diff --git a/fastgen_amd/_lib.py b/fastgen_amd/_lib.py
--- a/fastgen_amd/_lib.py
+++ b/fastgen_amd/_lib.py
@@ -94,6 +94,12 @@
                                   POINTER(c_int), POINTER(c_int)]),
     "fg_edm_run_block": (c_int, [c_void_p, c_int, c_void_p, c_int, c_void_p, c_int, c_void_p, c_void_p, c_int, c_void_p,
                                  c_size_t, c_void_p]),
+    "fg_edm_run_block_ex": (c_int, [c_void_p, c_int, c_void_p, c_int, c_void_p, c_int, c_void_p, c_void_p, c_int, c_int, c_void_p, c_void_p,
+                                    c_void_p, c_void_p, c_void_p, c_size_t, c_void_p]),
+    "fg_op_gn_silu_pool": (c_int, [c_void_p, c_void_p, c_void_p, c_void_p, c_int, c_int, c_int, c_void_p]),
+    "fg_op_aux_head_workspace_bytes": (c_size_t, [c_int]),
+    "fg_op_aux_head": (c_int, [c_void_p, c_void_p, c_void_p, c_void_p, c_void_p, c_void_p, c_void_p, c_void_p, c_int, c_int, c_int, c_void_p,
+                               c_size_t, c_void_p]),
     "fg_op_gn_coeffs": (c_int, [c_void_p, c_int, c_void_p, c_int, c_void_p, c_void_p, c_float, c_void_p, c_int, c_int, c_void_p]),
     "fg_op_adm_conv_pack_bytes": (c_size_t, [c_int, c_int, c_int, c_int]),
     "fg_op_adm_conv_pack": (c_int, [c_int, c_void_p, c_void_p, c_int, c_int, c_int, c_void_p]),
diff --git a/fastgen_amd/csrc/aux.hip b/fastgen_amd/csrc/aux.hip
--- a/fastgen_amd/csrc/aux.hip
+++ b/fastgen_amd/csrc/aux.hip
@@ -1,3 +1,7 @@
+#include <stdlib.h>
+
+#include <type_traits>
+
 #include "common.h"
 #include "misc.h"
 
@@ -116,6 +120,182 @@
     }
 }
 
+constexpr int A16_HPIX = HROWS * HWID;
+constexpr int A16_NIT = (A16_HPIX + 63) / 64;
+constexpr int A16_PLANE = A16_NIT * 64 * 16;
+constexpr int A16_BUF = 8 * A16_PLANE;
+constexpr int A16_TAPB = 2048;
+
+struct A16Frag {
+    bf16x8 hi, lo;
+};
+
+__device__ __forceinline__ void a16_barrier() {
+    asm volatile("s_waitcnt lgkmcnt(0)\n\ts_barrier" ::: "memory");
+}
+
+__global__ __launch_bounds__(256) void aux_head16_kernel(const float* __restrict__ x, const float2* __restrict__ ab,
+                                                         const __bf16* __restrict__ wpack, const float* __restrict__ bias,
+                                                         const float* __restrict__ x_t, const float* __restrict__ coef,
+                                                         float* __restrict__ out, float* __restrict__ raw, int B, int C, int cout) {
+    __shared__ __attribute__((aligned(16))) char smem[2 * A16_BUF];
+    const int tid = threadIdx.x, lane = tid & 63;
+    const int wave = __builtin_amdgcn_readfirstlane(tid >> 6);
+    const int col = lane & 15, g4 = lane >> 4;
+    const int n = blockIdx.x >> 3, row0 = (blockIdx.x & 7) * 4;
+    const int nchunk = C / 32;
+
+    const int oct = tid & 3, pslot = tid >> 2;
+    const float* src[A16_NIT];
+    bool valid[A16_NIT];
+    int hlds[A16_NIT];
+#pragma unroll
+    for (int i = 0; i < A16_NIT; ++i) {
+        const int hq = pslot + 64 * i;
+        const int hqc = min(hq, A16_HPIX - 1);
+        const int hy = hqc / HWID, hx = hqc - hy * HWID;
+        const int y = row0 + hy - 1, xx = hx - 1;
+        valid[i] = hq < A16_HPIX && y >= 0 && y < 32 && xx >= 0 && xx < 32;
+        const int yc = min(max(y, 0), 31), xc = min(max(xx, 0), 31);
+        src[i] = x + (((size_t)n * 32 + yc) * 32 + xc) * C + oct * 8;
+        hlds[i] = oct * A16_PLANE + hq * 16;
+    }
+    const float2* abn = ab + (size_t)n * C + oct * 8;
+
+    struct Staged {
+        f32x4 raw[A16_NIT][2];
+        float2 ab[8];
+    };
+    auto stage_load = [&](Staged& st, int chunk) __attribute__((always_inline)) {
+#pragma unroll
+        for (int i = 0; i < A16_NIT; ++i) {
+            const float* p = src[i] + chunk * 32;
+            st.raw[i][0] = *reinterpret_cast<const f32x4*>(p);
+            st.raw[i][1] = *reinterpret_cast<const f32x4*>(p + 4);
+        }
+        const float2* p = abn + chunk * 32;
+#pragma unroll
+        for (int j = 0; j < 8; j += 2) {
+            const f32x4 q = *reinterpret_cast<const f32x4*>(p + j);
+            st.ab[j] = make_float2(q[0], q[1]);
+            st.ab[j + 1] = make_float2(q[2], q[3]);
+        }
+    };
+    auto stage_store = [&](const Staged& st, char* abuf) __attribute__((always_inline)) {
+#pragma unroll
+        for (int i = 0; i < A16_NIT; ++i) {
+            float v[8];
+#pragma unroll
+            for (int j = 0; j < 8; ++j) v[j] = silu_f<true>(fmaf(st.raw[i][j >> 2][j & 3], st.ab[j].x, st.ab[j].y));
+            bf16x8 hi, lo;
+            split8(v, hi, lo);
+            fg_u32x4 wh = __builtin_bit_cast(fg_u32x4, hi), wl = __builtin_bit_cast(fg_u32x4, lo);
+#pragma unroll
+            for (int j = 0; j < 4; ++j) {
+                wh[j] = valid[i] ? wh[j] : 0u;
+                wl[j] = valid[i] ? wl[j] : 0u;
+            }
+            *reinterpret_cast<fg_u32x4*>(abuf + hlds[i]) = wh;
+            *reinterpret_cast<fg_u32x4*>(abuf + hlds[i] + 4 * A16_PLANE) = wl;
+        }
+    };
+
+    const __amdgpu_buffer_rsrc_t wrs = make_rsrc(wpack);
+    const int wvoff = lane * 16;
+    auto load_w = [&](int byte_off) -> A16Frag {
+        A16Frag f;
+        f.hi = __builtin_bit_cast(bf16x8, __builtin_amdgcn_raw_buffer_load_b128(wrs, wvoff, byte_off, 0));
+        f.lo = __builtin_bit_cast(bf16x8, __builtin_amdgcn_raw_buffer_load_b128(wrs, wvoff, byte_off + 1024, 0));
+        return f;
+    };
+    A16Frag wq[9];
+#pragma unroll
+    for (int tap = 0; tap < 9; ++tap) wq[tap] = load_w(tap * A16_TAPB);
+
+    f32x4 acc[2];
+    acc[0] = acc[1] = f32x4{0.f, 0.f, 0.f, 0.f};
+
+    Staged st;
+    stage_load(st, 0);
+    stage_store(st, smem);
+    a16_barrier();
+
+    const int lane_off = g4 * A16_PLANE + (wave * HWID + col) * 16;
+    auto chunk_step = [&](int c, auto more_c) __attribute__((always_inline)) {
+        constexpr bool more = decltype(more_c)::value;
+        if (more) stage_load(st, c + 1);
+        const char* abase = smem + (c & 1) * A16_BUF + lane_off;
+        const int wnxt = (c + 1) * 9 * A16_TAPB;
+        auto read_x = [&](int tap, A16Frag (&xf)[2]) {
+            const int off = ((tap / 3) * HWID + tap % 3) * 16;
+#pragma unroll
+            for (int pt = 0; pt < 2; ++pt) {
+                xf[pt].hi = *reinterpret_cast<const bf16x8*>(abase + off + pt * 256);
+                xf[pt].lo = *reinterpret_cast<const bf16x8*>(abase + off + pt * 256 + 4 * A16_PLANE);
+            }
+        };
+        auto mma6 = [&](int tap, const A16Frag (&xf)[2]) {
+#pragma unroll
+            for (int pt = 0; pt < 2; ++pt) acc[pt] = __builtin_amdgcn_mfma_f32_16x16x32_bf16(wq[tap].hi, xf[pt].lo, acc[pt], 0, 0, 0);
+#pragma unroll
+            for (int pt = 0; pt < 2; ++pt) acc[pt] = __builtin_amdgcn_mfma_f32_16x16x32_bf16(wq[tap].lo, xf[pt].hi, acc[pt], 0, 0, 0);
+#pragma unroll
+            for (int pt = 0; pt < 2; ++pt) acc[pt] = __builtin_amdgcn_mfma_f32_16x16x32_bf16(wq[tap].hi, xf[pt].hi, acc[pt], 0, 0, 0);
+            if (more) wq[tap] = load_w(wnxt + tap * A16_TAPB);
+        };
+        A16Frag x0[2], x1[2];
+        read_x(0, x0);
+#pragma unroll
+        for (int tap = 0; tap < 9; tap += 2) {
+            if (tap + 1 < 9) read_x(tap + 1, x1);
+            __builtin_amdgcn_sched_barrier(0);
+            mma6(tap, x0);
+            __builtin_amdgcn_sched_barrier(0);
+            if (tap + 2 < 9) read_x(tap + 2, x0);
+            __builtin_amdgcn_sched_barrier(0);
+            if (tap + 1 < 9) mma6(tap + 1, x1);
+            __builtin_amdgcn_sched_barrier(0);
+        }
+        if (more) stage_store(st, smem + ((c + 1) & 1) * A16_BUF);
+        a16_barrier();
+    };
+    for (int c = 0; c + 1 < nchunk; ++c) chunk_step(c, std::true_type{});
+    chunk_step(nchunk - 1, std::false_type{});
+    const float c_skip = coef[2 * B + n], c_out = coef[3 * B + n];
+    const int y = row0 + wave;
+#pragma unroll
+    for (int e = 0; e < 4; ++e) {
+        const int ch = 4 * g4 + e;
+        if (ch < cout) {
+            const float bv = bias[ch];
+#pragma unroll
+            for (int pt = 0; pt < 2; ++pt) {
+                const size_t o = (((size_t)n * cout + ch) * 32 + y) * 32 + pt * 16 + col;
+                out[o] = c_skip * x_t[o] + c_out * (acc[pt][e] + bv);
+                if (raw) raw[o] = acc[pt][e] + bv;
+            }
+        }
+    }
+}
+
+__global__ void pack_aux16_weights_kernel(const float* __restrict__ w, __bf16* __restrict__ out, int C, int cout) {
+    const int total = C * 9 * 16;
+    for (int idx = blockIdx.x * blockDim.x + threadIdx.x; idx < total; idx += gridDim.x * blockDim.x) {
+        int t = idx;
+        const int j = t % 8; t /= 8;
+        const int lane = t % 64; t /= 64;
+        const int tap = t % 9; t /= 9;
+        const int chunk = t;
+        const int co = lane & 15;
+        const int ci = chunk * 32 + 8 * (lane >> 4) + j;
+        const float v = (co < cout) ? w[((size_t)co * C + ci) * 9 + tap] : 0.f;
+        const size_t o = ((size_t)idx / 512) * 1024 + (idx % 512);
+        const __bf16 hi = (__bf16)v;
+        out[o] = hi;
+        out[o + 512] = (__bf16)(v - (float)hi);
+    }
+}
+
 template <typename T>
 __global__ __launch_bounds__(256) void stem_kernel(const float* __restrict__ x, const float* __restrict__ c_in,
                                                    const T* __restrict__ wpack, const float* __restrict__ bias,
@@ -189,9 +369,20 @@
 
 size_t aux_pack_elems(int C) { return (size_t)C * 9 * 32; }
 
+static bool aux16_enabled() {
+    static const bool on = [] {
+        const char* e = getenv("FASTGEN_AMD_AUX16");
+        return !(e && e[0] == '0');
+    }();
+    return on;
+}
+static bool aux16_use(int dtype, int C, int cout) { return dtype == 2 && aux16_enabled() && cout >= 1 && cout <= 16 && C >= 32 && C % 32 == 0; }
+
 int launch_pack_aux_weights(int dtype, const float* w, void* out, int C, int cout, hipStream_t s) {
     const int grid = (int)((aux_pack_elems(C) + 255) / 256);
-    if (dtype == 2)
+    if (aux16_use(dtype, C, cout))
+        hipLaunchKernelGGL(pack_aux16_weights_kernel, dim3((grid + 1) / 2), dim3(256), 0, s, w, (__bf16*)out, C, cout);
+    else if (dtype == 2)
         hipLaunchKernelGGL(pack_aux_weights_kernel<bf16x3>, dim3(grid), dim3(256), 0, s, w, (__bf16*)out, C, cout);
     else if (dtype)
         hipLaunchKernelGGL(pack_aux_weights_kernel<__bf16>, dim3(grid), dim3(256), 0, s, w, (__bf16*)out, C, cout);
@@ -204,7 +395,9 @@
 
 int launch_aux_head(int dtype, const void* x, const float2* ab, const void* wpack, const float* bias, const float* x_t,
                     const float* coef, float* out, int B, int C, int cout, hipStream_t s, float* raw) {
-    if (dtype == 2)
+    if (aux16_use(dtype, C, cout))
+        hipLaunchKernelGGL(aux_head16_kernel, dim3(B * 8), dim3(256), 0, s, (const float*)x, ab, (const __bf16*)wpack, bias, x_t, coef, out, raw, B, C, cout);
+    else if (dtype == 2)
         hipLaunchKernelGGL(aux_head_kernel<bf16x3>, dim3(B * 8), dim3(256), 0, s, (const float*)x, ab, (const __bf16*)wpack, bias, x_t, coef, out, raw, B, C, cout);
     else if (dtype)
         hipLaunchKernelGGL(aux_head_kernel<__bf16>, dim3(B * 8), dim3(256), 0, s, (const __bf16*)x, ab, (const __bf16*)wpack, bias, x_t, coef, out, raw, B, C, cout);
diff --git a/fastgen_amd/csrc/engine.hip b/fastgen_amd/csrc/engine.hip
--- a/fastgen_amd/csrc/engine.hip
+++ b/fastgen_amd/csrc/engine.hip
@@ -109,6 +109,8 @@
     std::vector<Act> skip;
     Act xa, xb, h, xattn;
     void *sbuf, *aout, *pool;
+    void* praw = nullptr;
+    int down_sel = -1;
     void *cvt1, *cvt2;
     void *q, *k, *vt;
     float *x, *x_pred, *eps;
@@ -668,6 +670,7 @@
     w.h = act((size_t)B * max_act, st_elems);
     w.sbuf = A.take((size_t)B * max_act * tsz);
     w.pool = A.take((size_t)B * max_act * tsz);
+    w.praw = h->cmode == FG_DTYPE_BF16X3 ? A.take((size_t)B * max_act * tsz) : nullptr;
     w.cvt1 = A.take((size_t)B * max_act * 4 * tsz);
     w.cvt2 = A.take((size_t)B * max_act * 4 * tsz);
     w.xattn = act((size_t)B * max_attn_hw * 256, st_elems);
@@ -733,6 +736,14 @@
 bool attn_merge_enabled() {
     static const bool on = [] {
         const char* e = getenv("FASTGEN_AMD_ATTN_MERGE");
+        return !(e && e[0] == '0');
+    }();
+    return on;
+}
+
+bool down_fused_enabled() {
+    static const bool on = [] {
+        const char* e = getenv("FASTGEN_AMD_DOWN_FUSED");
         return !(e && e[0] == '0');
     }();
     return on;
@@ -753,6 +764,9 @@
     a.temb = temb + b.temb_off; a.temb_stride = h->temb_total;
     a.resid = nullptr; a.scale = 1.0f; a.out = w.h.p; a.Cout = b.cout; a.stats = w.h.st;
     const bool x3_up = b.up && w.infer && !w.a1d && h->cmode == FG_DTYPE_BF16X3 && conv_ws_enabled();
+    const bool x3_down = b.down && !c2 && w.infer && !w.a1d && h->cmode == FG_DTYPE_BF16X3 && w.praw &&
+                         (w.down_sel < 0 ? down_fused_enabled() : w.down_sel != 0);
+    if (b.down && !x3_down) a.wpack_ws = nullptr;
     bool sub0 = false;
     if (x3_up && conv_subpix_mode() == 2 && b.p_conv0_sub) {
         ConvArgs p = a;
@@ -764,7 +778,7 @@
         w.h.slots = conv_launch_stat_slots(h->cmode, 3, PRO_GN_SILU, RES_SUBPIX, OUT_NHWC, a);
         HIP_TRY(conv_launch(h, 3, PRO_GN_SILU, RES_SUBPIX, OUT_NHWC, a, s));
     } else if (b.down && !c2) {
-        HIP_TRY(launch_gn_silu_pool(h->dtype, x1.p, w.ab0, w.pool, B, b.res_out, b.res_out, c1, s));
+        HIP_TRY(launch_gn_silu_pool(h->dtype, x1.p, w.ab0, w.pool, B, b.res_out, b.res_out, c1, s, x3_down && b.has_skip ? (float*)w.praw : nullptr));
         a.src1 = w.pool; a.Hs = a.Ws = b.res_out; a.ab = nullptr;
         w.h.slots = conv_launch_stat_slots(h->cmode, 3, PRO_NONE, RES_NONE, OUT_NHWC, a);
         HIP_TRY(conv_launch(h, 3, PRO_NONE, RES_NONE, OUT_NHWC, a, s));
@@ -788,7 +802,8 @@
         k.src1 = x1.p; k.src2 = c2 ? x2.p : nullptr; k.C1 = c1; k.C2 = c2;
         k.Hs = k.Ws = b.res_in; k.H = k.W = low ? b.res_in : b.res_out; k.B = B;
         k.wpack = b.p_skip; k.bias = h->P(b.skip_b); k.scale = 1.0f; k.out = w.sbuf; k.Cout = b.cout;
-        HIP_TRY(conv_launch(h, 1, PRO_NONE, low ? RES_NONE : res_mode, OUT_NHWC, k, s));
+        if (x3_down) k.src1 = w.praw, k.Hs = k.Ws = b.res_out;
+        HIP_TRY(conv_launch(h, 1, PRO_NONE, (low || x3_down) ? RES_NONE : res_mode, OUT_NHWC, k, s));
         resid = w.sbuf;
         d.rshift = low ? 1 : 0;
     }
@@ -926,7 +941,7 @@
         if ((rc = h->alloc(&b->p_conv0, conv_pack_elems(b->cout, b->cin, 3) * tsz))) return rc;
         if ((rc = h->alloc(&b->p_conv1, conv_pack_elems(b->cout, b->cout, 3) * tsz))) return rc;
         const bool x3 = h->cmode == FG_DTYPE_BF16X3;
-        if ((x3 ? conv_x3ws_shape_ok(b->cout, b->cin, b->res_out) : conv_ws_shape_ok(h->cmode, b->cout, b->cin, b->res_out)) && !b->down &&
+        if ((x3 ? conv_x3ws_shape_ok(b->cout, b->cin, b->res_out) : conv_ws_shape_ok(h->cmode, b->cout, b->cin, b->res_out)) && (x3 || !b->down) &&
             (rc = h->alloc(&b->p_conv0_ws, conv_pack_elems(b->cout, b->cin, 3) * tsz)))
             return rc;
         if ((x3 ? conv_x3ws_shape_ok(b->cout, b->cout, b->res_out) : conv_ws_shape_ok(h->cmode, b->cout, b->cout, b->res_out)) &&
@@ -1304,8 +1319,18 @@
 
 int fg_edm_run_block(fg_edm* h, int index, const float* x1, int c1, const float* x2, int c2, const float* emb, float* out,
                      int batch, void* workspace, size_t workspace_bytes, void* stream) {
+    return fg_edm_run_block_ex(h, index, x1, c1, x2, c2, emb, out, batch, -1, nullptr, nullptr, nullptr, nullptr, workspace, workspace_bytes, stream);
+}
+
+int fg_edm_run_block_ex(fg_edm* h, int index, const float* x1, int c1, const float* x2, int c2, const float* emb, float* out, int batch,
+                        int down_fused, float* skip_out, const float* next_gamma, const float* next_beta, float* next_ab,
+                        void* workspace, size_t workspace_bytes, void* stream) {
     if (!h || !x1 || !emb || !out) return fail(FG_EINVAL, "null argument");
-    if (h->adm) return adm_run_block(h, index, x1, c1, x2, c2, emb, out, batch, workspace, workspace_bytes, (hipStream_t)stream);
+    if (h->adm) {
+        if (down_fused >= 0 || skip_out || next_ab) return adm_refuse(h, "fg_edm_run_block_ex's extra outputs");
+        return adm_run_block(h, index, x1, c1, x2, c2, emb, out, batch, workspace, workspace_bytes, (hipStream_t)stream);
+    }
+    if (next_ab && (!next_gamma || !next_beta)) return fail(FG_EINVAL, "next_ab needs next_gamma and next_beta");
     if (!h->packed) return fail(FG_ENOTREADY, "weights are not packed (call fg_edm_pack_weights)");
     if (index < 0 || index >= (int)h->blocks.size()) return fail(FG_EINVAL, "block index out of range");
     Workspace w;
@@ -1323,9 +1348,18 @@
         a2.p = w.cvt2;
     }
     w.infer = true;
+    w.down_sel = down_fused < 0 ? -1 : (down_fused ? 1 : 0);
+    if (skip_out && !b.has_skip) return fail(FG_EINVAL, "%s has no skip convolution", b.key.c_str());
     int rc = run_block(h, b, a1, c1, a2, c2, w.temb, w.xa, batch, w, s);
     if (rc) return rc;
     HIP_TRY(launch_from_act(h->dtype, w.xa.p, out, (int64_t)npix_out * b.cout, s));
+    if (skip_out) {
+        const bool low = b.up && h->cmode == FG_DTYPE_BF16X3 && conv_ws_enabled() && conv_subpix_mode() >= 1;
+        HIP_TRY(launch_from_act(h->dtype, w.sbuf, skip_out, (int64_t)(low ? npix_in : npix_out) * b.cout, s));
+    }
+    if (next_ab)
+        HIP_TRY(launch_gn_finalize(w.xa.st, b.cout, w.xa.slots, nullptr, 0, 0, next_gamma, next_beta, kBlockEps, (float2*)next_ab, batch,
+                                   b.res_out * b.res_out, s, nullptr));
     return FG_OK;
 }
 
@@ -1339,6 +1373,30 @@
                     float* ab_out, int batch, int hw, void* stream) {
     if (!x1 || !gamma || !beta || !ab_out) return fail(FG_EINVAL, "null argument");
     HIP_TRY(launch_gn_coeffs(0, x1, c1, c2 ? x2 : nullptr, c2, gamma, beta, eps, (float2*)ab_out, batch, hw, (hipStream_t)stream));
+    return FG_OK;
+}
+
+int fg_op_gn_silu_pool(const float* x, const float* ab, float* out, float* raw_out, int batch, int h_out, int c, void* stream) {
+    if (!x || !ab || !out) return fail(FG_EINVAL, "fg_op_gn_silu_pool: null pointer");
+    if (batch <= 0 || h_out <= 0 || h_out > 4096 || c <= 0 || c % 8) return fail(FG_EINVAL, "fg_op_gn_silu_pool: batch %d, h_out %d, c %d (a multiple of 8)", batch, h_out, c);
+    if (((uintptr_t)x | (uintptr_t)out | (uintptr_t)raw_out) & 15 || (uintptr_t)ab & 7)
+        return fail(FG_EINVAL, "fg_op_gn_silu_pool: x / out / raw_out must be 16-byte aligned, ab 8-byte aligned");
+    HIP_TRY(launch_gn_silu_pool(0, x, (const float2*)ab, out, batch, h_out, h_out, c, (hipStream_t)stream, raw_out));
+    return FG_OK;
+}
+
+size_t fg_op_aux_head_workspace_bytes(int c) { return c > 0 && c % 32 == 0 ? aux_pack_elems(c) * 4 : 0; }
+int fg_op_aux_head(const float* x, const float* ab, const float* w_oihw, const float* bias, const float* x_t, const float* coef, float* out,
+                   float* raw_out, int batch, int c, int cout, void* workspace, size_t workspace_bytes, void* stream) {
+    if (!x || !ab || !w_oihw || !bias || !x_t || !coef || !out || !workspace) return fail(FG_EINVAL, "fg_op_aux_head: null pointer");
+    if (batch <= 0 || batch > (1 << 20) || !aux_head_supported(FG_DTYPE_BF16X3, 32, c, cout) || c < 32 || cout < 1)
+        return fail(FG_EINVAL, "fg_op_aux_head: batch %d, c %d (a multiple of 32), cout %d (1 .. 32)", batch, c, cout);
+    if (workspace_bytes < fg_op_aux_head_workspace_bytes(c))
+        return fail(FG_EINVAL, "fg_op_aux_head: workspace too small (%zu < %zu bytes)", workspace_bytes, fg_op_aux_head_workspace_bytes(c));
+    if (((uintptr_t)x | (uintptr_t)workspace) & 15 || (uintptr_t)ab & 15) return fail(FG_EINVAL, "fg_op_aux_head: x / ab / workspace must be 16-byte aligned");
+    hipStream_t s = (hipStream_t)stream;
+    HIP_TRY(launch_pack_aux_weights(FG_DTYPE_BF16X3, w_oihw, workspace, c, cout, s));
+    HIP_TRY(launch_aux_head(FG_DTYPE_BF16X3, x, (const float2*)ab, workspace, bias, x_t, coef, out, batch, c, cout, s, raw_out));
     return FG_OK;
 }
 
diff --git a/fastgen_amd/csrc/engine_train.inc b/fastgen_amd/csrc/engine_train.inc
--- a/fastgen_amd/csrc/engine_train.inc
+++ b/fastgen_amd/csrc/engine_train.inc
@@ -469,7 +469,7 @@
         ad0 = q.dskip;
     }
     if ((rc = tangent_conv(h, 3, RES_NONE, ad0, cin, res, res, b.p_conv0, cout, dtemb + b.temb_off, nullptr, 1.0f, q.dh0, B, s,
-                           b.p_conv0_ws))) return rc;
+                           b.down ? nullptr : b.p_conv0_ws))) return rc;
     DropArgs drop;
     if (st.a1d && h->dropout_p > 0.f) drop.p = h->dropout_p, drop.seed = h->dropout_seed, drop.block = st.index;
     HIP_TRY(launch_gn_jvp(h->dtype, 0, st.h, cout, nullptr, 0, q.dh0, st.ab1, st.mr1, q.P, q.S, q.g1, B, res, s, drop));
diff --git a/fastgen_amd/csrc/misc.h b/fastgen_amd/csrc/misc.h
--- a/fastgen_amd/csrc/misc.h
+++ b/fastgen_amd/csrc/misc.h
@@ -32,7 +32,7 @@
 int launch_guided_multistep(const float* v, float* x, float* x2, float* x_last, float* m_prev, const double* tab, int guided, int first,
                             int64_t total, hipStream_t s);
 int launch_copy_rows(const float* src, int64_t src_pitch, float* dst, int64_t dst_pitch, int64_t run, int64_t rows, hipStream_t s);
-int launch_gn_silu_pool(int dtype, const void* x, const float2* ab, void* out, int B, int H, int W, int C, hipStream_t s);
+int launch_gn_silu_pool(int dtype, const void* x, const float2* ab, void* out, int B, int H, int W, int C, hipStream_t s, float* raw = nullptr);
 int launch_to_act(int dtype, const float* in, void* out, int64_t total, hipStream_t s);
 int launch_from_act(int dtype, const void* in, float* out, int64_t total, hipStream_t s);
 struct DropArgs {
diff --git a/fastgen_amd/csrc/misc.hip b/fastgen_amd/csrc/misc.hip
--- a/fastgen_amd/csrc/misc.hip
+++ b/fastgen_amd/csrc/misc.hip
@@ -425,9 +425,9 @@
     }
 }
 
-template <typename AT, bool FAST>
-__global__ void gn_silu_pool_kernel(const AT* __restrict__ x, const float2* __restrict__ ab, AT* __restrict__ out, int B,
-                                    int H, int W, int C) {
+template <typename AT, bool FAST, bool RAW>
+__global__ void gn_silu_pool_kernel(const AT* __restrict__ x, const float2* __restrict__ ab, AT* __restrict__ out,
+                                    float* __restrict__ raw, int B, int H, int W, int C) {
     const int oc = C >> 3;
     const int64_t total = (int64_t)B * H * W * oc;
     for (int64_t i = (int64_t)blockIdx.x * blockDim.x + threadIdx.x; i < total; i += (int64_t)gridDim.x * blockDim.x) {
@@ -440,9 +440,9 @@
         const float2* kp = ab + (size_t)n * C + o * 8;
 #pragma unroll
         for (int j = 0; j < 8; ++j) k[j] = kp[j];
-        float acc[8];
-#pragma unroll
-        for (int j = 0; j < 8; ++j) acc[j] = 0.f;
+        float acc[8], racc[8];
+#pragma unroll
+        for (int j = 0; j < 8; ++j) acc[j] = racc[j] = 0.f;
 #pragma unroll
         for (int d = 0; d < 4; ++d) {
             const AT* p = x + ((((size_t)n * 2 * H + 2 * y + (d >> 1)) * 2 * W) + 2 * xx + (d & 1)) * C + o * 8;
@@ -451,11 +451,17 @@
             for (int j = 0; j < 4; ++j) {
                 acc[j] += silu_f<FAST>(fmaf(lo[j], k[j].x, k[j].y));
                 acc[j + 4] += silu_f<FAST>(fmaf(hi[j], k[j + 4].x, k[j + 4].y));
+                if (RAW) racc[j] += lo[j], racc[j + 4] += hi[j];
             }
         }
         AT* q = out + (size_t)i * 8;
         store4(q, f32x4{0.25f * acc[0], 0.25f * acc[1], 0.25f * acc[2], 0.25f * acc[3]});
         store4(q + 4, f32x4{0.25f * acc[4], 0.25f * acc[5], 0.25f * acc[6], 0.25f * acc[7]});
+        if (RAW) {
+            float* rq = raw + (size_t)i * 8;
+            *reinterpret_cast<f32x4*>(rq) = f32x4{racc[0] * 0.25f, racc[1] * 0.25f, racc[2] * 0.25f, racc[3] * 0.25f};
+            *reinterpret_cast<f32x4*>(rq + 4) = f32x4{racc[4] * 0.25f, racc[5] * 0.25f, racc[6] * 0.25f, racc[7] * 0.25f};
+        }
     }
 }
 
@@ -732,13 +738,17 @@
     hipLaunchKernelGGL(randn_kernel, dim3(ew_grid((total + 3) / 4)), dim3(256), 0, s, out, total, seed, offset, seed_dev);
     RET_LAST();
 }
-int launch_gn_silu_pool(int dtype, const void* x, const float2* ab, void* out, int B, int H, int W, int C, hipStream_t s) {
+int launch_gn_silu_pool(int dtype, const void* x, const float2* ab, void* out, int B, int H, int W, int C, hipStream_t s, float* raw) {
     if (C % 8) return (int)hipErrorInvalidValue;
     const int64_t total = (int64_t)B * H * W * (C / 8);
-    if (dtype)
-        hipLaunchKernelGGL((gn_silu_pool_kernel<__bf16, true>), dim3(ew_grid(total)), dim3(256), 0, s, (const __bf16*)x, ab, (__bf16*)out, B, H, W, C);
+    if (dtype && raw)
+        hipLaunchKernelGGL((gn_silu_pool_kernel<__bf16, true, true>), dim3(ew_grid(total)), dim3(256), 0, s, (const __bf16*)x, ab, (__bf16*)out, raw, B, H, W, C);
+    else if (dtype)
+        hipLaunchKernelGGL((gn_silu_pool_kernel<__bf16, true, false>), dim3(ew_grid(total)), dim3(256), 0, s, (const __bf16*)x, ab, (__bf16*)out, raw, B, H, W, C);
+    else if (raw)
+        hipLaunchKernelGGL((gn_silu_pool_kernel<float, false, true>), dim3(ew_grid(total)), dim3(256), 0, s, (const float*)x, ab, (float*)out, raw, B, H, W, C);
     else
-        hipLaunchKernelGGL((gn_silu_pool_kernel<float, false>), dim3(ew_grid(total)), dim3(256), 0, s, (const float*)x, ab, (float*)out, B, H, W, C);
+        hipLaunchKernelGGL((gn_silu_pool_kernel<float, false, false>), dim3(ew_grid(total)), dim3(256), 0, s, (const float*)x, ab, (float*)out, raw, B, H, W, C);
     RET_LAST();
 }
 int launch_to_act(int dtype, const float* in, void* out, int64_t total, hipStream_t s) {
diff --git a/include/fastgen_amd.h b/include/fastgen_amd.h
--- a/include/fastgen_amd.h
+++ b/include/fastgen_amd.h
@@ -101,9 +101,18 @@
                       int* has_attention);
 FG_API int fg_edm_run_block(fg_edm* h, int index, const float* x1, int c1, const float* x2, int c2, const float* emb,
                      float* out, int batch, void* workspace, size_t workspace_bytes, void* stream);
+FG_API int fg_edm_run_block_ex(fg_edm* h, int index, const float* x1, int c1, const float* x2, int c2, const float* emb, float* out,
+                        int batch, int down_fused, float* skip_out, const float* next_gamma, const float* next_beta, float* next_ab,
+                        void* workspace, size_t workspace_bytes, void* stream);
 
 FG_API int fg_op_gn_coeffs(const float* x1, int c1, const float* x2, int c2, const float* gamma, const float* beta,
                     float eps, float* ab_out, int batch, int hw, void* stream);
+
+FG_API int fg_op_gn_silu_pool(const float* x, const float* ab, float* out, float* raw_out, int batch, int h_out, int c, void* stream);
+
+FG_API size_t fg_op_aux_head_workspace_bytes(int c);
+FG_API int fg_op_aux_head(const float* x, const float* ab, const float* w_oihw, const float* bias, const float* x_t, const float* coef,
+                   float* out, float* raw_out, int batch, int c, int cout, void* workspace, size_t workspace_bytes, void* stream);
 
 FG_API size_t fg_op_adm_conv_pack_bytes(int mode, int cout, int cin, int ks);
 FG_API int fg_op_adm_conv_pack(int mode, const float* w_oihw, void* packed, int cout, int cin, int ks, void* stream);
```
